# CDCgov/zoe

Measured on AMD Instinct MI355X. Metric: read-alignments/sec (150 bp vs 2 kb ref), higher is better.
Workload: dtype int16

## Files before the change

include/zoe_sw.h:

```cpp
#ifndef ZOE_SW_H
#define ZOE_SW_H

#include <stddef.h>
#include <stdint.h>

#ifdef __cplusplus
extern "C" {
#endif

typedef enum zsw_error {
    ZSW_OK = 0,
    ZSW_ERR_EMPTY_SEQUENCE = 1,
    ZSW_ERR_GAP_OPEN_OUT_OF_RANGE = 2,
    ZSW_ERR_GAP_EXTEND_OUT_OF_RANGE = 3,
    ZSW_ERR_BAD_GAP_WEIGHTS = 4,
    ZSW_ERR_INVALID_ARGUMENT = -1,
    ZSW_ERR_HIP = -2,
    ZSW_ERR_NO_DEVICE = -3,
    ZSW_ERR_UNSUPPORTED = -4,
    ZSW_ERR_NOT_CONFIGURED = -5
} zsw_error;

typedef enum zsw_status {
    ZSW_STATUS_SOME = 0,
    ZSW_STATUS_OVERFLOWED = 1,
    ZSW_STATUS_UNMAPPED = 2,
    ZSW_STATUS_EMPTY = 3,
    ZSW_STATUS_BELOW_MIN_SCORE = 4
} zsw_status;

typedef enum zsw_int_type { ZSW_I8 = 0, ZSW_I16 = 1, ZSW_I32 = 2, ZSW_U8 = 3, ZSW_U16 = 4, ZSW_U32 = 5 } zsw_int_type;

typedef enum zsw_mem { ZSW_MEM_HOST = 0, ZSW_MEM_DEVICE = 1 } zsw_mem;

typedef struct zsw_context zsw_context;

typedef enum zsw_encoding { ZSW_ENCODING_BYTES = 0, ZSW_ENCODING_PACKED4 = 1 } zsw_encoding;

typedef struct zsw_batch {
    const uint8_t* bases;
    const uint64_t* offsets;
    uint32_t fixed_len;
    uint64_t n_reads;
    zsw_mem mem;
    zsw_encoding encoding;
} zsw_batch;

typedef struct zsw_alignment {
    uint32_t score;
    uint32_t ref_start, ref_end;
    uint32_t query_start, query_end;
    uint32_t ref_len, query_len;
    uint32_t n_ciglets;
    uint64_t ciglet_offset;
} zsw_alignment;

zsw_error zsw_pack4_host(zsw_context* ctx, const uint8_t* bases, uint64_t n_reads, uint32_t len, uint8_t* out_packed);

zsw_error zsw_create(int device_id, zsw_context** out);
void zsw_destroy(zsw_context* ctx);
const char* zsw_last_error_string(const zsw_context* ctx);
int zsw_device_count(void);

zsw_error zsw_set_scoring(zsw_context* ctx, const int8_t* weights, int S, const uint8_t* index_map, int gap_open,
                          int gap_extend);

zsw_error zsw_set_reference(zsw_context* ctx, const uint8_t* reference, size_t len, zsw_mem mem);

zsw_error zsw_score_batch(zsw_context* ctx, const zsw_batch* reads, zsw_int_type int_type, int lanes,
                          uint32_t* out_score, uint8_t* out_status, void* stream);

zsw_error zsw_score_batch_from(zsw_context* ctx, const zsw_batch* reads, int from_width, int preset_bits,
                               uint32_t* out_score, uint8_t* out_status, uint8_t* out_tier, void* stream);

zsw_error zsw_score_ends_batch(zsw_context* ctx, const zsw_batch* reads, zsw_int_type int_type, int lanes,
                               uint32_t* out_score, uint32_t* out_ref_end, uint32_t* out_query_end,
                               uint8_t* out_status, void* stream);

zsw_error zsw_score_ranges_batch(zsw_context* ctx, const zsw_batch* reads, zsw_int_type int_type, int lanes,
                                 uint32_t* out_score, uint32_t* out_ref_start, uint32_t* out_ref_end,
                                 uint32_t* out_query_start, uint32_t* out_query_end, uint8_t* out_status, void* stream);

zsw_error zsw_score_ranges_batch_from(zsw_context* ctx, const zsw_batch* reads, int from_width, int preset_bits,
                                      uint32_t* out_score, uint32_t* out_ref_start, uint32_t* out_ref_end,
                                      uint32_t* out_query_start, uint32_t* out_query_end, uint8_t* out_status, uint8_t* out_tier,
                                      void* stream);

zsw_error zsw_align_batch(zsw_context* ctx, const zsw_batch* reads, zsw_int_type int_type, int lanes, int invert,
                          zsw_alignment* out_aln, uint8_t* out_status, uint32_t* out_inc, uint8_t* out_op,
                          uint64_t ciglet_cap, uint64_t* out_n_ciglets, void* stream);

zsw_error zsw_align_batch_from(zsw_context* ctx, const zsw_batch* reads, int from_width, int preset_bits, int invert,
                               zsw_alignment* out_aln, uint8_t* out_status, uint8_t* out_tier, uint32_t* out_inc,
                               uint8_t* out_op, uint64_t ciglet_cap, uint64_t* out_n_ciglets, void* stream);

zsw_error zsw_align_3pass_batch(zsw_context* ctx, const zsw_batch* reads, zsw_int_type int_type, int lanes, int invert,
                                zsw_alignment* out_aln, uint8_t* out_status, uint32_t* out_inc, uint8_t* out_op,
                                uint64_t ciglet_cap, uint64_t* out_n_ciglets, void* stream);
zsw_error zsw_align_3pass_batch_from(zsw_context* ctx, const zsw_batch* reads, int from_width, int preset_bits, int invert,
                                     zsw_alignment* out_aln, uint8_t* out_status, uint8_t* out_tier, uint32_t* out_inc,
                                     uint8_t* out_op, uint64_t ciglet_cap, uint64_t* out_n_ciglets, void* stream);


zsw_error zsw_set_complement(zsw_context* ctx, const uint8_t* table );

zsw_error zsw_score_strands_batch_from(zsw_context* ctx, const zsw_batch* reads, int from_width, int preset_bits,
                                       uint32_t* out_score, uint8_t* out_status, uint8_t* out_tier, uint8_t* out_strand, void* stream);

zsw_error zsw_orient_batch(zsw_context* ctx, const zsw_batch* reads, const uint8_t* strand, uint8_t* out_bases, void* stream);

zsw_error zsw_align_3pass_strands_batch_from(zsw_context* ctx, const zsw_batch* reads, int from_width, int preset_bits, int invert,
                                             zsw_alignment* out_aln, uint8_t* out_status, uint8_t* out_tier, uint8_t* out_strand,
                                             uint32_t* out_inc, uint8_t* out_op, uint64_t ciglet_cap, uint64_t* out_n_ciglets, void* stream);

zsw_error zsw_strand_counts(zsw_context* ctx, uint64_t* out );

zsw_error zsw_set_profile_sequence(zsw_context* ctx, const uint8_t* sequence, size_t len, zsw_mem mem);
zsw_error zsw_score_shared_batch(zsw_context* ctx, const zsw_batch* reads, zsw_int_type int_type, int lanes, uint32_t* out_score,
                                 uint8_t* out_status, void* stream);
zsw_error zsw_score_shared_batch_from(zsw_context* ctx, const zsw_batch* reads, int from_width, int preset_bits, uint32_t* out_score,
                                      uint8_t* out_status, uint8_t* out_tier, void* stream);
zsw_error zsw_score_ends_shared_batch(zsw_context* ctx, const zsw_batch* reads, zsw_int_type int_type, int lanes, uint32_t* out_score,
                                      uint32_t* out_ref_end, uint32_t* out_query_end, uint8_t* out_status, void* stream);
zsw_error zsw_score_ranges_shared_batch(zsw_context* ctx, const zsw_batch* reads, zsw_int_type int_type, int lanes, uint32_t* out_score,
                                        uint32_t* out_ref_start, uint32_t* out_ref_end, uint32_t* out_query_start, uint32_t* out_query_end,
                                        uint8_t* out_status, void* stream);
zsw_error zsw_score_ranges_shared_batch_from(zsw_context* ctx, const zsw_batch* reads, int from_width, int preset_bits, uint32_t* out_score,
                                             uint32_t* out_ref_start, uint32_t* out_ref_end, uint32_t* out_query_start, uint32_t* out_query_end,
                                             uint8_t* out_status, uint8_t* out_tier, void* stream);
zsw_error zsw_align_shared_batch(zsw_context* ctx, const zsw_batch* reads, zsw_int_type int_type, int lanes, int invert, zsw_alignment* out_aln,
                                 uint8_t* out_status, uint32_t* out_inc, uint8_t* out_op, uint64_t ciglet_cap, uint64_t* out_n_ciglets,
                                 void* stream);
zsw_error zsw_align_shared_batch_from(zsw_context* ctx, const zsw_batch* reads, int from_width, int preset_bits, int invert,
                                      zsw_alignment* out_aln, uint8_t* out_status, uint8_t* out_tier, uint32_t* out_inc, uint8_t* out_op,
                                      uint64_t ciglet_cap, uint64_t* out_n_ciglets, void* stream);
zsw_error zsw_align_3pass_shared_batch(zsw_context* ctx, const zsw_batch* reads, zsw_int_type int_type, int lanes, int invert, zsw_alignment* out_aln,
                                       uint8_t* out_status, uint32_t* out_inc, uint8_t* out_op, uint64_t ciglet_cap, uint64_t* out_n_ciglets,
                                       void* stream);
zsw_error zsw_align_3pass_shared_batch_from(zsw_context* ctx, const zsw_batch* reads, int from_width, int preset_bits, int invert,
                                            zsw_alignment* out_aln, uint8_t* out_status, uint8_t* out_tier, uint32_t* out_inc, uint8_t* out_op,
                                            uint64_t ciglet_cap, uint64_t* out_n_ciglets, void* stream);

typedef enum zsw_filter_result {
    ZSW_FILTER_REJECT = 0,
    ZSW_FILTER_PASS = 1,
    ZSW_FILTER_NONE = 2,
    ZSW_FILTER_BAD_WINDOW = 255
} zsw_filter_result;
zsw_error zsw_sneaky_snake_batch(zsw_context* ctx, const zsw_batch* reads, const uint32_t* ref_start, const uint32_t* ref_len,
                                 float threshold, uint8_t* out_pass, void* stream);

typedef struct zsw_group zsw_group;
zsw_error zsw_group_create(const int* device_ids, int n_devices, zsw_group** out);
void zsw_group_destroy(zsw_group* group);
int zsw_group_size(const zsw_group* group);
zsw_context* zsw_group_context(zsw_group* group, int i);
const char* zsw_group_last_error_string(const zsw_group* group);
zsw_error zsw_group_set_scoring(zsw_group* group, const int8_t* weights, int S, const uint8_t* index_map, int gap_open,
                                int gap_extend);
zsw_error zsw_group_set_reference(zsw_group* group, const uint8_t* reference, size_t len);

zsw_error zsw_group_score_batch_from(zsw_group* group, const zsw_batch* reads, int from_width, int preset_bits,
                                     uint32_t* out_score, uint8_t* out_status, uint8_t* out_tier);

zsw_error zsw_group_align_batch_from(zsw_group* group, const zsw_batch* reads, int from_width, int preset_bits, int invert,
                                     zsw_alignment* out_aln, uint8_t* out_status, uint8_t* out_tier, uint32_t* out_inc,
                                     uint8_t* out_op, uint64_t ciglet_cap, uint64_t* out_n_ciglets);
zsw_error zsw_group_align_3pass_batch_from(zsw_group* group, const zsw_batch* reads, int from_width, int preset_bits, int invert,
                                           zsw_alignment* out_aln, uint8_t* out_status, uint8_t* out_tier, uint32_t* out_inc,
                                           uint8_t* out_op, uint64_t ciglet_cap, uint64_t* out_n_ciglets);

zsw_error zsw_group_score_batch_from_device(zsw_group* group, const zsw_batch* shards, int from_width, int preset_bits,
                                            uint32_t* const* out_score, uint8_t* const* out_status);

zsw_error zsw_synth_reads(zsw_context* ctx, uint64_t seed, uint64_t first, uint64_t n, uint32_t len, uint8_t* out_device,
                          void* stream);
zsw_error zsw_synth_reads_ragged(zsw_context* ctx, uint64_t seed, uint64_t first, uint64_t n, uint32_t min_len,
                                 uint32_t max_len, const uint64_t* offsets_device, uint8_t* out_device, void* stream);
uint32_t zsw_synth_length(uint64_t seed, uint64_t index, uint32_t min_len, uint32_t max_len);

zsw_error zsw_selftest(zsw_context* ctx);

void zsw_synth_reference_host(uint64_t seed, uint64_t len, uint8_t* out);
void zsw_synth_reads_host(uint64_t seed, uint64_t first, uint64_t n, uint32_t len, const uint8_t* ref, uint32_t R,
                          uint8_t* out);
void zsw_synth_reads_ragged_host(uint64_t seed, uint64_t first, uint64_t n, uint32_t min_len, uint32_t max_len,
                                 const uint64_t* offsets, const uint8_t* ref, uint32_t R, uint8_t* out);

zsw_error zsw_timing_enable(zsw_context* ctx, int enable);
zsw_error zsw_timing_read(zsw_context* ctx, double* seconds, uint64_t* launches);
zsw_error zsw_timing_read_window(zsw_context* ctx, double* seconds, uint64_t* launches);

typedef enum zsw_option { ZSW_OPTION_EXACT_PRUNING = 1, ZSW_OPTION_MIN_SCORE = 2 } zsw_option;
zsw_error zsw_set_option(zsw_context* ctx, zsw_option option, int64_t value);

zsw_error zsw_min_score_counts(zsw_context* ctx, uint64_t* out );

typedef enum zsw_debug_flag {
    ZSW_DEBUG_SCORE_V1 = 1,
    ZSW_DEBUG_NO_TILES = 2,
    ZSW_DEBUG_NO_W32 = 4,
    ZSW_DEBUG_NO_WIDE = 8,
    ZSW_DEBUG_NO_SIDE_STREAMS = 16,
    ZSW_DEBUG_NO_PIPELINE = 32,
    ZSW_DEBUG_ALIGN_NO_PACKED = 64,
    ZSW_DEBUG_SCORE_PRUNE = 128,
    ZSW_DEBUG_SCORE_PRUNE_ANY_SIZE = 256,
    ZSW_DEBUG_PRUNE_STRIP = 512,
    ZSW_DEBUG_ALIGN_LONG_WARMUP = 1024,
    ZSW_DEBUG_SEED_NO_BAND = 2048,
    ZSW_DEBUG_SEED_WIDE_BAND = 4096,
    ZSW_DEBUG_NO_ROW_CHUNKS = 8192,
    ZSW_DEBUG_RANGES_EXACT_REVERSE = 16384,
    ZSW_DEBUG_ALIGN_NO_CERTIFICATE = 32768,
    ZSW_DEBUG_SEED_STRIP_FIRST_TIER = 65536,
    ZSW_DEBUG_SEED_DIAG_LANE_EVENTS = 131072
} zsw_debug_flag;
zsw_error zsw_debug_set(zsw_context* ctx, uint32_t flags);

zsw_error zsw_debug_band_records(zsw_context* ctx, int32_t* records);

zsw_error zsw_debug_cert_records(zsw_context* ctx, int32_t* records);

zsw_error zsw_debug_strand_records(zsw_context* ctx, int32_t* records);

typedef enum zsw_launch_kind {
    ZSW_LAUNCH_V1_FAST = 0,
    ZSW_LAUNCH_V1_BIASED = 1,
    ZSW_LAUNCH_V2 = 2,
    ZSW_LAUNCH_WIDE = 3,
    ZSW_LAUNCH_V1_FAST_REV = 4,
    ZSW_LAUNCH_V1_BIASED_REV = 5,
    ZSW_LAUNCH_WIDE_REV = 6,
    ZSW_LAUNCH_TILE_V2 = 7,
    ZSW_LAUNCH_TILE_WIDE = 8,
    ZSW_LAUNCH_TILE_W32 = 9,
    ZSW_LAUNCH_EXACT32 = 10,
    ZSW_LAUNCH_EXACT32_WORKLIST = 11,
    ZSW_LAUNCH_SEED_WINDOW = 12,
    ZSW_LAUNCH_SEED_BAND = 13,
    ZSW_LAUNCH_PRUNED = 14
} zsw_launch_kind;
zsw_error zsw_debug_score_launches(zsw_context* ctx, uint32_t* records, uint32_t capacity, uint32_t* out_n);

zsw_error zsw_prune_rescored(zsw_context* ctx, uint64_t* out_reads);

#ifdef __cplusplus
}
#endif
#endif
```

zoe_amd/_lib.py:

```python
from __future__ import annotations

import ctypes as C
import os

_HERE = os.path.dirname(os.path.abspath(__file__))
LIB_PATH = os.path.join(_HERE, "libzoe_sw_hip.so")

ZSW_OK = 0
ERROR_NAMES = {
    0: "ZSW_OK",
    1: "ProfileError::EmptySequence",
    2: "ProfileError::GapOpenOutOfRange",
    3: "ProfileError::GapExtendOutOfRange",
    4: "ProfileError::BadGapWeights",
    -1: "ZSW_ERR_INVALID_ARGUMENT",
    -2: "ZSW_ERR_HIP",
    -3: "ZSW_ERR_NO_DEVICE",
    -4: "ZSW_ERR_UNSUPPORTED",
    -5: "ZSW_ERR_NOT_CONFIGURED",
}
MEM_HOST, MEM_DEVICE = 0, 1
DEBUG_SCORE_V1, DEBUG_NO_TILES, DEBUG_NO_W32, DEBUG_NO_WIDE, DEBUG_NO_SIDE_STREAMS, DEBUG_NO_PIPELINE, DEBUG_ALIGN_NO_PACKED = 1, 2, 4, 8, 16, 32, 64
DEBUG_SCORE_PRUNE, DEBUG_SCORE_PRUNE_ANY_SIZE, DEBUG_PRUNE_STRIP, DEBUG_ALIGN_LONG_WARMUP, DEBUG_SEED_NO_BAND, DEBUG_SEED_WIDE_BAND = 128, 256, 512, 1024, 2048, 4096
DEBUG_NO_ROW_CHUNKS = 8192
DEBUG_RANGES_EXACT_REVERSE = 16384
DEBUG_ALIGN_NO_CERTIFICATE = 32768
DEBUG_SEED_STRIP_FIRST_TIER = 65536
DEBUG_SEED_DIAG_LANE_EVENTS = 131072
(LAUNCH_V1_FAST, LAUNCH_V1_BIASED, LAUNCH_V2, LAUNCH_WIDE, LAUNCH_V1_FAST_REV, LAUNCH_V1_BIASED_REV, LAUNCH_WIDE_REV, LAUNCH_TILE_V2, LAUNCH_TILE_WIDE,
 LAUNCH_TILE_W32, LAUNCH_EXACT32, LAUNCH_EXACT32_WORKLIST, LAUNCH_SEED_WINDOW, LAUNCH_SEED_BAND, LAUNCH_PRUNED) = range(15)
OPTION_EXACT_PRUNING = 1
OPTION_MIN_SCORE = 2
INT_TYPES = {"i8": 0, "i16": 1, "i32": 2, "u8": 3, "u16": 4, "u32": 5}

SYMBOLS = [
    "zsw_pack4_host", "zsw_create", "zsw_destroy", "zsw_last_error_string", "zsw_device_count", "zsw_set_scoring", "zsw_set_reference",
    "zsw_score_batch", "zsw_score_batch_from", "zsw_score_ends_batch", "zsw_score_ranges_batch", "zsw_score_ranges_batch_from", "zsw_align_batch", "zsw_align_batch_from", "zsw_align_3pass_batch", "zsw_align_3pass_batch_from", "zsw_sneaky_snake_batch",
    "zsw_set_profile_sequence", "zsw_score_shared_batch", "zsw_score_shared_batch_from", "zsw_score_ends_shared_batch", "zsw_score_ranges_shared_batch",
    "zsw_score_ranges_shared_batch_from", "zsw_align_shared_batch", "zsw_align_shared_batch_from", "zsw_align_3pass_shared_batch", "zsw_align_3pass_shared_batch_from",
    "zsw_synth_reads", "zsw_synth_reads_ragged", "zsw_synth_length", "zsw_synth_reference_host", "zsw_synth_reads_host",
    "zsw_synth_reads_ragged_host", "zsw_selftest", "zsw_timing_enable", "zsw_timing_read", "zsw_timing_read_window", "zsw_debug_set", "zsw_debug_band_records", "zsw_debug_cert_records", "zsw_prune_rescored", "zsw_set_option",
    "zsw_group_create", "zsw_group_destroy", "zsw_group_size", "zsw_group_context", "zsw_group_last_error_string", "zsw_group_set_scoring",
    "zsw_group_set_reference", "zsw_group_score_batch_from", "zsw_group_score_batch_from_device", "zsw_group_align_batch_from",
    "zsw_group_align_3pass_batch_from",
    "zsw_set_complement", "zsw_score_strands_batch_from", "zsw_orient_batch", "zsw_align_3pass_strands_batch_from", "zsw_strand_counts", "zsw_debug_strand_records", "zsw_debug_score_launches",
    "zsw_min_score_counts",
]


class ZswBatch(C.Structure):
    _fields_ = [
        ("bases", C.c_void_p),
        ("offsets", C.c_void_p),
        ("fixed_len", C.c_uint32),
        ("n_reads", C.c_uint64),
        ("mem", C.c_int),
        ("encoding", C.c_int),
    ]


class ZswAlignment(C.Structure):
    _fields_ = [
        ("score", C.c_uint32),
        ("ref_start", C.c_uint32),
        ("ref_end", C.c_uint32),
        ("query_start", C.c_uint32),
        ("query_end", C.c_uint32),
        ("ref_len", C.c_uint32),
        ("query_len", C.c_uint32),
        ("n_ciglets", C.c_uint32),
        ("ciglet_offset", C.c_uint64),
    ]


class ZswError(RuntimeError):
    def __init__(self, code: int, detail: str = ""):
        self.code = code
        name = ERROR_NAMES.get(code, str(code))
        super().__init__(f"{name}{': ' + detail if detail else ''}")


_lib = None


def load() -> C.CDLL:
    global _lib
    if _lib is not None:
        return _lib
    if not os.path.exists(LIB_PATH):
        raise ZswError(-3, f"{LIB_PATH} not built: run `python -m zoe_amd.build` (hipcc, gfx950)")
    import torch

    lib = C.CDLL(LIB_PATH)
    vp, u8p, u32p, u64p = C.c_void_p, C.c_void_p, C.c_void_p, C.c_void_p
    lib.zsw_create.argtypes = [C.c_int, C.POINTER(C.c_void_p)]
    lib.zsw_destroy.argtypes = [vp]
    lib.zsw_destroy.restype = None
    lib.zsw_last_error_string.argtypes = [vp]
    lib.zsw_last_error_string.restype = C.c_char_p
    lib.zsw_set_scoring.argtypes = [vp, C.c_void_p, C.c_int, C.c_void_p, C.c_int, C.c_int]
    lib.zsw_set_reference.argtypes = [vp, C.c_void_p, C.c_size_t, C.c_int]
    lib.zsw_score_batch.argtypes = [vp, C.POINTER(ZswBatch), C.c_int, C.c_int, u32p, u8p, vp]
    lib.zsw_score_batch_from.argtypes = [vp, C.POINTER(ZswBatch), C.c_int, C.c_int, u32p, u8p, u8p, vp]
    lib.zsw_score_ends_batch.argtypes = [vp, C.POINTER(ZswBatch), C.c_int, C.c_int, u32p, u32p, u32p, u8p, vp]
    lib.zsw_score_ranges_batch.argtypes = [vp, C.POINTER(ZswBatch), C.c_int, C.c_int, u32p, u32p, u32p, u32p, u32p, u8p, vp]
    lib.zsw_score_ranges_batch_from.argtypes = [vp, C.POINTER(ZswBatch), C.c_int, C.c_int, u32p, u32p, u32p, u32p, u32p, u8p, u8p, vp]
    lib.zsw_align_batch.argtypes = [vp, C.POINTER(ZswBatch), C.c_int, C.c_int, C.c_int, vp, u8p, u32p, u8p, C.c_uint64, C.POINTER(C.c_uint64), vp]
    lib.zsw_align_batch_from.argtypes = [vp, C.POINTER(ZswBatch), C.c_int, C.c_int, C.c_int, vp, u8p, u8p, u32p, u8p, C.c_uint64, C.POINTER(C.c_uint64), vp]
    lib.zsw_align_3pass_batch.argtypes = lib.zsw_align_batch.argtypes
    lib.zsw_align_3pass_batch_from.argtypes = lib.zsw_align_batch_from.argtypes
    lib.zsw_set_profile_sequence.argtypes = [vp, C.c_void_p, C.c_size_t, C.c_int]
    lib.zsw_score_shared_batch.argtypes = lib.zsw_score_batch.argtypes
    lib.zsw_score_shared_batch_from.argtypes = lib.zsw_score_batch_from.argtypes
    lib.zsw_score_ends_shared_batch.argtypes = lib.zsw_score_ends_batch.argtypes
    lib.zsw_score_ranges_shared_batch.argtypes = lib.zsw_score_ranges_batch.argtypes
    lib.zsw_score_ranges_shared_batch_from.argtypes = lib.zsw_score_ranges_batch_from.argtypes
    lib.zsw_align_shared_batch.argtypes = lib.zsw_align_batch.argtypes
    lib.zsw_align_shared_batch_from.argtypes = lib.zsw_align_batch_from.argtypes
    lib.zsw_align_3pass_shared_batch.argtypes = lib.zsw_align_shared_batch.argtypes
    lib.zsw_align_3pass_shared_batch_from.argtypes = lib.zsw_align_batch_from.argtypes
    lib.zsw_sneaky_snake_batch.argtypes = [vp, C.POINTER(ZswBatch), u32p, u32p, C.c_float, u8p, vp]
    lib.zsw_synth_reads.argtypes = [vp, C.c_uint64, C.c_uint64, C.c_uint64, C.c_uint32, vp, vp]
    lib.zsw_synth_reads_ragged.argtypes = [vp, C.c_uint64, C.c_uint64, C.c_uint64, C.c_uint32, C.c_uint32, u64p, vp, vp]
    lib.zsw_synth_length.argtypes = [C.c_uint64, C.c_uint64, C.c_uint32, C.c_uint32]
    lib.zsw_synth_length.restype = C.c_uint32
    lib.zsw_synth_reference_host.argtypes = [C.c_uint64, C.c_uint64, vp]
    lib.zsw_synth_reference_host.restype = None
    lib.zsw_synth_reads_host.argtypes = [C.c_uint64, C.c_uint64, C.c_uint64, C.c_uint32, vp, C.c_uint32, vp]
    lib.zsw_synth_reads_host.restype = None
    lib.zsw_synth_reads_ragged_host.argtypes = [C.c_uint64, C.c_uint64, C.c_uint64, C.c_uint32, C.c_uint32, u64p, vp, C.c_uint32, vp]
    lib.zsw_synth_reads_ragged_host.restype = None
    lib.zsw_selftest.argtypes = [vp]
    lib.zsw_timing_enable.argtypes = [vp, C.c_int]
    lib.zsw_timing_read.argtypes = [vp, C.POINTER(C.c_double), C.POINTER(C.c_uint64)]
    lib.zsw_timing_read_window.argtypes = [vp, C.POINTER(C.c_double), C.POINTER(C.c_uint64)]
    lib.zsw_debug_set.argtypes = [vp, C.c_uint32]
    lib.zsw_debug_band_records.argtypes = [vp, vp]
    lib.zsw_debug_cert_records.argtypes = [vp, vp]
    lib.zsw_pack4_host.argtypes = [vp, vp, C.c_uint64, C.c_uint32, vp]
    lib.zsw_prune_rescored.argtypes = [vp, C.POINTER(C.c_uint64)]
    lib.zsw_set_option.argtypes = [vp, C.c_int, C.c_int64]
    lib.zsw_group_create.argtypes = [C.POINTER(C.c_int), C.c_int, C.POINTER(vp)]
    lib.zsw_group_destroy.argtypes = [vp]
    lib.zsw_group_destroy.restype = None
    lib.zsw_group_size.argtypes = [vp]
    lib.zsw_group_context.argtypes = [vp, C.c_int]
    lib.zsw_group_context.restype = vp
    lib.zsw_group_last_error_string.argtypes = [vp]
    lib.zsw_group_last_error_string.restype = C.c_char_p
    lib.zsw_group_set_scoring.argtypes = [vp, vp, C.c_int, vp, C.c_int, C.c_int]
    lib.zsw_group_set_reference.argtypes = [vp, vp, C.c_size_t]
    lib.zsw_group_score_batch_from.argtypes = [vp, C.POINTER(ZswBatch), C.c_int, C.c_int, vp, vp, vp]
    lib.zsw_group_score_batch_from_device.argtypes = [vp, C.POINTER(ZswBatch), C.c_int, C.c_int, C.POINTER(vp), C.POINTER(vp)]
    lib.zsw_group_align_batch_from.argtypes = [vp, C.POINTER(ZswBatch), C.c_int, C.c_int, C.c_int, vp, vp, vp, vp, vp, C.c_uint64, C.POINTER(C.c_uint64)]
    lib.zsw_group_align_3pass_batch_from.argtypes = lib.zsw_group_align_batch_from.argtypes
    lib.zsw_set_complement.argtypes = [vp, vp]
    lib.zsw_score_strands_batch_from.argtypes = [vp, C.POINTER(ZswBatch), C.c_int, C.c_int, u32p, u8p, u8p, u8p, vp]
    lib.zsw_orient_batch.argtypes = [vp, C.POINTER(ZswBatch), u8p, u8p, vp]
    lib.zsw_align_3pass_strands_batch_from.argtypes = [vp, C.POINTER(ZswBatch), C.c_int, C.c_int, C.c_int, vp, u8p, u8p, u8p, u32p, u8p, C.c_uint64, C.POINTER(C.c_uint64), vp]
    lib.zsw_strand_counts.argtypes = [vp, C.POINTER(C.c_uint64)]
    lib.zsw_debug_strand_records.argtypes = [vp, vp]
    lib.zsw_debug_score_launches.argtypes = [vp, u32p, C.c_uint32, u32p]
    lib.zsw_min_score_counts.argtypes = [vp, C.POINTER(C.c_uint64)]
    _lib = lib
    return lib
```

zoe_amd/build.py:

```python
from __future__ import annotations

import os
import shutil
import subprocess
import sys

HERE = os.path.dirname(os.path.abspath(__file__))
CSRC = os.path.join(HERE, "csrc")
LIB = os.path.join(HERE, "libzoe_sw_hip.so")
SOURCES = ["zsw_capi.hip", "zsw_capi_shared.hip", "zsw_shared.hip", "zsw_score.hip", "zsw_align.hip", "zsw_align_pk8.hip", "zsw_align_pk16.hip", "zsw_align_pk32.hip", "zsw_align_pk64.hip", "zsw_group.hip", "zsw_threepass.hip", "zsw_filter.hip", "zsw_score_wide.hip", "zsw_score_w32.hip", "zsw_score_prune.hip", "zsw_score_seed.hip", "zsw_score_seed_m0.hip", "zsw_score_seed_m1.hip", "zsw_score_seed_m2.hip", "zsw_score_band.hip", "zsw_multi.hip", "zsw_strand.hip"]
HEADERS = ["zsw_internal.hpp", "zsw_align_dev.hpp", "zsw_align_pk.hpp", "zsw_align_pk_kernel.hpp", "zsw_score_v1.hpp", "zsw_score_v2.hpp", "zsw_handback.hpp", "zsw_score_prune.hpp", "zsw_seed.hpp", "zsw_seed_diag.hpp", "zsw_cert.hpp", "zsw_context.hpp", "zsw_shared.hpp", "zsw_score_seed.hpp", "zsw_score_seed_kernel.hpp", "zsw_align.hpp", "zsw_timer.hpp", "zsw_strand.hpp", "zsw_synth.h", "zsw_exports.map", os.path.join("..", "..", "include", "zoe_sw.h")]
ARCH = "gfx950"
EXTRA_FLAGS = {}


def _hipcc() -> str:
    for cand in (shutil.which("hipcc"), "/opt/rocm/bin/hipcc"):
        if cand and os.path.exists(cand):
            return cand
    raise RuntimeError("hipcc not found: the HIP extension cannot be built")


def needs_build() -> bool:
    if not os.path.exists(LIB):
        return True
    t = os.path.getmtime(LIB)
    deps = [os.path.join(CSRC, s) for s in SOURCES + HEADERS] + [os.path.abspath(__file__)]
    return any(os.path.exists(d) and os.path.getmtime(d) > t for d in deps)


def build(force: bool = False, verbose: bool = False) -> str:
    if not force and not needs_build():
        return LIB
    objs = []
    procs = []
    for s in SOURCES:
        src = os.path.join(CSRC, s)
        if not os.path.exists(src):
            continue
        obj = os.path.join(CSRC, s.replace(".hip", ".o"))
        cmd = [_hipcc(), f"--offload-arch={ARCH}", "-O3", "-std=c++17", "-fPIC", "-c", src, "-o", obj,
               "-Wall", "-Wno-unused-function", "-Wno-unused-result"] + EXTRA_FLAGS.get(s, [])
        if verbose:
            cmd.append("-Rpass-analysis=kernel-resource-usage")
        procs.append((s, subprocess.Popen(cmd, stdout=subprocess.PIPE, stderr=subprocess.STDOUT, text=True)))
        objs.append(obj)
    failed = False
    for s, p in procs:
        out, _ = p.communicate()
        if p.returncode != 0:
            failed = True
            sys.stderr.write(f"--- hipcc failed for {s}\n{out}\n")
        elif verbose or out.strip():
            sys.stderr.write(out)
    if failed:
        raise RuntimeError("hipcc compilation failed")
    cmd = [_hipcc(), f"--offload-arch={ARCH}", "-shared", "-fPIC", "-o", LIB, "-Wl,--version-script=" + os.path.join(CSRC, "zsw_exports.map")] + objs
    subprocess.run(cmd, check=True)
    return LIB


def fatbin_sha256(path: str = LIB) -> str:
    import hashlib
    import struct

    with open(path, "rb") as f:
        data = f.read()
    if data[:4] != b"\x7fELF" or data[4] != 2:
        raise RuntimeError("not a 64-bit ELF file: " + path)
    shoff, = struct.unpack_from("<Q", data, 0x28)
    shentsize, shnum, shstrndx = struct.unpack_from("<HHH", data, 0x3A)

    def section(i):
        name, _type, _flags, _addr, off, size = struct.unpack_from("<IIQQQQ", data, shoff + i * shentsize)
        return name, off, size

    _, stroff, strsize = section(shstrndx)
    names = data[stroff:stroff + strsize]
    for i in range(shnum):
        name, off, size = section(i)
        if names[name:names.index(b"\0", name)] == b".hip_fatbin":
            return hashlib.sha256(data[off:off + size]).hexdigest()
    raise RuntimeError("no .hip_fatbin section in " + path)


def build_driver(name: str = "zsw_driver") -> str:
    root = os.path.dirname(HERE)
    src = os.path.join(root, "examples", name + ".cpp")
    out = os.path.join(root, "examples", name)
    deps = [src, os.path.join(root, "include", "zoe_sw.hpp"), os.path.join(root, "include", "zoe_sw.h"), LIB]
    if os.path.exists(out) and all(os.path.getmtime(d) <= os.path.getmtime(out) for d in deps):
        return out
    subprocess.run(["g++", "-O2", "-std=c++17", "-Wall", "-I" + os.path.join(root, "include"), src, "-o", out, "-L" + HERE,
                    "-lzoe_sw_hip", "-Wl,-rpath,$ORIGIN/../zoe_amd", "-Wl,-rpath-link,/opt/rocm/lib"], check=True)
    return out


if __name__ == "__main__":
    print(build(force="--force" in sys.argv, verbose="-v" in sys.argv))
```

zoe_amd/csrc/zsw_handback.hpp:

```cpp
#pragma once
#include <algorithm>
#include <cstdint>

namespace zsw {

struct StripCfg {
    int G, C;
};

inline bool strip_config_first_fit(const StripCfg* cfgs, int n_ascending, uint32_t max_len, int* G, int* C) {
    for (int k = 0; k < n_ascending; ++k) {
        if ((uint32_t)(cfgs[k].G * cfgs[k].C) >= max_len) {
            *G = cfgs[k].G;
            *C = cfgs[k].C;
            return true;
        }
    }
    return false;
}

inline bool strip_config_for_batch(const StripCfg* cfgs, int n_cfgs, uint32_t max_len, uint32_t n_items, int* G, int* C) {
    double best = 0;
    bool found = false;
    for (int k = 0; k < n_cfgs; ++k) {
        const StripCfg& c = cfgs[k];
        if ((uint32_t)(c.G * c.C) < max_len) continue;
        const double waves = ((double)((n_items + 1) / 2) * c.G) / 64.0;
        const double cost = (7.5 * c.C + 25.0) * std::max(2048.0, waves);
        if (!found || cost < best * 0.97) {
            best = cost;
            *G = c.G;
            *C = c.C;
            found = true;
        }
    }
    return found;
}

constexpr uint32_t HANDBACK_CUTS[2] = {49152u, 327680u};
constexpr uint32_t HANDBACK_PROBE[2] = {16384u, 131072u};
constexpr int HANDBACK_MAX_LAUNCHES = 3;

struct HandbackLaunch {
    uint32_t lo, hi;
    int G, C;
    uint32_t grid_items;
    bool own_tables;
};

template <class TablesOk>
inline int handback_plan(const StripCfg* cfgs, int n_cfgs, uint32_t longest, int g, int c, uint32_t n_items, TablesOk tables_ok,
                         HandbackLaunch out[HANDBACK_MAX_LAUNCHES]) {
    int n = 0;
    uint32_t lo = 0;
    for (int k = 0; k < 3; ++k) {
        const uint32_t hi = k < 2 ? HANDBACK_CUTS[k] : 0xffffffffu;
        if (n_items == 0 || lo > n_items) break;
        int g2 = g, c2 = c;
        const bool other = k < 2 && strip_config_for_batch(cfgs, n_cfgs, longest, HANDBACK_PROBE[k], &g2, &c2) && g2 != g;
        if (k < 2 && (!other || !tables_ok(g2))) continue;
        out[n++] = other ? HandbackLaunch{lo, hi, g2, c2, std::min(n_items, hi), true} : HandbackLaunch{lo, hi, g, c, n_items, false};
        lo = hi;
    }
    return n;
}

}
```

zoe_amd/csrc/zsw_score.hip:

```cpp
#include <stdlib.h>

#include <algorithm>

#include "zsw_internal.hpp"
#include "zsw_score_v1.hpp"
#include "zsw_score_prune.hpp"
#include "zsw_score_seed.hpp"
#include "zsw_score_v2.hpp"
#include "zsw_handback.hpp"
#include "zsw_timer.hpp"

namespace zsw {

__global__ __launch_bounds__(64) void exact32_kernel(BatchDev b, const uint32_t* list, const uint32_t* list_count,
                                                     const uint8_t* ref, uint32_t ref_len, const ScoringDev* sc,
                                                     ResultRule rule, ScoreOut out, int32_t* scratch, uint32_t slots,
                                                     uint32_t scratch_len, const uint32_t* rev_ref_end,
                                                     const uint32_t* rev_query_end) {
    __shared__ uint8_t lut[256];
    __shared__ int32_t w[MAX_S * MAX_S];
    for (int i = threadIdx.x; i < 256; i += 64) lut[i] = sc->index_map[i];
    for (int i = threadIdx.x; i < MAX_S * MAX_S; i += 64) w[i] = sc->w[i];
    __syncthreads();
    const int S = sc->S;
// ... 235 lines not shown
    }
    return v2_range_setup(s, G, a);
}

static bool doubled_tables(const ScoringDev& s, ScoreArgsV2* a) {
    ScoringDev d = s;
    for (int i = 0; i < s.S * s.S; ++i) d.w[i] = 2 * s.w[i];
    d.gap_open = 2 * s.gap_open;
    d.gap_extend = 2 * s.gap_extend;
    return v2_ok(d, 0) && build_tables_v2(d, 1, a);
}

static bool wide_ok(const ScoringDev& s, uint32_t debug) {
    if (debug & ZSW_DEBUG_NO_WIDE) return false;
    if (s.S <= 7 || s.S > 32) return false;
    for (int i = 0; i < s.S * s.S; ++i) {
        const int t = s.w[i] + s.gap_extend;
        if (t < -128 || t > 127) return false;
    }
    return true;
}

static void fill_wide_table(const ScoringDev& s, ScoreArgsV2* a) {
    const int ge = s.gap_extend;
    for (int r = 0; r < 33; ++r)
        for (int q = 0; q < WIDE_STRIDE; ++q)
            a->wide[r * WIDE_STRIDE + q] = (int8_t)((r < s.S && q < s.S) ? s.w[r * s.S + q] + ge : ge);
}

static bool build_tables_wide(const ScoringDev& s, int G, ScoreArgsV2* a) {
    fill_wide_table(s, a);
    return v2_range_setup(s, G, a);
}

static bool w32_ok(const ScoringDev& s, uint32_t ref_len, uint32_t max_len, uint32_t debug) {
    if ((debug & ZSW_DEBUG_NO_W32) || s.S > 32) return false;
    int maxw = 0;
    for (int i = 0; i < s.S * s.S; ++i) {
        const int t = s.w[i] + s.gap_extend;
        if (t < -128 || t > 127) return false;
        maxw = std::max(maxw, (int)s.w[i]);
    }
    const uint64_t top = ((uint64_t)ref_len + TILE_G + 4) * (uint64_t)s.gap_extend + (uint64_t)max_len * (uint64_t)maxw;
    return top < 0x7f000000ull;
}

static hipError_t launch_table_cfg(const ScoreArgs& a, int G, int C, bool fast, int mode, hipStream_t stream) {
    switch (G * 100 + C) {
#define ZSW_CASE(GV, CV) \
    case GV * 100 + CV: return launch_cfg<GV, CV>(a, fast, mode, stream);
        ZSW_FOR_EACH_STRIP_CONFIG(ZSW_CASE)
#undef ZSW_CASE
    }
    return hipErrorInvalidValue;
}

static const int kBucketCfg[] = {0, 1, 2, 3, 4, 5, 6, 8, 9, 10, 11, 12, 13, 14, 15, 16, 17, 18, 19};
constexpr int NCLS = 19;

struct BucketCaps {
    uint32_t cap[NCLS];
};

__device__ __forceinline__ int bucket_of(const BucketCaps& caps, uint32_t len) {
    int k = 0;
    while (k < NCLS && len > caps.cap[k]) ++k;
    return k;
}

__global__ void reverse_bytes_kernel(const uint8_t* in, uint32_t n, uint8_t* out) {
    const uint32_t i = blockIdx.x * blockDim.x + threadIdx.x;
    if (i < n) out[i] = in[n - 1 - i];
}

__global__ void iota_kernel(uint32_t* out, uint32_t n) {
    const uint32_t i = blockIdx.x * blockDim.x + threadIdx.x;
    if (i < n) out[i] = i;
}

__global__ void bucket_count_kernel(const uint64_t* offsets, uint32_t n, BucketCaps caps, uint32_t* counts) {
    __shared__ uint32_t sh[NCLS + 1];
    if (threadIdx.x <= NCLS) sh[threadIdx.x] = 0;
    __syncthreads();
    for (uint32_t i = blockIdx.x * blockDim.x + threadIdx.x; i < n; i += gridDim.x * blockDim.x)
        atomicAdd(&sh[bucket_of(caps, (uint32_t)(offsets[i + 1] - offsets[i]))], 1u);
    __syncthreads();
    if (threadIdx.x <= NCLS && sh[threadIdx.x]) atomicAdd(&counts[threadIdx.x], sh[threadIdx.x]);
}

__global__ void bucket_scatter_kernel(const uint64_t* offsets, uint32_t n, BucketCaps caps, uint32_t* cursors, uint32_t* items) {
    const int lane = threadIdx.x & 63;
    const uint32_t per_sweep = gridDim.x * blockDim.x;
    for (uint32_t base = blockIdx.x * blockDim.x; base < n; base += per_sweep) {
        const uint32_t i = base + threadIdx.x;
        const bool valid = i < n;
        const int k = valid ? bucket_of(caps, (uint32_t)(offsets[i + 1] - offsets[i])) : -1;
        unsigned long long todo = __ballot(valid);
        while (todo) {
            const int leader = __ffsll((long long)todo) - 1;
            const int kl = __shfl(k, leader, 64);
            const unsigned long long same = __ballot(valid && k == kl);
            if (k == kl) {
                uint32_t start = 0;
                if (lane == leader) start = atomicAdd(&cursors[kl], (uint32_t)__popcll(same));
                start = (uint32_t)__shfl((int)start, leader, 64);
                items[start + (uint32_t)__popcll(same & ((1ull << lane) - 1ull))] = i;
            }
            todo &= ~same;
        }
    }
}

__global__ void add_count_kernel(const uint32_t* count, uint32_t* total) { atomicAdd(total, *count); }

__global__ void min_filter_kernel(BatchDev b, uint32_t min_thr, ScoreOut out, uint32_t* count) {
    uint32_t mine = 0;
    for (uint32_t i = blockIdx.x * blockDim.x + threadIdx.x; i < b.n_items; i += gridDim.x * blockDim.x) {
        const uint32_t id = b.items ? b.items[i] : i;
        const uint8_t st = out.status[id];
        if (st == ZSW_STATUS_UNMAPPED || (st == ZSW_STATUS_SOME && out.score[id] < min_thr)) {
            out.score[id] = 0;
            out.status[id] = ZSW_STATUS_BELOW_MIN_SCORE;
            if (out.tier) out.tier[id] = 0;
            if (out.ref_end) out.ref_end[id] = 0;
            if (out.query_end) out.query_end[id] = 0;
            ++mine;
        }
    }
#pragma unroll
    for (int d = 32; d >= 1; d >>= 1) mine += (uint32_t)__shfl_xor((int)mine, d, 64);
    if ((threadIdx.x & 63) == 0 && mine) atomicAdd(count, mine);
}

static hipError_t launch_score_passes(const ScoringDev* d_sc, const ScoringDev& h_sc, const BatchDev& b, uint32_t max_len,
                                      const uint8_t* d_ref, uint32_t ref_len, const ResultRule& rule, const ScoreOut& out,
                                      const ScoreWorkspace& ws, hipStream_t stream, KernelTimer* timer, int mode);

hipError_t launch_score(const ScoringDev* d_sc, const ScoringDev& h_sc, const BatchDev& b, uint32_t max_len,
                        const uint8_t* d_ref, uint32_t ref_len, const ResultRule& rule, const ScoreOut& out,
                        const ScoreWorkspace& ws, hipStream_t stream, KernelTimer* timer, int mode) {
    hipError_t e = launch_score_passes(d_sc, h_sc, b, max_len, d_ref, ref_len, rule, out, ws, stream, timer, mode);
    if (e != hipSuccess || !ws.min_score || !ws.min_counts || b.n_items == 0) return e;
    hipLaunchKernelGGL(min_filter_kernel, dim3(std::min<uint32_t>((b.n_items + 255) / 256, 4096u)), dim3(256), 0, stream, b, min_threshold(rule, ws.min_score), out,
                       ws.min_counts + 2);
    return hipGetLastError();
}

static hipError_t launch_score_passes(const ScoringDev* d_sc, const ScoringDev& h_sc, const BatchDev& b, uint32_t max_len,
                                      const uint8_t* d_ref, uint32_t ref_len, const ResultRule& rule, const ScoreOut& out,
                                      const ScoreWorkspace& ws, hipStream_t stream, KernelTimer* timer, int mode) {
    hipError_t e = hipMemsetAsync(out.fb_count, 0, sizeof(uint32_t), stream);
    if (e != hipSuccess) return e;
    int G = 0, C = 0;
    const bool wide = wide_ok(h_sc, ws.debug);
    const bool table_ok = h_sc.S <= 7 || fast_ok(h_sc) || wide;
    const uint32_t exact_grid = (uint32_t)(ws.slots / 64);
    ScoreArgs a;
    a.b = b;
    a.ref = d_ref;
    a.ref_len = ref_len;
    a.sc = d_sc;
    a.rule = rule;
    a.out = out;
    a.rev_ref_end = nullptr;
    a.rev_query_end = nullptr;
    a.rev_score = nullptr;
    a.gtab = nullptr;
    const bool fast = fast_ok(h_sc);
    if (table_ok && !wide) build_tables(h_sc, fast, &a);
    const bool use_v2 = table_ok && !wide && v2_ok(h_sc, ws.debug);
    ScoreArgsV2 a2;
    a2.b = b;
    a2.ref = d_ref;
    a2.ref_len = ref_len;
    a2.sc = d_sc;
    a2.rule = rule;
    a2.out = out;
    a2.tile_q0 = 0;
    a2.tile_in = nullptr;
    a2.tile_out = nullptr;
    a2.tile_state = nullptr;
    a2.rev_ref_end = nullptr;
    a2.rev_query_end = nullptr;
    std::vector<uint32_t>* const launches = ws.launch_log;
    auto launch_one = [&](const BatchDev& bb, int g, int c) -> hipError_t {
        if (wide) {
            if (build_tables_wide(h_sc, g, &a2)) {
                a2.b = bb;
                if (bb.n_items) note_launch(launches, ZSW_LAUNCH_WIDE, g, c, mode == 0 ? 0 : 2);
                return launch_table_cfg_v2_wide(a2, g, c, mode, stream);
            }
            note_launch(launches, ZSW_LAUNCH_EXACT32, 0, 0, std::min(mode, 2));
            hipLaunchKernelGGL(exact32_kernel, dim3(exact_grid), dim3(64), 0, stream, bb, (const uint32_t*)nullptr,
                               (const uint32_t*)nullptr, d_ref, ref_len, d_sc, rule, out, ws.scratch, (uint32_t)ws.slots,
                               ws.scratch_len, (const uint32_t*)nullptr, (const uint32_t*)nullptr);
            return hipGetLastError();
        }
        if (use_v2 && build_tables_v2(h_sc, g, &a2)) {
            a2.b = bb;
            if (bb.n_items) note_launch(launches, ZSW_LAUNCH_V2, g, c, std::min(mode, 2));
            return launch_table_cfg_v2(a2, g, c, mode, stream);
        }
        a.b = bb;
        if (bb.n_items) note_launch(launches, fast ? ZSW_LAUNCH_V1_FAST : ZSW_LAUNCH_V1_BIASED, g, c, std::min(mode, 2));
        return launch_table_cfg(a, g, c, fast, mode, stream);
    };
    auto launch_tiled = [&](const BatchDev& bb, uint32_t longest) -> hipError_t {
        if (!ws.tile_buf || !ws.tile_state || !bb.items || (ws.debug & ZSW_DEBUG_NO_TILES)) return hipErrorNotSupported;
        if (!(wide || use_v2)) return hipErrorNotSupported;
        if (!(wide ? build_tables_wide(h_sc, TILE_G, &a2) : build_tables_v2(h_sc, TILE_G, &a2))) return hipErrorNotSupported;
        const size_t per_pair = (size_t)ref_len * sizeof(uint2);
        const size_t half = ws.tile_bytes / 2;
        const size_t fit = per_pair ? half / per_pair : (size_t)bb.n_items;
        if (fit == 0) return hipErrorNotSupported;
        const uint32_t chunk = (uint32_t)std::min<size_t>(2 * fit, 0x7ffffffeu);
        uint2* buf[2] = {ws.tile_buf, reinterpret_cast<uint2*>(reinterpret_cast<uint8_t*>(ws.tile_buf) + half)};
        const uint32_t n_tiles = (longest + TILE_COLS - 1) / TILE_COLS;
        for (uint32_t first = 0; first < bb.n_items; first += chunk) {
            a2.b = bb;
            a2.b.items = bb.items + first;
            a2.b.n_items = std::min<uint32_t>(chunk, bb.n_items - first);
            a2.tile_state = ws.tile_state;
            for (uint32_t t = 0; t < n_tiles; ++t) {
                a2.tile_q0 = t * (uint32_t)TILE_COLS;
                a2.tile_in = t ? buf[(t - 1) & 1] : nullptr;
                a2.tile_out = t + 1 < n_tiles ? buf[t & 1] : nullptr;
                if (a2.b.n_items) note_launch(launches, wide ? ZSW_LAUNCH_TILE_WIDE : ZSW_LAUNCH_TILE_V2, TILE_G, TILE_C, mode == 0 ? 0 : 2);
                hipError_t te = launch_tile_v2(a2, wide, mode, stream);
                if (te != hipSuccess) return te;
            }
        }
        return hipSuccess;
    };
    auto finish_worklist = [&]() -> hipError_t {
        int maxw = 1;
        for (int i = 0; i < h_sc.S * h_sc.S; ++i) maxw = std::max(maxw, (int)h_sc.w[i]);
        if ((uint64_t)max_len * (uint64_t)maxw >= 16384 && ws.tile_buf && ws.tile_state && w32_ok(h_sc, ref_len, max_len, ws.debug)) {
            uint32_t cnt = 0;
            hipError_t we = hipMemcpyAsync(&cnt, out.fb_count, sizeof(cnt), hipMemcpyDeviceToHost, stream);
            if (we == hipSuccess) we = hipStreamSynchronize(stream);
            if (we != hipSuccess) return we;
            if (cnt == 0) return hipSuccess;
            fill_wide_table(h_sc, &a2);
            a2.ge2 = (uint32_t)h_sc.gap_extend * 0x00010001u;
            a2.gd2 = (uint32_t)(h_sc.gap_open - h_sc.gap_extend) * 0x00010001u;
            const size_t per_read = (size_t)ref_len * sizeof(uint2), half = ws.tile_bytes / 2;
            const size_t fit = per_read ? half / per_read : (size_t)cnt;
            if (fit > 0) {
                uint2* buf[2] = {ws.tile_buf, reinterpret_cast<uint2*>(reinterpret_cast<uint8_t*>(ws.tile_buf) + half)};
                const uint32_t n_tiles = (max_len + TILE_COLS - 1) / TILE_COLS;
                for (uint32_t first = 0; first < cnt; first += (uint32_t)std::min<size_t>(fit, 0x7fffffffu)) {
                    a2.b = b;
                    a2.b.n_items = (uint32_t)std::min<size_t>(fit, cnt - first);
                    a2.tile_state = ws.tile_state;
                    for (uint32_t t = 0; t < n_tiles; ++t) {
                        a2.tile_q0 = t * (uint32_t)TILE_COLS;
                        a2.tile_in = t ? buf[(t - 1) & 1] : nullptr;
                        a2.tile_out = t + 1 < n_tiles ? buf[t & 1] : nullptr;
                        if (a2.b.n_items) note_launch(launches, ZSW_LAUNCH_TILE_W32, TILE_G, TILE_C, mode == 0 ? 0 : 2);
                        we = launch_tile_w32(a2, out.fb_list + first, mode, stream);
                        if (we != hipSuccess) return we;
                    }
                }
                return hipSuccess;
            }
        }
        note_launch(launches, ZSW_LAUNCH_EXACT32_WORKLIST, 0, 0, std::min(mode, 2));
        hipLaunchKernelGGL(exact32_kernel, dim3(exact_grid), dim3(64), 0, stream, b, out.fb_list, out.fb_count, d_ref, ref_len, d_sc,
                           rule, out, ws.scratch, (uint32_t)ws.slots, ws.scratch_len, (const uint32_t*)nullptr, (const uint32_t*)nullptr);
        return hipGetLastError();
    };
    auto exact_all = [&](const BatchDev& bb) {
        note_launch(launches, ZSW_LAUNCH_EXACT32, 0, 0, std::min(mode, 2));
        hipLaunchKernelGGL(exact32_kernel, dim3(exact_grid), dim3(64), 0, stream, bb, (const uint32_t*)nullptr,
                           (const uint32_t*)nullptr, d_ref, ref_len, d_sc, rule, out, ws.scratch, (uint32_t)ws.slots, ws.scratch_len, (const uint32_t*)nullptr, (const uint32_t*)nullptr);
        return hipGetLastError();
    };
    bool gtab_built = false;
    auto seed_items = [&](const BatchDev& bb, int g, int c, uint32_t longest, size_t work_off, uint32_t list_off, uint32_t* counter,
                          uint32_t band_grid_cap) -> hipError_t {
        if (!use_v2 || !ws.seed || !ws.seed_work || !ws.prune_fail_list || !(ws.debug & ZSW_DEBUG_SCORE_PRUNE) || (ws.debug & ZSW_DEBUG_PRUNE_STRIP))
            return hipErrorNotSupported;
        if (bb.n_items < SEED_MIN_READS && !(ws.debug & ZSW_DEBUG_SCORE_PRUNE_ANY_SIZE)) return hipErrorNotSupported;
        if (g == 32 || work_off + seed_workspace_bytes(bb.n_items, longest, band_grid_cap) > ws.seed_bytes) return hipErrorNotSupported;
        ScoreArgsV2 ap = a2;
        if (!build_tables_v2(h_sc, g, &ap) || !seed_applicable(*ws.seed, longest, ref_len, ap.limit)) return hipErrorNotSupported;
        if (!ws.seed_gtab) return hipErrorNotSupported;
        hipError_t pe = hipSuccess;
        ScoreArgsV2 ab = a2;
        const bool band_ok = !(ws.debug & ZSW_DEBUG_SEED_NO_BAND) && doubled_tables(h_sc, &ab);
        uint2* const gtab_band = ws.seed_gtab + (ref_len + 2 * SEED_GTAB_PAD);
        if (!gtab_built) {
            pe = seed_build_gtab(ap, ws.seed_gtab, stream);
            if (pe != hipSuccess) return pe;
            if (band_ok) {
                pe = seed_build_gtab(ab, gtab_band, stream);
                if (pe != hipSuccess) return pe;
            }
            gtab_built = true;
        }
        pe = hipMemsetAsync(counter, 0, 4, stream);
        if (pe != hipSuccess) return pe;
        ap.b = bb;
        pe = launch_score_seeded(ap, g, c, longest, *ws.seed, ws.seed_work + work_off, seed_workspace_bytes(bb.n_items, longest, band_grid_cap), ws.seed_gtab,
                                 ws.prune_fail_list + list_off, counter, mode, band_ok ? &ab : nullptr, gtab_band, ws.band_dbg,
                                 (ws.debug & ZSW_DEBUG_SEED_WIDE_BAND) ? 0xffffffffu : (ws.debug & ZSW_DEBUG_SCORE_PRUNE_ANY_SIZE) ? 0u : SEED_NARROW_MIN_READS, band_grid_cap, stream,
                                 ws.window_timer, out.narrow_only, out.reads_reversed && out.skip_handed_back, launches,
                                 (ws.debug & ZSW_DEBUG_SEED_STRIP_FIRST_TIER) != 0, (ws.debug & ZSW_DEBUG_SEED_DIAG_LANE_EVENTS) != 0,
                                 (ws.min_score && ws.min_counts && !out.skip_handed_back) ? min_threshold(rule, ws.min_score) : 0u, ws.min_counts);
        if (pe != hipSuccess) return pe;
        ap.b.items = ws.prune_fail_list + list_off;
        ap.n_items_dev = counter;
        if (!out.skip_handed_back) {
            int maxw = 0;
            for (int i = 0; i < h_sc.S * h_sc.S; ++i) maxw = std::max(maxw, (int)h_sc.w[i]);
            const uint64_t overlap = h_sc.gap_extend > 0 ? (uint64_t)longest + (uint64_t)longest * (uint64_t)maxw / (uint64_t)h_sc.gap_extend + 2 : ~0ull;
            const uint64_t rows = std::max<uint64_t>(4 * overlap, 2048);
            if (ws.chunk_keys && !(ws.debug & ZSW_DEBUG_NO_ROW_CHUNKS) && h_sc.gap_extend > 0 && rows * 2 <= ref_len && longest < (1u << CHUNK_COL_BITS) &&
                ref_len < (1u << CHUNK_ROW_BITS) - 2) {
                ap.chunk_rows = (uint32_t)rows;
                ap.chunk_overlap = (uint32_t)overlap;
                ap.chunk_keys = ws.chunk_keys;
                const uint32_t zgrid = (bb.n_items + 255) / 256;
                hipLaunchKernelGGL(chunk_zero_kernel, dim3(zgrid), dim3(256), 0, stream, ap.b.items, counter, bb.n_items, ws.chunk_keys);
                note_launch(launches, ZSW_LAUNCH_V2, g, c, std::min(mode, 2));
                pe = launch_table_cfg_v2(ap, g, c, mode, stream);
                if (pe != hipSuccess) return pe;
                hipLaunchKernelGGL(chunk_finalize_kernel, dim3(zgrid), dim3(256), 0, stream, ap.b, counter, ws.chunk_keys, ap.limit, rule, out, std::min(mode, 2));
                pe = hipGetLastError();
            } else {
                HandbackLaunch plan[HANDBACK_MAX_LAUNCHES];
                ScoreArgsV2 tabs[HANDBACK_MAX_LAUNCHES];
                int n_tabs = 0;
                const int n_plan = handback_plan(kCfgs, N_CFGS, longest, g, c, bb.n_items, [&](int g2) {
                    tabs[n_tabs] = a2;
                    if (!build_tables_v2(h_sc, g2, &tabs[n_tabs])) return false;
                    ++n_tabs;
                    return true;
                }, plan);
                for (int k = 0, t = 0; k < n_plan && pe == hipSuccess; ++k) {
                    ScoreArgsV2 ah = ap;
                    if (plan[k].own_tables) {
                        ah = tabs[t++];
                        ah.b = ap.b;
                        ah.n_items_dev = counter;
                    }
                    ah.b.n_items = plan[k].grid_items;
                    ah.gate_lo = plan[k].lo;
                    ah.gate_hi = plan[k].hi;
                    note_launch(launches, ZSW_LAUNCH_V2, plan[k].G, plan[k].C, std::min(mode, 2));
                    pe = launch_table_cfg_v2(ah, plan[k].G, plan[k].C, mode, stream);
                }
            }
        }
        if (pe != hipSuccess) return pe;
        if (!out.skip_handed_back) hipLaunchKernelGGL(add_count_kernel, dim3(1), dim3(1), 0, stream, counter, ws.prune_fail_count + 1);
        return hipGetLastError();
    };
    auto prune_items = [&](const BatchDev& bb, int cls, uint32_t n_cls) -> hipError_t {
        if (!(use_v2 || wide) || !ws.prune_work || !(ws.debug & ZSW_DEBUG_SCORE_PRUNE)) return hipErrorNotSupported;
        if (!wide && !(ws.debug & ZSW_DEBUG_PRUNE_STRIP)) return hipErrorNotSupported;
        if (bb.n_items < PR_MIN_READS && !(ws.debug & ZSW_DEBUG_SCORE_PRUNE_ANY_SIZE)) return hipErrorNotSupported;
        const int last = n_cls < bb.n_items ? cls + 1 : cls;
        ScoreArgsV2 ap = a2;
        auto tables = [&](int g, ScoreArgsV2* t) { return wide ? build_tables_wide(h_sc, g, t) : build_tables_v2(h_sc, g, t); };
        if (!tables(1, &ap)) return hipErrorNotSupported;
        const uint32_t floor_strip = ap.floor0;
        uint32_t limit = ap.limit, floor_window[2] = {0, 0};
        for (int c = cls; c <= last; ++c) {
            if (!tables(kPruneClasses[c].g, &ap)) return hipErrorNotSupported;
            floor_window[c - cls] = ap.floor0;
            limit = std::min(limit, ap.limit);
        }
        if (!prune_applicable(h_sc, kPruneClasses[last].max_len, ref_len, limit)) return hipErrorNotSupported;
        int Gr = 0, Cr = 0;
        if (!score_config_for(kPruneClasses[last].max_len, &Gr, &Cr)) return hipErrorNotSupported;
        hipError_t pe = hipMemsetAsync(ws.prune_fail_count, 0, 4, stream);
        if (pe != hipSuccess) return pe;
        ap.b = bb;
        uint32_t est_failed = 0xffffffffu;
        pe = launch_score_pruned(ap, cls, n_cls, floor_strip, floor_window, h_sc, ws.prune_work, ws.prune_bytes, ws.prune_chunk,
                                 ws.prune_fail_list, ws.prune_fail_count, mode, wide, stream, &est_failed);
        if (pe != hipSuccess) return pe;
        note_launch(launches, ZSW_LAUNCH_PRUNED, kPruneClasses[cls].g, kPruneClasses[cls].cp, std::min(mode, 2));
        if (est_failed != 0xffffffffu) (void)score_config_for_batch(kPruneClasses[last].max_len, est_failed + est_failed / 4 + 1024, &Gr, &Cr);
        if (!tables(Gr, &a2)) return hipErrorInvalidValue;
        a2.b = bb;
        a2.b.items = ws.prune_fail_list;
        a2.n_items_dev = ws.prune_fail_count;
        note_launch(launches, wide ? ZSW_LAUNCH_WIDE : ZSW_LAUNCH_V2, Gr, Cr, wide ? (mode == 0 ? 0 : 2) : std::min(mode, 2));
        pe = wide ? launch_table_cfg_v2_wide(a2, Gr, Cr, mode, stream) : launch_table_cfg_v2(a2, Gr, Cr, mode, stream);
        a2.n_items_dev = nullptr;
        if (pe != hipSuccess) return pe;
        hipLaunchKernelGGL(add_count_kernel, dim3(1), dim3(1), 0, stream, ws.prune_fail_count, ws.prune_fail_count + 1);
        return hipGetLastError();
    };
    if (!table_ok) {
        if (timer) timer->begin(stream);
        e = exact_all(b);
        if (timer) timer->end(stream);
        return e;
    }
    if (b.offsets && !b.items && b.n_items > 0) {
        BucketCaps caps;
        for (int k = 0; k < NCLS; ++k) caps.cap[k] = (uint32_t)(kCfgs[kBucketCfg[k]].G * kCfgs[kBucketCfg[k]].C);
        e = hipMemsetAsync(ws.bucket_counts, 0, 64 * sizeof(uint32_t), stream);
        if (e != hipSuccess) return e;
        const uint32_t hgrid = std::min<uint32_t>(1024, (b.n_items + 255) / 256);
        hipLaunchKernelGGL(bucket_count_kernel, dim3(hgrid), dim3(256), 0, stream, b.offsets, b.n_items, caps, ws.bucket_counts);
        uint32_t counts[NCLS + 1];
        e = hipMemcpyAsync(counts, ws.bucket_counts, sizeof(counts), hipMemcpyDeviceToHost, stream);
        if (e != hipSuccess) return e;
        e = hipStreamSynchronize(stream);
        if (e != hipSuccess) return e;
        uint32_t starts[NCLS + 1], run = 0;
        for (int k = 0; k <= NCLS; ++k) {
            starts[k] = run;
            run += counts[k];
        }
        e = hipMemcpyAsync(ws.bucket_counts + 32, starts, sizeof(starts), hipMemcpyHostToDevice, stream);
        if (e != hipSuccess) return e;
        hipLaunchKernelGGL(bucket_scatter_kernel, dim3(hgrid), dim3(256), 0, stream, b.offsets, b.n_items, caps,
                           ws.bucket_counts + 32, ws.bucket_items);
        if (timer) timer->begin(stream);
        SideStreams* side = ws.side;
        const bool fork = side != nullptr && !(ws.debug & ZSW_DEBUG_NO_SIDE_STREAMS);
        if (use_v2 && ws.seed && ws.seed_gtab && (ws.debug & ZSW_DEBUG_SCORE_PRUNE) && !(ws.debug & ZSW_DEBUG_PRUNE_STRIP)) {
            ScoreArgsV2 ag = a2;
            if (build_tables_v2(h_sc, 4, &ag)) {
                e = seed_build_gtab(ag, ws.seed_gtab, stream);
                if (e != hipSuccess) return e;
                ScoreArgsV2 ab = a2;
                if (!(ws.debug & ZSW_DEBUG_SEED_NO_BAND) && doubled_tables(h_sc, &ab)) {
                    e = seed_build_gtab(ab, ws.seed_gtab + (ref_len + 2 * SEED_GTAB_PAD), stream);
                    if (e != hipSuccess) return e;
                }
                gtab_built = true;
            }
        }
        if (fork) {
            e = hipEventRecord(side->fork, stream);
            if (e != hipSuccess) return e;
            for (int i = 0; i < SideStreams::N; ++i) {
                e = hipStreamWaitEvent(side->s[i], side->fork, 0);
                if (e != hipSuccess) return e;
            }
        }
        const hipStream_t main_stream = stream;
        int used = 0;
        {
            size_t work_off = 0;
            uint32_t n_seedable = 0;
            for (int k = 0; k < NCLS; ++k) n_seedable += counts[k];
            for (int k = NCLS - 1; k >= 0; --k) {
                if (!counts[k]) continue;
                BatchDev bk = b;
                bk.items = ws.bucket_items + starts[k];
                bk.n_items = counts[k];
                const Cfg& cf = kCfgs[kBucketCfg[k]];
                stream = fork ? side->s[used % SideStreams::N] : main_stream;
                const uint32_t grid_cap = seed_band_class_cap(counts[k], n_seedable);
                e = seed_items(bk, cf.G, cf.C, caps.cap[k], work_off, starts[k], ws.prune_fail_count + 2 + k, grid_cap);
                stream = main_stream;
                if (e == hipSuccess) ++used;
                if (e == hipSuccess) {
                    work_off += seed_workspace_bytes(counts[k], caps.cap[k], grid_cap);
                    counts[k] = 0;
                } else if (e != hipErrorNotSupported) {
                    return e;
                }
            }
        }
        {
            int k0[PR_N_CLASSES], k1[PR_N_CLASSES];
            uint32_t cnt[PR_N_CLASSES];
            for (int pc = 0; pc < PR_N_CLASSES; ++pc) {
                k0[pc] = k1[pc] = -1;
                cnt[pc] = 0;
                for (int k = 0; k < NCLS; ++k) {
                    const uint32_t cap = caps.cap[k];
                    if (cap <= kPruneClasses[pc].max_len && (pc == 0 || cap > kPruneClasses[pc - 1].max_len) && cap > (uint32_t)kPruneClasses[pc].cp + 40) {
                        if (k0[pc] < 0) k0[pc] = k;
                        k1[pc] = k;
                        cnt[pc] += counts[k];
                    }
                }
            }
            for (int pc = 0; pc < PR_N_CLASSES; ++pc) {
                if (k0[pc] < 0) continue;
                int last = pc;
                if (pc + 1 < PR_N_CLASSES && k0[pc + 1] == k1[pc] + 1 && kPruneClasses[pc + 1].cp == kPruneClasses[pc].cp && ref_len < (1u << 24)) last = pc + 1;
                BatchDev bp = b;
                bp.items = ws.bucket_items + starts[k0[pc]];
                bp.n_items = starts[k1[last]] + counts[k1[last]] - starts[k0[pc]];
                if (bp.n_items) {
                    e = prune_items(bp, pc, cnt[pc]);
                    if (e == hipSuccess) {
                        for (int k = k0[pc]; k <= k1[last]; ++k) counts[k] = 0;
                    } else if (e != hipErrorNotSupported) {
                        return e;
                    }
                }
                pc = last;
            }
        }
        for (int k = NCLS; k >= 0; --k) {
            if (!counts[k]) continue;
            BatchDev bk = b;
            bk.items = ws.bucket_items + starts[k];
            bk.n_items = counts[k];
            if (k == NCLS) {
                e = launch_tiled(bk, max_len);
                if (e == hipErrorNotSupported) e = exact_all(bk);
            } else {
                stream = fork ? side->s[used++ % SideStreams::N] : main_stream;
                e = launch_one(bk, kCfgs[kBucketCfg[k]].G, kCfgs[kBucketCfg[k]].C);
                stream = main_stream;
            }
            if (e != hipSuccess) return e;
        }
        if (fork) {
            for (int i = 0; i < SideStreams::N; ++i) {
                e = hipEventRecord(side->join[i], side->s[i]);
                if (e != hipSuccess) return e;
                e = hipStreamWaitEvent(stream, side->join[i], 0);
                if (e != hipSuccess) return e;
            }
        }
        if (timer) timer->end(stream);
    } else {
        if (!score_config_for_batch(max_len, b.n_items, &G, &C)) {
            if (timer) timer->begin(stream);
            BatchDev bl = b;
            if (!bl.items && ws.bucket_items) {
                hipLaunchKernelGGL(iota_kernel, dim3((b.n_items + 255) / 256), dim3(256), 0, stream, ws.bucket_items, b.n_items);
                bl.items = ws.bucket_items;
            }
            e = launch_tiled(bl, max_len);
            if (e == hipErrorNotSupported) {
                e = exact_all(b);
                if (timer) timer->end(stream);
                return e;
            }
            if (timer) timer->end(stream);
            if (e != hipSuccess) return e;
            return finish_worklist();
        }
        if (timer) timer->begin(stream);
        e = hipErrorNotSupported;
        {
            int Gs = 0, Cs = 0;
            if (score_config_for(max_len, &Gs, &Cs)) e = seed_items(b, Gs, Cs, max_len, 0, 0, ws.prune_fail_count, SEED_BAND_MAX_GRID);
        }
        const int cls = prune_class_for(max_len);
        if (e == hipErrorNotSupported && cls >= 0) e = prune_items(b, cls, b.n_items);
        if (e == hipErrorNotSupported) e = launch_one(b, G, C);
        if (timer) timer->end(stream);
        if (e != hipSuccess) return e;
    }
    return finish_worklist();
}

__global__ void gtab_kernel(const uint8_t* ref, uint32_t n, const ScoringDev* sc, ScoreArgs a, int wide, uint2* gtab) {
    const uint32_t i = blockIdx.x * blockDim.x + threadIdx.x;
    if (i < n) {
        const int idx = sc->index_map[ref[i]];
        gtab[i] = wide ? make_uint2((uint32_t)(idx * WIDE_STRIDE), 0u) : make_uint2(a.wtab[idx][0], a.wtab[idx][1]);
    }
}

template <int G, int C>
static hipError_t launch_cfg_rev(const ScoreArgs& a, bool fast, hipStream_t stream) {
    const uint32_t reads_per_block = 2 * (BLOCK / G);
    const uint32_t grid = (a.b.n_items + reads_per_block - 1) / reads_per_block;
    if (grid == 0) return hipSuccess;
    if (fast) hipLaunchKernelGGL((score_kernel<G, C, true, 2, true>), dim3(grid), dim3(BLOCK), 0, stream, a);
    else hipLaunchKernelGGL((score_kernel<G, C, false, 2, true>), dim3(grid), dim3(BLOCK), 0, stream, a);
    return hipGetLastError();
}

hipError_t launch_score_rev(const ScoringDev* d_sc, const ScoringDev& h_sc, const BatchDev& b, uint32_t max_len,
                            const uint8_t* d_ref, uint32_t ref_len, const ResultRule& rule, const ScoreOut& out,
                            const ScoreWorkspace& ws, const uint32_t* d_fwd_ref_end, const uint32_t* d_fwd_query_end,
                            const uint32_t* d_fwd_score, uint2* d_gtab, hipStream_t stream) {
    hipError_t e = hipMemsetAsync(out.fb_count, 0, sizeof(uint32_t), stream);
    if (e != hipSuccess) return e;
    const uint32_t exact_grid = (uint32_t)(ws.slots / 64);
    int G = 0, C = 0;
    const bool wide = wide_ok(h_sc, ws.debug);
    const bool table_ok = (h_sc.S <= 7 || fast_ok(h_sc) || wide) && score_config_for(max_len, &G, &C);
    if (!score_config_for(max_len, &G, &C) && ws.tile_buf && ws.tile_state && ws.bucket_items && w32_ok(h_sc, ref_len, max_len, ws.debug) && b.n_items) {
        uint8_t* d_rev = reinterpret_cast<uint8_t*>(d_gtab);
        if (ref_len) hipLaunchKernelGGL(reverse_bytes_kernel, dim3((ref_len + 255) / 256), dim3(256), 0, stream, d_ref, ref_len, d_rev);
        hipLaunchKernelGGL(iota_kernel, dim3((b.n_items + 255) / 256), dim3(256), 0, stream, ws.bucket_items, b.n_items);
        ScoreArgsV2 a2;
        a2.b = b;
        a2.ref = d_rev;
        a2.ref_len = ref_len;
        a2.sc = d_sc;
        a2.rule = rule;
        a2.out = out;
        a2.rev_ref_end = d_fwd_ref_end;
        a2.rev_query_end = d_fwd_query_end;
        a2.tile_state = ws.tile_state;
        fill_wide_table(h_sc, &a2);
        a2.ge2 = (uint32_t)h_sc.gap_extend * 0x00010001u;
        a2.gd2 = (uint32_t)(h_sc.gap_open - h_sc.gap_extend) * 0x00010001u;
        const size_t per_read = (size_t)ref_len * sizeof(uint2), half = ws.tile_bytes / 2;
        const size_t fit = per_read ? half / per_read : (size_t)b.n_items;
        if (fit > 0) {
            uint2* buf[2] = {ws.tile_buf, reinterpret_cast<uint2*>(reinterpret_cast<uint8_t*>(ws.tile_buf) + half)};
            const uint32_t n_tiles = (max_len + TILE_COLS - 1) / TILE_COLS;
            for (uint32_t first = 0; first < b.n_items; first += (uint32_t)std::min<size_t>(fit, 0x7fffffffu)) {
                a2.b.n_items = (uint32_t)std::min<size_t>(fit, b.n_items - first);
                for (uint32_t t = 0; t < n_tiles; ++t) {
                    a2.tile_q0 = t * (uint32_t)TILE_COLS;
                    a2.tile_in = t ? buf[(t - 1) & 1] : nullptr;
                    a2.tile_out = t + 1 < n_tiles ? buf[t & 1] : nullptr;
                    note_launch(ws.launch_log, ZSW_LAUNCH_TILE_W32, TILE_G, TILE_C, 2);
                    e = launch_tile_w32(a2, ws.bucket_items + first, 2, stream);
                    if (e != hipSuccess) return e;
                }
            }
            return hipSuccess;
        }
    }
    if (!table_ok) {
        note_launch(ws.launch_log, ZSW_LAUNCH_EXACT32, 0, 0, 2);
        hipLaunchKernelGGL(exact32_kernel, dim3(exact_grid), dim3(64), 0, stream, b, (const uint32_t*)nullptr,
                           (const uint32_t*)nullptr, d_ref, ref_len, d_sc, rule, out, ws.scratch, (uint32_t)ws.slots,
                           ws.scratch_len, d_fwd_ref_end, d_fwd_query_end);
        return hipGetLastError();
    }
    ScoreArgs a;
    a.b = b;
    a.ref = d_ref;
    a.ref_len = ref_len;
    a.sc = d_sc;
    a.rule = rule;
    a.out = out;
    a.rev_ref_end = d_fwd_ref_end;
    a.rev_query_end = d_fwd_query_end;
    a.rev_score = d_fwd_score;
    a.gtab = d_gtab;
    const bool fast = fast_ok(h_sc);
    if (wide) {
        for (int r = 0; r < 33; ++r)
            for (int q = 0; q < WIDE_STRIDE; ++q)
// ... 34 lines not shown
```

zoe_amd/csrc/zsw_score_band.hip:

```cpp
#include <algorithm>
#include <type_traits>

#include "zsw_score_seed.hpp"
#include "zsw_seed_diag.hpp"
#include "zsw_score_v2.hpp"
#include "zsw_timer.hpp"

namespace zsw {

namespace {

constexpr int BC_NARROW = 16, BC_WIDE = 48;

enum BandField {
    BF_M_A, BF_STRIDE_A, BF_C0_A, BF_MAGIC_A, BF_MASKS_A, BF_M_B, BF_STRIDE_B, BF_C0_B, BF_MAGIC_B, BF_MASKS_B, BF_LAM2,
    BF_UP_CH, BF_UP_FR, BF_LO_CH, BF_LO_FR, BF_OA, BF_OB, BF_YH, BF_YF, BF_N
};
constexpr uint32_t PKB = 0x2000u, PKB2 = PKB * 0x00010001u;

struct BandLayout {
    int m, stride, c0;
    uint32_t magic, fa, fb;
};
struct BandPk {
    uint32_t ch, fr;
};

__device__ __forceinline__ void band_lane_init(const SeedParams& p, int* st, int lenA, uint32_t masksA, int lenB, uint32_t masksB) {
    int m, stride, c0;
    seed_layout(lenA, p.K, p.spacer, &m, &stride, &c0);
    st[BF_M_A * BLOCK] = m;
    st[BF_STRIDE_A * BLOCK] = stride;
    st[BF_C0_A * BLOCK] = c0;
    st[BF_MAGIC_A * BLOCK] = (int)seed_div_magic(stride);
    st[BF_MASKS_A * BLOCK] = (int)masksA;
    const uint32_t lamA = (uint32_t)seed_lambda(p, stride);
    seed_layout(lenB, p.K, p.spacer, &m, &stride, &c0);
    st[BF_M_B * BLOCK] = m;
    st[BF_STRIDE_B * BLOCK] = stride;
    st[BF_C0_B * BLOCK] = c0;
    st[BF_MAGIC_B * BLOCK] = (int)seed_div_magic(stride);
    st[BF_MASKS_B * BLOCK] = (int)masksB;
    st[BF_LAM2 * BLOCK] = (int)(lamA | ((uint32_t)seed_lambda(p, stride) << 16));
    st[BF_UP_CH * BLOCK] = st[BF_LO_CH * BLOCK] = (int)PKB2;
    st[BF_UP_FR * BLOCK] = st[BF_LO_FR * BLOCK] = 0;
    st[BF_OA * BLOCK] = st[BF_OB * BLOCK] = 0;
    st[BF_YH * BLOCK] = st[BF_YF * BLOCK] = 0;
}
__device__ __forceinline__ BandLayout band_layout(const int* st, bool second) {
    BandLayout y;
    const int o = second ? (BF_M_B - BF_M_A) * BLOCK : 0;
    y.m = st[BF_M_A * BLOCK + o];
    y.stride = st[BF_STRIDE_A * BLOCK + o];
    y.c0 = st[BF_C0_A * BLOCK + o];
    y.magic = (uint32_t)st[BF_MAGIC_A * BLOCK + o];
    const uint32_t masks = (uint32_t)st[BF_MASKS_A * BLOCK + o];
    y.fa = masks & 0xffffu;
    y.fb = masks >> 16;
    return y;
}

__device__ __forceinline__ uint32_t half_mask(uint32_t bitsA, uint32_t bitsB, int c) {
    const uint32_t mA = (uint32_t)__builtin_amdgcn_sbfe((int)bitsA, (uint32_t)c, 1u), mB = (uint32_t)__builtin_amdgcn_sbfe((int)bitsB, (uint32_t)c, 1u);
    return __builtin_amdgcn_perm(mB, mA, 0x05040100u);
}
__device__ __forceinline__ uint32_t half_mask(uint64_t bitsA, uint64_t bitsB, int c) {
    return half_mask((uint32_t)(c < 32 ? bitsA : bitsA >> 32), (uint32_t)(c < 32 ? bitsB : bitsB >> 32), c & 31);
}
__device__ __forceinline__ int mask_popc(uint32_t x) { return __popc(x); }
__device__ __forceinline__ int mask_popc(uint64_t x) { return __popcll(x); }
template <class M>
__device__ __forceinline__ M mask_first(int n) {
    return n >= (int)sizeof(M) * 8 ? ~(M)0 : (((M)1 << n) - 1u);
}
__device__ __forceinline__ uint32_t pk_subu_sat(uint32_t a, uint32_t b) {
    return __builtin_bit_cast(uint32_t, __builtin_elementwise_sub_sat(__builtin_bit_cast(us2, a), __builtin_bit_cast(us2, b)));
}
__device__ __forceinline__ uint32_t pk_shr1(uint32_t a) { return __builtin_bit_cast(uint32_t, __builtin_bit_cast(us2, a) >> (us2){1, 1}); }
template <int TAG>
__device__ __forceinline__ uint32_t pk_tag(uint32_t v) {
    if (TAG < 0) return pk_maxu(v << 1, 0x00010001u) - 0x00010001u;
    uint32_t nz;
    asm("v_pk_min_u16 %0, %1, %2" : "=v"(nz) : "v"(v), "v"(0x00010001u));
    return (v << 1) | nz;
}
template <int TAG>
__device__ __forceinline__ uint32_t pk_untag(uint32_t t2) {
    return TAG > 0 ? pk_shr1(t2) : pk_shr1(pk_addu(t2, 0x00010001u));
}
__device__ __forceinline__ void pk_events(BandPk* t, uint32_t sm, uint32_t em, uint32_t lam2) {
    t->fr = pk_maxu(t->fr, PKB2 & sm);
    t->ch = pk_subu(t->ch, lam2 & em);
    t->ch = pk_maxu(t->ch, t->fr & em);
    t->fr &= ~em;
}

struct BandPair {
    uint32_t ridA, ridB, idA, idB, itemA, itemB, lenA, lenB;
    int dtA, dtB;
    bool validB;
};
struct BandEnds {
    int rowA = 0x7fffffff, rowB = 0x7fffffff, colA = 0x7fffffff, colB = 0x7fffffff;
    bool multA = false, multB = false;
};

__device__ __forceinline__ int band_fetch(const SeedBandArgs& a, int tid, uint32_t n_items, uint32_t n_pairs, bool bail, int slack, BandPair* p) {
    uint32_t base = 0;
    if ((tid & 63) == 0) base = atomicAdd(a.next_pair, 64u);
    base = (uint32_t)__shfl((int)base, 0, 64);
    if (base >= n_pairs) return 0;
    const uint32_t pair = base + (uint32_t)(tid & 63);
    const uint32_t itemA = 2 * pair, itemB = itemA + 1;
    uint32_t ridA = 0, keyA = a.fail_key;
    if (pair < n_pairs) {
        ridA = a.order[itemA];
        keyA = a.keys[ridA];
    }
    const bool active = keyA != a.fail_key;
    if (__ballot(active) == 0) return 0;
    if (!active) return 1;
    uint32_t ridB = itemB < n_items ? a.order[itemB] : ridA;
    uint32_t keyB = itemB < n_items ? a.keys[ridB] : a.fail_key;
    bool validB = keyB != a.fail_key;
    const int dtA = (int)keyA - (int)a.key_bias;
    int dtB = validB ? (int)keyB - (int)a.key_bias : dtA;
    const uint32_t idA = a.b.items ? a.b.items[ridA] : ridA;
    uint32_t idB = validB ? (a.b.items ? a.b.items[ridB] : ridB) : idA;
    if (bail) {
        a.fail_list[atomicAdd(a.fail_count, 1u)] = idA;
        if (validB) a.fail_list[atomicAdd(a.fail_count, 1u)] = idB;
        return 1;
    }
    if (validB && dtB - dtA > slack) {
        if (a.retry) a.retry[itemB] = 1;
        else a.fail_list[atomicAdd(a.fail_count, 1u)] = idB;
        validB = false;
        dtB = dtA;
    }
    if (!validB) ridB = ridA;
    p->ridA = ridA;
    p->ridB = ridB;
    p->idA = idA;
    p->idB = idB;
    p->itemA = itemA;
    p->itemB = itemB;
    p->lenA = a.b.offsets ? (uint32_t)(a.b.offsets[idA + 1] - a.b.offsets[idA]) : a.b.fixed_len;
    p->lenB = validB ? (a.b.offsets ? (uint32_t)(a.b.offsets[idB + 1] - a.b.offsets[idB]) : a.b.fixed_len) : 0u;
    p->dtA = dtA;
    p->dtB = dtB;
    p->validB = validB;
    return 2;
}

template <int MODE, bool MINS>
__device__ __forceinline__ void band_finish(const SeedBandArgs& a, const BandPair& p, uint32_t best, uint32_t oa2, uint32_t ob2, int dtmin, int dtmax, int geom, int C,
                                            uint32_t infoA, uint32_t infoB, const BandEnds& e, uint32_t* n_accepted, uint32_t* n_below) {
    const uint32_t best2A = best & 0xffffu, best2B = best >> 16;
    const int tallA = (int)(infoA & 0xffffu), tallB = (int)(infoB & 0xffffu);
    const int dfaA = (int)((infoA >> 16) & 0xffu), dfaB = (int)((infoB >> 16) & 0xffu);
#pragma unroll
    for (int h = 0; h < 2; ++h) {
        if (h == 1 && !p.validB) break;
        const uint32_t id = h ? p.idB : p.idA;
        const uint32_t b2 = h ? best2B : best2A;
        const int oa = (int)((oa2 >> (h ? 16 : 0)) & 0xffffu), ob = (int)((ob2 >> (h ? 16 : 0)) & 0xffffu);
        const int S = (int)(b2 >> 1), outside = max(oa, ob);
        const bool redo = (b2 & 1u) != 0 || (MODE == 0 ? outside > S : outside >= S);
        if (a.dbg) {
            int* rec = a.dbg + (size_t)id * 8;
            rec[0] = (int)b2;
            rec[1] = oa;
            rec[2] = ob;
            rec[3] = dtmin;
            rec[4] = dtmax;
            rec[5] = geom;
            rec[6] = h ? p.dtB : p.dtA;
            rec[7] = (((h ? p.lenB : p.lenA) == 0 || redo) ? 0 : 1) | (C << 8);
        }
        if (MINS && (h ? p.lenB : p.lenA) != 0 && redo && seed_below_min(seed_band_upper(b2, oa, ob), a.min_thr)) {
            ++*n_accepted;
            ++*n_below;
            a.out.score[id] = 0;
            a.out.status[id] = ZSW_STATUS_BELOW_MIN_SCORE;
            if (a.out.tier) a.out.tier[id] = 0;
            if (MODE != 0 && a.out.ref_end) a.out.ref_end[id] = 0;
            if (MODE >= 2 && a.out.query_end) a.out.query_end[id] = 0;
        } else if ((h ? p.lenB : p.lenA) == 0 || redo) {
            if (a.retry) a.retry[h ? p.itemB : p.itemA] = 1;
            else a.fail_list[atomicAdd(a.fail_count, 1u)] = id;
        } else {
            ++*n_accepted;
            uint32_t score;
            uint8_t status, tier;
            apply_rule(a.rule, (uint64_t)S, &score, &status, &tier);
            a.out.score[id] = score;
            a.out.status[id] = status;
            if (a.out.tier) a.out.tier[id] = tier;
            const bool some = status == ZSW_STATUS_SOME;
            if (MODE != 0 && a.out.ref_end) a.out.ref_end[id] = some ? (uint32_t)(h ? e.rowB : e.rowA) + 1 : 0;
            if (MODE >= 2 && a.out.query_end) a.out.query_end[id] = some ? (uint32_t)(h ? e.colB : e.colA) + 1 : 0;
            if (MODE == 3 && a.out.unique) a.out.unique[id] = (some && !(h ? e.multB : e.multA)) ? 1 : 0;
            if (MODE != 0 && a.out.safe_row)
                a.out.safe_row[id] = (uint32_t)seed_safe_start(a.sp, h ? tallB : tallA, h ? dfaB : dfaA, h ? p.dtB : p.dtA, S);
        }
    }
}

__device__ __forceinline__ void band_count_accepted(const SeedBandArgs& a, int tid, uint32_t n_accepted) {
    if (a.retry && a.accepted) {
#pragma unroll
        for (int d = 32; d >= 1; d >>= 1) n_accepted += (uint32_t)__shfl_xor((int)n_accepted, d, 64);
        if ((tid & 63) == 0 && n_accepted) atomicAdd(a.accepted, n_accepted);
    }
}
__device__ __forceinline__ void band_count_below(const SeedBandArgs& a, int tid, uint32_t n_below) {
#pragma unroll
    for (int d = 32; d >= 1; d >>= 1) n_below += (uint32_t)__shfl_xor((int)n_below, d, 64);
    if ((tid & 63) == 0 && n_below) atomicAdd(a.min_count, n_below);
}

template <int C, int MINW, int MODE, bool MINS>
__global__ __launch_bounds__(BLOCK, MINW) void seed_band_kernel(SeedBandArgs a) {
    constexpr int TAG = MODE == 0 ? -1 : 1;
    using M = std::conditional_t<(C > 32), uint64_t, uint32_t>;
    static_assert(C % 8 == 0 && C <= 64, "a strip's residue codes are whole dwords; its column masks at most 64 bits");
    __shared__ uint16_t sel_lut[16];
    __shared__ int sst[BF_N * BLOCK];
    const int tid = threadIdx.x;
    int* const st = sst + tid;
    if (tid < 16) {
        const uint32_t k = (uint32_t)tid;
        sel_lut[tid] = (uint16_t)(k < 4 ? (2 * k + 1) | ((8 + k) << 8) : (k == 15 ? 0x0c00u : (2 * (k - 3)) | 0x0c00u));
    }
    __syncthreads();
    const int R = (int)a.ref_len;
    const uint32_t n_items = a.n_dev ? min(*a.n_dev, a.n) : a.n;
    const uint32_t n_pairs = (n_items + 1) / 2;
    const bool bail = a.bail_check && a.accepted && ((uint64_t)(*a.accepted) * SEED_BAIL_RATIO < (uint64_t)n_items || n_items < a.bail_below);
    uint32_t n_accepted = 0;
    uint32_t n_below = 0;
    const uint32_t ge2 = a.ge2, gd2 = a.gd2;
    const uint32_t ge1 = ge2 & 0xffffu;
    const uint32_t maxw2 = (uint32_t)a.sp.maxw * 0x00010001u, go2p = (uint32_t)a.sp.go * 0x00010001u;
    uint2* bnd = a.bnd + (size_t)blockIdx.x * (size_t)a.nb * BLOCK + tid;

    for (;;) {
        BandPair P;
        const int fetched = band_fetch(a, tid, n_items, n_pairs, bail, SEED_BAND_SLACK, &P);
        if (fetched == 0) break;
        if (fetched == 2) {
        const uint32_t ridA = P.ridA, ridB = P.ridB, lenA = P.lenA, lenB = P.lenB;
        const int dtA = P.dtA, dtB = P.dtB;
        const bool validB = P.validB;
        const int lenmax = (int)max(lenA, lenB);
        const int n_strips = (lenmax + C - 1) / C;
        const int wu = a.wu0 + lenmax * a.wu_per16 / 16, wd = a.wd0 + lenmax * a.wd_per32 / 32;
        const int dtmin = min(dtA, dtB), dtmax = max(dtA, dtB);
        const uint32_t infoA = a.info[ridA], infoB = a.info[ridB];
        band_lane_init(a.sp, st, (int)lenA, a.band_masks[ridA], (int)lenB, validB ? a.band_masks[ridB] : 0u);

        const uint32_t* codeA = a.codes + (size_t)ridA * a.cs;
        const uint32_t* codeB = a.codes + (size_t)ridB * a.cs;
        uint32_t best = 0;
        int bestA = 0, bestB = 0, rowA = 0x7fffffff, rowB = 0x7fffffff, colA = 0x7fffffff, colB = 0x7fffffff;
        bool multA = false, multB = false;
        int prev_bot = 0;
#pragma unroll 1
        for (int k = 0; k < n_strips; ++k) {
            uint32_t sel[C];
#pragma unroll
            for (int d = 0; d < C / 8; ++d) {
                const uint32_t di = (uint32_t)(k * (C / 8) + d);
                const uint32_t wa = di < a.cs ? codeA[di] : 0xffffffffu;
                const uint32_t wb = (validB && di < a.cs) ? codeB[di] : 0xffffffffu;
#pragma unroll
                for (int j = 0; j < 8; ++j)
                    sel[8 * d + j] = (uint32_t)sel_lut[(wa >> (4 * j)) & 15u] | ((uint32_t)sel_lut[(wb >> (4 * j)) & 15u] << 16);
            }
            const int top = max(0, min(R, dtmin + k * C - wu)), bot = max(0, min(R, dtmax + (k + 1) * C + wd));
            const bool has_next = k + 1 < n_strips;
            const int next_top = max(0, min(R, dtmin + (k + 1) * C - wu));
            const int nrA = max(0, min(C, (int)lenA - k * C)), nrB = max(0, min(C, (int)lenB - k * C));
            uint32_t Dr = (a.floor0 - ge1) * 0x00010001u;
            uint32_t H[C], E[C];
            const bool all_full = __ballot(nrA != C || nrB != C) == 0;
            const uint32_t lam2 = (uint32_t)st[BF_LAM2 * BLOCK];
            {
                const BandLayout yA = band_layout(st, false), yB = band_layout(st, true);
                const SeedStripEventsT<M> eA = seed_strip_events_t<M>(k * C, C, yA.m, yA.c0, yA.stride, a.sp.K, yA.magic, yA.fa);
                const SeedStripEventsT<M> eB = seed_strip_events_t<M>(k * C, C, yB.m, yB.c0, yB.stride, a.sp.K, yB.magic, yB.fa);
                const M any = eA.start | eA.end | eB.start | eB.end;
                BandPk up;
                up.ch = (uint32_t)st[BF_UP_CH * BLOCK];
                up.fr = (uint32_t)st[BF_UP_FR * BLOCK];
                uint32_t oa2 = (uint32_t)st[BF_OA * BLOCK];
                const uint32_t above = top > 0 ? 0xffffffffu : 0u;
                const uint32_t DrE = pk_addu(Dr, ge2);
                auto sweep = [&](auto full_tag) {
                    constexpr bool FULL = decltype(full_tag)::value;
                    const M realA = mask_first<M>(nrA), realB = mask_first<M>(nrB);
#pragma unroll
                    for (int c = 0; c < C; ++c) {
                        up.ch += maxw2;
                        up.fr += maxw2;
                        if (__ballot((uint32_t)(any >> c) & 1u) != 0) pk_events(&up, half_mask(eA.start, eB.start, c), half_mask(eA.end, eB.end, c), lam2);
                        uint32_t v = pk_subu_sat(pk_maxu(up.ch, up.fr), PKB2) & above;
                        if (!FULL) v &= half_mask(realA, realB, c);
                        oa2 = pk_maxu(oa2, v);
                        H[c] = pk_addu(Dr, pk_tag<TAG>(v));
                        E[c] = pk_addu(DrE, pk_tag<TAG>(pk_subu_sat(v, go2p)));
                    }
                };
                if (all_full) sweep(std::true_type{});
                else sweep(std::false_type{});
                st[BF_UP_CH * BLOCK] = (int)up.ch;
                st[BF_UP_FR * BLOCK] = (int)up.fr;
                st[BF_OA * BLOCK] = (int)oa2;
            }
            const bool have_left = k > 0;
            const uint32_t yh2 = have_left ? pk_tag<TAG>((uint32_t)st[BF_YH * BLOCK]) : 0u;
            const uint32_t yf2 = have_left ? pk_tag<TAG>((uint32_t)st[BF_YF * BLOCK]) : 0u;
            uint32_t Hin_prev = Dr;
            if (have_left && top >= 1) Hin_prev = pk_addu(Dr, top - 1 < prev_bot ? bnd[0].x : yh2);
            uint2 w = a.gtab[SEED_GTAB_PAD + top];
            uint2 bl = make_uint2(0u, 0u);
            if (have_left && top < prev_bot) bl = bnd[(size_t)1 * BLOCK];
            uint32_t uk = 0;
            uint32_t sbest = 0, snapD = 0;
            int srA = 0x7fffffff, srB = 0x7fffffff;
            uint32_t snap[MODE >= 2 ? C : 1];
            if (MODE >= 2) {
#pragma unroll
                for (int c = 0; c < C; ++c) snap[MODE >= 2 ? c : 0] = 0;
            }
            const M realA = mask_first<M>(nrA), realB = mask_first<M>(nrB);
            bool smA = false, smB = false;
#pragma unroll 1
            for (int r = top; r < bot; ++r) {
                const uint2 wn = a.gtab[SEED_GTAB_PAD + r + 1];
                const bool left = have_left && r < prev_bot;
                uint2 bln = make_uint2(0u, 0u);
                if (have_left && r + 1 < prev_bot) bln = bnd[(size_t)(r + 1 - top + 1) * BLOCK];
                Dr = pk_addu(Dr, ge2);
                const uint32_t Dn = pk_addu(Dr, ge2);
                const uint32_t Hin = pk_addu(Dr, left ? bl.x : yh2);
                uint32_t F = pk_addu(Dr, left ? bl.y : yf2);
                uint32_t hd = pk_addu(Hin_prev, __builtin_amdgcn_perm(w.y, w.x, sel[0]));
                Hin_prev = Hin;
                uint32_t rmax = 0x04000400u;
#pragma unroll
                for (int c = 0; c < C; ++c) {
                    uint32_t hd_next = 0;
                    if (c + 1 < C) hd_next = pk_addu(H[c], __builtin_amdgcn_perm(w.y, w.x, sel[c + 1 < C ? c + 1 : c]));
                    const uint32_t h = pk_max3(hd, E[c], F);
                    H[c] = h;
                    const uint32_t hg = h - gd2;
                    E[c] = pk_max3(E[c], hg, Dn);
                    F = pk_max3(F, hg, Dn) - ge2;
                    if (c & 1) rmax = pk_max3(rmax, H[c - (c & 1)], h);
                    else if (c == C - 1) rmax = pk_max3(rmax, h, h);
                    hd = hd_next;
                }
                const uint32_t tH = pk_subu(H[C - 1], Dr);
                if (has_next) {
                    if (r >= next_top - 1) bnd[(size_t)(r - (next_top - 1)) * BLOCK] = make_uint2(tH, pk_subu(F, Dr));
                    if (r < next_top) uk = pk_maxu(uk, tH);
                }
                const uint32_t tmax = pk_subu(rmax, Dr);
                if (MODE != 0) {
                    const uint32_t nsb = pk_maxu(sbest, tmax);
                    const uint32_t ch = nsb ^ sbest;
                    if (ch & 0xffffu) srA = r;
                    if (ch >> 16) srB = r;
                    if (MODE >= 2) {
                        const uint32_t m = ((ch & 0xffffu) ? 0xffffu : 0u) | ((ch >> 16) ? 0xffff0000u : 0u);
#pragma unroll
                        for (int c = 0; c < C; ++c) snap[MODE >= 2 ? c : 0] = (H[c] & m) | (snap[MODE >= 2 ? c : 0] & ~m);
                        snapD = (Dr & m) | (snapD & ~m);
                    }
                    if (MODE == 3) {
                        const uint32_t eq = tmax ^ nsb;
                        const bool tA = !(ch & 0xffffu) && !(eq & 0xffffu) && (nsb & 0xffffu) != 0;
                        const bool tB = !(ch >> 16) && !(eq >> 16) && (nsb >> 16) != 0;
                        if (ch & 0xffffu) smA = false;
                        if (ch >> 16) smB = false;
                        if (tA || tB) {
                            const uint32_t target = pk_addu(nsb, Dr);
                            M hitA = 0, hitB = 0;
#pragma unroll
                            for (int c = 0; c < C; ++c) {
                                const uint32_t x = H[c] ^ target;
                                if (!(x & 0xffffu)) hitA |= (M)1 << c;
                                if (!(x >> 16)) hitB |= (M)1 << c;
                            }
                            if (tA && (hitA & realA)) smA = true;
                            if (tB && (hitB & realB)) smB = true;
                        }
                    }
                    sbest = nsb;
                }
                best = pk_maxu(best, tmax);
                w = wn;
                bl = bln;
            }
            if (MODE != 0) {
                const int sA = (int)(sbest & 0xffffu), sB = (int)(sbest >> 16);
                const bool eqA = sA == bestA && sA > 0, eqB = sB == bestB && sB > 0;
                const bool upA = sA > bestA || (eqA && srA < rowA);
                const bool upB = sB > bestB || (eqB && srB < rowB);
                if (upA) {
                    bestA = sA;
                    rowA = srA;
                }
                if (upB) {
                    bestB = sB;
                    rowB = srB;
                }
                if (MODE >= 2 && (upA || upB || (MODE == 3 && (eqA || eqB)))) {
                    int cA = 0x7fffffff, cB = 0x7fffffff;
                    M hitA = 0, hitB = 0;
                    const int sdA = (int)(snapD & 0xffffu), sdB = (int)(snapD >> 16);
#pragma unroll
                    for (int c = C - 1; c >= 0; --c) {
                        const uint32_t sv = snap[MODE >= 2 ? c : 0];
                        if ((int)(sv & 0xffffu) - sdA == sA) {
                            cA = k * C + c;
                            hitA |= (M)1 << c;
                        }
                        if ((int)(sv >> 16) - sdB == sB) {
                            cB = k * C + c;
                            hitB |= (M)1 << c;
                        }
                    }
                    if (upA) colA = cA;
                    if (upB) colB = cB;
                    if (MODE == 3) {
                        const int nA = mask_popc(hitA & realA) + (smA ? 1 : 0), nB = mask_popc(hitB & realB) + (smB ? 1 : 0);
                        if (sA > 0 && (upA && !eqA)) multA = nA > 1;
                        else if (eqA && nA > 0) multA = true;
                        if (sB > 0 && (upB && !eqB)) multB = nB > 1;
                        else if (eqB && nB > 0) multB = true;
                    }
                }
            }
            const int xl = (k + 1) * C - 1;
            const BandLayout yA = band_layout(st, false), yB = band_layout(st, true);
            if (has_next && min(bot, next_top) > top) {
                const uint32_t joinA = xl < (int)lenA - 1 ? 0xffffu : 0u, joinB = xl < (int)lenB - 1 ? 0xffff0000u : 0u;
                const uint32_t freeA = seed_exit_is_free(xl, yA.m, yA.c0, yA.stride, a.sp.K, a.sp.spacer, yA.magic, yA.fa) ? 0xffffu : 0u;
                const uint32_t freeB = seed_exit_is_free(xl, yB.m, yB.c0, yB.stride, a.sp.K, a.sp.spacer, yB.magic, yB.fa) ? 0xffff0000u : 0u;
                const uint32_t ux = pk_addu(pk_untag<TAG>(uk), PKB2) & (joinA | joinB);
                st[BF_UP_FR * BLOCK] = (int)pk_maxu((uint32_t)st[BF_UP_FR * BLOCK], ux & (freeA | freeB));
                st[BF_UP_CH * BLOCK] = (int)pk_maxu((uint32_t)st[BF_UP_CH * BLOCK], ux & ~(freeA | freeB));
            }
            {
                const uint32_t below = bot < R ? 0xffffffffu : 0u, exits = (bot < R && bot > top) ? 0xffffffffu : 0u;
                const SeedStripEventsT<M> eA = seed_strip_events_t<M>(k * C, C, yA.m, yA.c0, yA.stride, a.sp.K, yA.magic, yA.fb);
                const SeedStripEventsT<M> eB = seed_strip_events_t<M>(k * C, C, yB.m, yB.c0, yB.stride, a.sp.K, yB.magic, yB.fb);
                const M any = eA.start | eA.end | eB.start | eB.end;
                BandPk lo;
                lo.ch = (uint32_t)st[BF_LO_CH * BLOCK];
                lo.fr = (uint32_t)st[BF_LO_FR * BLOCK];
                uint32_t ob2 = (uint32_t)st[BF_OB * BLOCK], b2 = 0;
                auto sweep = [&](auto full_tag) {
                    constexpr bool FULL = decltype(full_tag)::value;
                    const M realA = mask_first<M>(nrA), realB = mask_first<M>(nrB);
#pragma unroll
                    for (int c = 0; c < C; ++c) {
                        lo.ch += maxw2;
                        lo.fr += maxw2;
                        if (__ballot((uint32_t)(any >> c) & 1u) != 0) pk_events(&lo, half_mask(eA.start, eB.start, c), half_mask(eA.end, eB.end, c), lam2);
                        uint32_t he = pk_addu(pk_untag<TAG>(pk_subu(H[c], Dr)), PKB2) & exits;
                        uint32_t rm = 0xffffffffu;
                        if (!FULL) {
                            rm = half_mask(realA, realB, c);
                            he &= rm;
                        }
                        const uint32_t im = half_mask(eA.inside, eB.inside, c);
                        lo.fr = pk_maxu(lo.fr, he & im);
                        lo.ch = pk_maxu(lo.ch, he & ~im);
                        b2 = pk_subu_sat(pk_maxu(lo.ch, lo.fr), PKB2) & rm;
                        ob2 = pk_maxu(ob2, b2 & below);
                    }
                };
                if (all_full) sweep(std::true_type{});
                else sweep(std::false_type{});
                st[BF_LO_CH * BLOCK] = (int)lo.ch;
                st[BF_LO_FR * BLOCK] = (int)lo.fr;
                st[BF_OB * BLOCK] = (int)ob2;
                const uint32_t nm = ((nrA == C ? 0xffffu : 0u) | (nrB == C ? 0xffff0000u : 0u)) & below;
                st[BF_YH * BLOCK] = (int)(b2 & nm);
                st[BF_YF * BLOCK] = (int)(pk_subu_sat(pk_addu(b2, pk_subu_sat(lam2, maxw2)), go2p) & nm);
            }
            prev_bot = bot;
        }
        BandEnds ends;
        ends.rowA = rowA;
        ends.rowB = rowB;
        ends.colA = colA;
        ends.colB = colB;
        ends.multA = multA;
        ends.multB = multB;
        band_finish<MODE, MINS>(a, P, best, (uint32_t)st[BF_OA * BLOCK], (uint32_t)st[BF_OB * BLOCK], dtmin, dtmax, n_strips | (wu << 8) | (wd << 20), C, infoA, infoB, ends,
                                &n_accepted, &n_below);
        }
    }
    band_count_accepted(a, tid, n_accepted);
    if (MINS) band_count_below(a, tid, n_below);
}

constexpr int DIAG_D = SEED_NARROW_WU + SEED_NARROW_WD + 1 + SEED_DIAG_SLACK;

__device__ __forceinline__ uint32_t pk_bit_mask(uint32_t x, uint32_t sh) {
    const uint32_t top = __builtin_bit_cast(uint32_t, __builtin_bit_cast(us2, x) << __builtin_bit_cast(us2, sh));
    uint32_t m;
    asm("v_pk_ashrrev_i16 %0, 15, %1 op_sel_hi:[0,1]" : "=v"(m) : "v"(top));
    return m;
}
__device__ __forceinline__ uint32_t pair_mask(uint32_t x, int u) { return pk_bit_mask(x, (uint32_t)(15 - u) * 0x00010001u); }
__device__ __forceinline__ uint32_t lane_mask(uint32_t x, int u) { return (uint32_t)__builtin_amdgcn_sbfe((int)x, (uint32_t)u, 1u); }
__device__ __forceinline__ uint32_t pair_bits(uint32_t bitsA, uint32_t bitsB) { return (bitsA & 0xffffu) | (bitsB << 16); }

struct DiagGroupEvents {
    uint32_t upS, upE, freeb, loS, loE, loI;
};
__device__ __forceinline__ DiagGroupEvents diag_group_events(const SeedGroupPatterns& gA, const SeedGroupPatterns& gB, uint32_t fa2, uint32_t fb2) {
    DiagGroupEvents e;
    e.upS = e.upE = e.freeb = e.loS = e.loE = e.loI = 0;
#pragma unroll
    for (int t = 0; t < SEED_GROUP_KMERS; ++t) {
        const uint32_t sh = (uint32_t)((15 - gA.j0 - t) & 15) | ((uint32_t)((15 - gB.j0 - t) & 15) << 16);
        const uint32_t ma = pk_bit_mask(fa2, sh), mb = pk_bit_mask(fb2, sh);
        const uint32_t s = pair_bits(gA.start[t], gB.start[t]), en = pair_bits(gA.end[t], gB.end[t]);
        e.upS |= ma & s;
        e.upE |= ma & en;
        e.freeb |= ma & pair_bits(gA.terr[t], gB.terr[t]);
        e.loS |= mb & s;
        e.loE |= mb & en;
        e.loI |= mb & pair_bits(gA.inside[t], gB.inside[t]);
    }
    return e;
}

template <int D, bool UNI, bool MINS>
__global__ __launch_bounds__(BLOCK, 3) void seed_diag_kernel(SeedBandArgs a) {
    constexpr int TAG = -1;
    static_assert(D == 16, "a group of columns is two dwords of residue codes and 16 bits per read in the column masks");
    static_assert(D <= SEED_GROUP_MAX, "three k-mers per group (zsw_seed_diag.hpp)");
    static_assert(SEED_NARROW_WU_PER16 == 0 && SEED_NARROW_WD_PER32 == 0, "the window's height is fixed at compile time");
    __shared__ uint16_t sel_lut[16];
    __shared__ int sst[UNI ? 1 : BF_N * BLOCK];
    const int tid = threadIdx.x;
    int* const st = sst + (UNI ? 0 : tid);
    if (tid < 16) {
        const uint32_t k = (uint32_t)tid;
        sel_lut[tid] = (uint16_t)(k < 4 ? (2 * k + 1) | ((8 + k) << 8) : (k == 15 ? 0x0c00u : (2 * (k - 3)) | 0x0c00u));
    }
    __syncthreads();
    const int R = (int)a.ref_len;
    const uint32_t n_items = a.n_dev ? min(*a.n_dev, a.n) : a.n;
    const uint32_t n_pairs = (n_items + 1) / 2;
    const bool bail = a.bail_check && a.accepted && ((uint64_t)(*a.accepted) * SEED_BAIL_RATIO < (uint64_t)n_items || n_items < a.bail_below);
    uint32_t n_accepted = 0;
    uint32_t n_below = 0;
    const uint32_t ge2 = a.ge2, gd2 = a.gd2;
    const uint32_t ge1 = ge2 & 0xffffu;
    const uint32_t maxw2 = (uint32_t)a.sp.maxw * 0x00010001u, go2p = (uint32_t)a.sp.go * 0x00010001u;
    const int wu = a.wu0, wd = a.wd0;
    int um = 0, ustride = 0, uc0 = 0;
    uint32_t umagic = 0, ulam2 = 0;
    if (UNI) {
        seed_layout((int)a.b.fixed_len, a.sp.K, a.sp.spacer, &um, &ustride, &uc0);
        umagic = seed_div_magic(ustride);
        ulam2 = (uint32_t)seed_lambda(a.sp, ustride) * 0x00010001u;
    }
    const char* const gt = reinterpret_cast<const char*>(a.gtab + SEED_GTAB_PAD);
    const uint32_t row_end = (uint32_t)R * (uint32_t)sizeof(uint2);

    for (;;) {
        BandPair P;
        const int fetched = band_fetch(a, tid, n_items, n_pairs, bail, SEED_DIAG_SLACK, &P);
        if (fetched == 0) break;
        if (fetched == 2) {
        const uint32_t ridA = P.ridA, ridB = P.ridB;
        const bool validB = P.validB;
        const int lenA = UNI ? (int)a.b.fixed_len : (int)P.lenA, lenB = UNI ? (validB ? (int)a.b.fixed_len : 0) : (int)P.lenB;
        const int lenmax = UNI ? (int)a.b.fixed_len : max(lenA, lenB);
        const int dtmin = min(P.dtA, P.dtB), dtmax = max(P.dtA, P.dtB);
        const bool narrow = dtmax - dtmin < SEED_DIAG_SLACK;
        const uint32_t infoA = a.info[ridA], infoB = a.info[ridB];
        const uint32_t masksA = a.band_masks[ridA], masksB = validB ? a.band_masks[ridB] : 0u;
        const uint32_t fa2 = __builtin_amdgcn_perm(masksB, masksA, 0x05040100u), fb2 = __builtin_amdgcn_perm(masksB, masksA, 0x07060302u);
        uint32_t lam2 = ulam2;
        if (!UNI) {
            band_lane_init(a.sp, st, lenA, masksA, lenB, masksB);
            lam2 = (uint32_t)st[BF_LAM2 * BLOCK];
        }
        const uint32_t lamx = pk_subu_sat(lam2, maxw2);
        const uint32_t* codeA = a.codes + (size_t)ridA * a.cs;
        const uint32_t* codeB = a.codes + (size_t)ridB * a.cs;
        const int base = dtmin - wu;
        const auto table_row = [&](uint32_t off) { return *reinterpret_cast<const uint2*>(gt + min(off, row_end)); };
        uint2 w[D];
        uint32_t H[D], F[D];
        uint32_t Dc = (a.floor0 - ge1) * 0x00010001u;
#pragma unroll
        for (int j = 0; j < D; ++j) {
            w[j] = table_row((uint32_t)(base + j) * (uint32_t)sizeof(uint2));
            H[j] = Dc;
            F[j] = pk_addu(Dc, ge2);
        }
        uint32_t Fbelow = pk_addu(Dc, ge2);
        BandPk up, lo;
        up.ch = lo.ch = PKB2;
        up.fr = lo.fr = 0;
        uint32_t oa2 = 0, ob2 = 0, best = 0;
#pragma unroll 1
        for (int k0 = 0; k0 < lenmax; k0 += D) {
            uint32_t sel[D];
#pragma unroll
            for (int d = 0; d < D / 8; ++d) {
                const uint32_t di = (uint32_t)(k0 / 8 + d);
                const uint32_t wa = di < a.cs ? codeA[di] : 0xffffffffu;
                const uint32_t wb = (validB && di < a.cs) ? codeB[di] : 0xffffffffu;
#pragma unroll
                for (int j = 0; j < 8; ++j)
                    sel[8 * d + j] = (uint32_t)sel_lut[(wa >> (4 * j)) & 15u] | ((uint32_t)sel_lut[(wb >> (4 * j)) & 15u] << 16);
            }
            uint32_t upS, upE, loS, loE, loI, freeb, anyup, anylo, inj, join, ex, bel, nm, topin;
            {
                DiagGroupEvents ev;
                if (UNI) {
                    const SeedGroupPatterns g = seed_group_patterns(k0, D, um, uc0, ustride, a.sp.K, a.sp.spacer, umagic);
                    ev = diag_group_events(g, g, fa2, fb2);
                } else {
                    const BandLayout yA = band_layout(st, false), yB = band_layout(st, true);
                    ev = diag_group_events(seed_group_patterns(k0, D, yA.m, yA.c0, yA.stride, a.sp.K, a.sp.spacer, yA.magic),
                                           seed_group_patterns(k0, D, yB.m, yB.c0, yB.stride, a.sp.K, a.sp.spacer, yB.magic), fa2, fb2);
                }
                upS = ev.upS;
                upE = ev.upE;
                loS = ev.loS;
                loE = ev.loE;
                loI = ev.loI;
                freeb = ev.freeb;
                anyup = upS | upE;
                anyup |= anyup >> 16;
                anylo = loS | loE;
                anylo |= anylo >> 16;
                const int t0 = base + k0, t1 = dtmax + k0 + 1 + wd;
                const uint32_t above = seed_bits_from(1 - t0), below = seed_bits_below(R - t1);
                topin = seed_bits_from(-t0) & seed_bits_below(R - t0);
                const uint32_t exits = below & seed_bits_from(1 - t1), yfok = below & seed_bits_from(-t1);
                const uint32_t realA = seed_bits_below(lenA - k0), realB = seed_bits_below(lenB - k0);
                inj = pair_bits(realA & above, realB & above);
                join = pair_bits(seed_bits_below(lenA - k0 - 1) & topin, seed_bits_below(lenB - k0 - 1) & topin);
                ex = pair_bits(realA & exits, realB & exits);
                bel = pair_bits(realA & below, realB & below);
                nm = pair_bits(realA & yfok, realB & yfok);
            }
            const uint32_t enter = (uint32_t)(base + k0 + D) * (uint32_t)sizeof(uint2);
#pragma unroll
            for (int u = 0; u < D; ++u) {
                if (k0 + u < lenmax) {
                Dc = pk_addu(Dc, ge2);
                const uint32_t Dn = pk_addu(Dc, ge2);
                up.ch += maxw2;
                up.fr += maxw2;
                if (__ballot((anyup >> u) & 1u) != 0) pk_events(&up, pair_mask(upS, u), pair_mask(upE, u), lam2);
                const uint32_t v = pk_subu_sat(pk_maxu(up.ch, up.fr), PKB2) & pair_mask(inj, u);
                oa2 = pk_maxu(oa2, v);
                uint32_t E = pk_addu(Dc, pk_tag<TAG>(pk_subu_sat(v, go2p) & lane_mask(topin, u)));
                uint32_t rmax = 0x04000400u;
#pragma unroll
                for (int j = 0; j < D; ++j) {
                    const uint2 wr = w[(u + j) % D];
                    const uint32_t hd = pk_addu(H[j], __builtin_amdgcn_perm(wr.y, wr.x, sel[u]));
                    const uint32_t Fin = j + 1 < D ? F[j + 1 < D ? j + 1 : j] : Fbelow;
                    const uint32_t h = pk_max3(hd, E, Fin);
                    H[j] = h;
                    const uint32_t hg = h - gd2;
                    F[j] = pk_max3(Fin, hg, Dn);
                    E = pk_max3(E, hg, Dn) - ge2;
                    if (j == D - 1) rmax = pk_max3(rmax, H[j - 1], narrow ? 0u : h);
                    else if (j & 1) rmax = pk_max3(rmax, H[j - 1], h);
                    if (j == 0) w[u] = table_row(enter + (uint32_t)u * (uint32_t)sizeof(uint2));
                }
                best = pk_maxu(best, pk_subu(rmax, Dc));
                {
                    const uint32_t ux = pk_addu(pk_untag<TAG>(pk_subu(H[0], Dc)), PKB2) & pair_mask(join, u);
                    const uint32_t fm = pair_mask(freeb, u);
                    up.fr = pk_maxu(up.fr, ux & fm);
                    up.ch = pk_maxu(up.ch, ux & ~fm);
                }
                lo.ch += maxw2;
                lo.fr += maxw2;
                if (__ballot((anylo >> u) & 1u) != 0) pk_events(&lo, pair_mask(loS, u), pair_mask(loE, u), lam2);
                const uint32_t he = pk_addu(pk_untag<TAG>(pk_subu(narrow ? H[D - 2] : H[D - 1], Dc)), PKB2) & pair_mask(ex, u);
                const uint32_t im = pair_mask(loI, u);
                lo.fr = pk_maxu(lo.fr, he & im);
                lo.ch = pk_maxu(lo.ch, he & ~im);
                const uint32_t b2 = pk_subu_sat(pk_maxu(lo.ch, lo.fr), PKB2);
                ob2 = pk_maxu(ob2, b2 & pair_mask(bel, u));
                Fbelow = pk_addu(Dn, pk_tag<TAG>(pk_subu_sat(pk_addu(b2, lamx), go2p) & pair_mask(nm, u)));
                if (narrow) F[D - 1] = Fbelow;
                }
            }
        }
        band_finish<0, MINS>(a, P, best, oa2, ob2, dtmin, dtmax, lenmax | (wu << 8) | (wd << 20), 1, infoA, infoB, BandEnds{}, &n_accepted, &n_below);
        }
    }
    band_count_accepted(a, tid, n_accepted);
    if (MINS) band_count_below(a, tid, n_below);
}

}

uint32_t seed_band_rows(const SeedParams& p, uint32_t max_len) { return (uint32_t)seed_rows_above(p, (int)max_len) + (uint32_t)seed_rows_below(p, (int)max_len) + SEED_BAND_SLACK + 4; }

uint32_t seed_band_grid(uint32_t n, uint32_t grid_cap) {
    const uint32_t pairs = (n + 1) / 2;
    return std::max<uint32_t>(1, std::min<uint32_t>((pairs + BLOCK - 1) / BLOCK, std::min(grid_cap, SEED_BAND_MAX_GRID)));
}

size_t seed_band_buffer_bytes(const SeedParams& p, uint32_t n, uint32_t max_len, uint32_t grid_cap) {
    return n ? (size_t)seed_band_grid(n, grid_cap) * BLOCK * (size_t)seed_band_rows(p, max_len) * sizeof(uint2) : 0;
}

constexpr int BC = BC_WIDE;
bool seed_band_applicable(const SeedParams& p, uint32_t max_len, uint32_t rebase_rows, uint32_t limit) {
    static_assert(SEED_NARROW_WU >= SEED_DN && SEED_NARROW_WD >= SEED_DM, "the band must hold the diagonals that count as near the anchor");
    if (p.M1 < p.Dn || p.Wd < p.Dm) return false;
    if (2ull * (uint64_t)p.maxw * max_len + 8 >= limit || (uint64_t)p.maxw * (max_len + BC) >= 0x2000u) return false;
    return (uint32_t)BC + seed_band_rows(p, max_len) + 2 <= rebase_rows;
}

bool seed_diag_applicable(uint32_t max_len, uint32_t rebase_rows) {
    return max_len <= SEED_DIAG_MAX_LEN && max_len + 2 <= rebase_rows;
}

template <bool MINS>
static hipError_t launch_seed_band_t(const SeedBandArgs& a, int mode, bool narrow_strips, hipStream_t stream, bool diagonal) {
    if (diagonal) {
        if (mode != 0 || !narrow_strips || a.wu_per16 != 0 || a.wd_per32 != 0 || a.wu0 + a.wd0 + 1 + SEED_DIAG_SLACK != DIAG_D) return hipErrorInvalidValue;
        if (a.sp.K + a.sp.spacer < SEED_GROUP_MIN_STRIDE || a.ref_len >= (1u << 24)) return hipErrorInvalidValue;
        if (a.b.offsets == nullptr && !a.diag_lane_events) hipLaunchKernelGGL((seed_diag_kernel<DIAG_D, true, MINS>), dim3(a.grid), dim3(BLOCK), 0, stream, a);
        else hipLaunchKernelGGL((seed_diag_kernel<DIAG_D, false, MINS>), dim3(a.grid), dim3(BLOCK), 0, stream, a);
        return hipGetLastError();
    }
    if (narrow_strips) {
        if (mode == 0) hipLaunchKernelGGL((seed_band_kernel<BC_NARROW, 4, 0, MINS>), dim3(a.grid), dim3(BLOCK), 0, stream, a);
        else if (mode == 1) hipLaunchKernelGGL((seed_band_kernel<BC_NARROW, 4, 1, MINS>), dim3(a.grid), dim3(BLOCK), 0, stream, a);
        else if (mode == 2) hipLaunchKernelGGL((seed_band_kernel<BC_NARROW, 3, 2, MINS>), dim3(a.grid), dim3(BLOCK), 0, stream, a);
        else hipLaunchKernelGGL((seed_band_kernel<BC_NARROW, 3, 3, MINS>), dim3(a.grid), dim3(BLOCK), 0, stream, a);
    } else {
        if (mode == 0) hipLaunchKernelGGL((seed_band_kernel<BC_WIDE, 2, 0, MINS>), dim3(a.grid), dim3(BLOCK), 0, stream, a);
        else if (mode == 1) hipLaunchKernelGGL((seed_band_kernel<BC_WIDE, 1, 1, MINS>), dim3(a.grid), dim3(BLOCK), 0, stream, a);
        else if (mode == 2) hipLaunchKernelGGL((seed_band_kernel<BC_WIDE, 1, 2, MINS>), dim3(a.grid), dim3(BLOCK), 0, stream, a);
        else hipLaunchKernelGGL((seed_band_kernel<BC_WIDE, 1, 3, MINS>), dim3(a.grid), dim3(BLOCK), 0, stream, a);
    }
    return hipGetLastError();
}

hipError_t launch_seed_band(const SeedBandArgs& a, int mode, bool narrow_strips, hipStream_t stream, bool diagonal) {
    if (a.min_thr && a.min_count) return launch_seed_band_t<true>(a, mode, narrow_strips, stream, diagonal);
    return launch_seed_band_t<false>(a, mode, narrow_strips, stream, diagonal);
}

}
```

zoe_amd/csrc/zsw_score_seed.hip:

```cpp
#include <hipcub/hipcub.hpp>

#include <algorithm>
#include <vector>

#include "zsw_score_seed.hpp"
#include "zsw_score_v2.hpp"
#include "zsw_timer.hpp"

namespace zsw {

namespace {

struct SeedArgs {
    BatchDev b;
    const ScoringDev* sc;
    SeedParams sp;
    const uint2* table;
    uint32_t first, n;
    uint32_t* keys;
    uint32_t* ids;
    uint32_t* info;
    uint32_t* masks;
    uint32_t* band_masks;
    uint8_t* band_dfb;
    uint32_t* codes;
    uint32_t cs;
    uint32_t key_bias, fail_key;
    uint32_t ref_len;
    uint32_t* fail_list;
    uint32_t* fail_count;
    bool reversed;
    uint32_t min_thr;
    ScoreOut out;
    uint32_t* min_count;
};

constexpr uint32_t SEED_STAGE_LEN = 160;

template <bool STAGED, bool MINS>
__global__ __launch_bounds__(256) void seed_kernel(SeedArgs a) {
    __shared__ uint16_t cell_lut[256];
    __shared__ __attribute__((aligned(16))) uint8_t sbytes[STAGED ? 256 * SEED_STAGE_LEN + 16 : 16];
    {
        const int res = (int)a.sc->index_map[threadIdx.x];
        const uint32_t cellv = seed_cell(a.sp, res);
        cell_lut[threadIdx.x] = (uint16_t)((cellv & 0xffu) | (((cellv >> 8) == 0xffu ? 0xfu : ((cellv >> 8) & 3u)) << 8) | ((uint32_t)(res & 15) << 12));
    }
    const uint32_t k = blockIdx.x * 256 + threadIdx.x;
    const bool valid = k < a.n;
    uint32_t id = 0, len = 0;
    uint64_t off = 0;
    if (valid) {
        id = a.b.items ? a.b.items[a.first + k] : a.first + k;
        off = a.b.offsets ? a.b.offsets[id] : (uint64_t)id * a.b.fixed_len;
        len = a.b.offsets ? (uint32_t)(a.b.offsets[id + 1] - off) : a.b.fixed_len;
    }
    if (STAGED) {
        const uint32_t L = a.b.fixed_len;
        const uint64_t b0 = (uint64_t)(a.first + blockIdx.x * 256u) * L;
        const uint32_t cnt = min(256u, a.n - blockIdx.x * 256u) * L;
        const uint8_t* src = a.b.bases + b0;
        const uint32_t head = (uint32_t)((16u - (uint32_t)(reinterpret_cast<uintptr_t>(src) & 15u)) & 15u);
        const uint32_t shift = (16u - head) & 15u;
        for (uint32_t i = threadIdx.x; i < min(head, cnt); i += 256) sbytes[shift + i] = src[i];
        const uint32_t n16 = cnt > head ? (cnt - head) / 16 : 0;
        for (uint32_t i = threadIdx.x; i < n16; i += 256)
            *reinterpret_cast<uint4*>(&sbytes[shift + head + 16 * i]) = *reinterpret_cast<const uint4*>(src + head + 16 * i);
        for (uint32_t i = head + 16 * n16 + threadIdx.x; i < cnt; i += 256) sbytes[shift + i] = src[i];
        __syncthreads();
        off = (uint64_t)shift + (uint64_t)threadIdx.x * L;
    } else {
        __syncthreads();
    }
    SeedRead sr;
    sr.ok = 0;
    sr.t_all = sr.d_fa = sr.d_bl = 0;
    sr.bl_mask = 0;
    if (valid && len >= SEED_MIN_LEN && len < SEED_KEY_BIAS) {
        const uint8_t* bases = STAGED ? sbytes + off : a.b.bases + off;
        const bool rev = a.reversed;
        const uint2* table = a.table;
        uint32_t* code_out = a.codes ? a.codes + (size_t)k * a.cs : nullptr;
        uint32_t acc = 0;
        sr = seed_read<MINS>(
            a.sp, (int)len,
            [&](int c) {
                const uint32_t v = cell_lut[bases[rev ? (int)len - 1 - c : c]];
                if (code_out) {
                    acc |= (v >> 12) << (4 * (c & 7));
                    if ((c & 7) == 7) {
                        code_out[c >> 3] = acc;
                        acc = 0;
                    }
                }
                return (v & 0xffu) | (((v >> 8) & 0xfu) == 0xfu ? 0xff00u : (v & 0x300u));
            },
            [&](uint32_t code, uint32_t* f1, uint32_t* l1) {
                const uint2 e = table[code];
                *f1 = e.x;
                *l1 = e.y;
            });
    }
    bool below = false;
    if (MINS && valid && len > 0 && len < SEED_KEY_BIAS) {
        int bound = sr.u_whole;
        if (len < SEED_MIN_LEN) {
            const uint8_t* bases = STAGED ? sbytes + off : a.b.bases + off;
            bound = 0;
            for (uint32_t c = 0; c < len; ++c) bound += (int)(cell_lut[bases[c]] & 0xffu);
        }
        below = seed_below_min(bound, a.min_thr);
        if (below) {
            a.out.score[id] = 0;
            a.out.status[id] = ZSW_STATUS_BELOW_MIN_SCORE;
            if (a.out.tier) a.out.tier[id] = 0;
            if (a.out.ref_end) a.out.ref_end[id] = 0;
            if (a.out.query_end) a.out.query_end[id] = 0;
        }
    }
    if (MINS) {
        const unsigned long long mb = __ballot(below);
        if (mb && (threadIdx.x & 63) == 0) atomicAdd(a.min_count, (uint32_t)__popcll(mb));
    }
    const bool fail = valid && !sr.ok && !below;
    if (valid) {
        a.keys[k] = (sr.ok && !below) ? (uint32_t)(sr.dt + (int)a.key_bias) : a.fail_key;
        a.ids[k] = k;
        a.info[k] = (uint32_t)sr.t_all | ((uint32_t)sr.d_fa << 16) | ((uint32_t)sr.d_bl << 24);
        a.masks[k] = sr.bl_mask;
        if (a.codes) {
            a.band_masks[k] = sr.fa_mask | (sr.fb_mask << 16);
            a.band_dfb[k] = (uint8_t)sr.d_fb;
            uint32_t* code_row = a.codes + (size_t)k * a.cs;
            const bool swept = len >= SEED_MIN_LEN && len < SEED_KEY_BIAS;
            const uint32_t full = swept ? len >> 3 : 0;
            if (full < a.cs) {
                uint32_t tail = 0xffffffffu;
                if (swept && (len & 7u)) {
                    const uint8_t* bases = STAGED ? sbytes + off : a.b.bases + off;
                    tail = 0;
                    for (uint32_t c = full * 8; c < full * 8 + 8; ++c)
                        tail |= (c < len ? (uint32_t)(cell_lut[bases[a.reversed ? len - 1 - c : c]] >> 12) : 15u) << (4 * (c & 7));
                }
                code_row[full] = tail;
                for (uint32_t d = full + 1; d < a.cs; ++d) code_row[d] = 0xffffffffu;
            }
        }
    }
    const unsigned long long m = __ballot(fail);
    if (m) {
        const int lane = threadIdx.x & 63;
        const int leader = __ffsll((long long)m) - 1;
        uint32_t base = 0;
        if (lane == leader) base = atomicAdd(a.fail_count, (uint32_t)__popcll(m));
        base = (uint32_t)__shfl((int)base, leader, 64);
        if (fail) a.fail_list[base + (uint32_t)__popcll(m & ((1ull << lane) - 1ull))] = id;
    }
}

__global__ void seed_gtab_kernel(const uint8_t* ref, uint32_t ref_len, const ScoringDev* sc, ScoreArgsV2 a, uint2* gtab) {
    const uint32_t i = blockIdx.x * blockDim.x + threadIdx.x;
    if (i >= ref_len + 2 * SEED_GTAB_PAD) return;
    const int row = (int)i - SEED_GTAB_PAD;
    const int idx = (row >= 0 && row < (int)ref_len) ? (int)sc->index_map[ref[row]] : NEUTRAL;
    gtab[i] = make_uint2(a.wtab[idx][0], a.wtab[idx][1]);
}

size_t round256(size_t x) { return (x + 255) & ~(size_t)255; }

size_t sort_temp_bytes(uint32_t n) {
    size_t bytes = 0, sel = 0;
    (void)hipcub::DeviceRadixSort::SortPairs(nullptr, bytes, (const uint32_t*)nullptr, (uint32_t*)nullptr, (const uint32_t*)nullptr,
                                             (uint32_t*)nullptr, (int)n, 0, 32, (hipStream_t)0);
    (void)hipcub::DeviceSelect::Flagged(nullptr, sel, (const uint32_t*)nullptr, (const uint8_t*)nullptr, (uint32_t*)nullptr, (uint32_t*)nullptr,
                                        (int)n, (hipStream_t)0);
    return std::max(bytes, sel);
}

}

uint32_t seed_codes_stride(uint32_t max_len) { return (max_len + 7) / 8 + 1; }

size_t seed_workspace_bytes(uint32_t n, uint32_t max_len, uint32_t band_grid_cap) {
    SeedParams p{};
    p.M1 = SEED_M1;
    p.M1_per8 = SEED_M1_PER8;
    p.Wd = SEED_WD;
    p.Wd_per16 = SEED_WD_PER16;
    return 7 * round256((size_t)n * 4 + 8) + round256((size_t)n + 8) + round256((size_t)n * seed_codes_stride(max_len) * 4 + 8) +
           round256(sort_temp_bytes(n)) + round256(seed_band_buffer_bytes(p, n, max_len, band_grid_cap)) + 256;
}

bool seed_applicable(const SeedIndex& ix, uint32_t max_len, uint32_t ref_len, uint32_t limit) {
    if (!ix.valid || !ix.usable || !ix.d_table || ref_len == 0 || ref_len >= (1u << 24)) return false;
    if (max_len < SEED_MIN_LEN || max_len > SEED_MAX_LEN) return false;
    return (uint64_t)ix.params.maxw * max_len + 8 < limit;
}

hipError_t launch_score_seeded(const ScoreArgsV2& a2, int G, int C, uint32_t max_len, const SeedIndex& ix, uint8_t* work, size_t work_bytes,
                               uint2* gtab, uint32_t* fail_list, uint32_t* fail_count, int mode, const ScoreArgsV2* band_tabs, const uint2* gtab_band, int32_t* band_dbg,
                               uint32_t narrow_min_reads, uint32_t band_grid_cap, hipStream_t stream, KernelTimer* window_timer, bool narrow_only, bool reads_reversed,
                               std::vector<uint32_t>* launches, bool strip_first_tier, bool diag_lane_events, uint32_t min_thr, uint32_t* min_counts) {
    const uint32_t n = a2.b.n_items;
    if (!min_counts) min_thr = 0;
    if (n == 0) return hipSuccess;
    if (!work || !gtab || work_bytes < seed_workspace_bytes(n, max_len, band_grid_cap)) return hipErrorNotSupported;
    const bool band = band_tabs != nullptr && gtab_band != nullptr && seed_band_applicable(ix.params, max_len, band_tabs->K, band_tabs->limit);
    const size_t per = round256((size_t)n * 4 + 8);
    uint32_t* keys = reinterpret_cast<uint32_t*>(work);
    uint32_t* keys_out = reinterpret_cast<uint32_t*>(work + per);
    uint32_t* ids = reinterpret_cast<uint32_t*>(work + 2 * per);
    uint32_t* order = reinterpret_cast<uint32_t*>(work + 3 * per);
    uint32_t* info = reinterpret_cast<uint32_t*>(work + 4 * per);
    uint32_t* masks = reinterpret_cast<uint32_t*>(work + 5 * per);
    uint32_t* band_masks = reinterpret_cast<uint32_t*>(work + 6 * per);
    uint8_t* p8 = work + 7 * per;
    uint8_t* band_dfb = p8;
    p8 += round256((size_t)n + 8);
    const uint32_t cs = seed_codes_stride(max_len);
    uint32_t* codes = reinterpret_cast<uint32_t*>(p8);
    p8 += round256((size_t)n * cs * 4 + 8);
    void* temp = p8;
    p8 += round256(sort_temp_bytes(n));
    uint2* band_buf = reinterpret_cast<uint2*>(p8);
    size_t temp_bytes = sort_temp_bytes(n);
    int key_bits = 1;
    while ((1ull << key_bits) < (uint64_t)a2.ref_len + 2ull * SEED_KEY_BIAS + 2 && key_bits < 32) ++key_bits;
    const uint32_t fail_key = key_bits >= 32 ? 0xffffffffu : (1u << key_bits) - 1u;

    SeedArgs s;
    s.b = a2.b;
    s.sc = a2.sc;
    s.sp = ix.params;
    s.table = reinterpret_cast<const uint2*>(ix.d_table);
    s.first = 0;
    s.n = n;
    s.keys = keys;
    s.ids = ids;
    s.info = info;
    s.masks = masks;
    s.band_masks = band_masks;
    s.band_dfb = band_dfb;
    s.codes = band ? codes : nullptr;
    s.cs = cs;
    s.key_bias = SEED_KEY_BIAS;
    s.fail_key = fail_key;
    s.ref_len = a2.ref_len;
    s.fail_list = fail_list;
    s.fail_count = fail_count;
    s.reversed = reads_reversed;
    s.min_thr = min_thr;
    s.out = a2.out;
    s.min_count = min_counts;
    const bool staged = !s.b.offsets && !s.b.items && s.b.fixed_len <= SEED_STAGE_LEN;
    if (min_thr) {
        if (staged) hipLaunchKernelGGL((seed_kernel<true, true>), dim3((n + 255) / 256), dim3(256), 0, stream, s);
        else hipLaunchKernelGGL((seed_kernel<false, true>), dim3((n + 255) / 256), dim3(256), 0, stream, s);
    } else if (staged)
        hipLaunchKernelGGL((seed_kernel<true, false>), dim3((n + 255) / 256), dim3(256), 0, stream, s);
    else
        hipLaunchKernelGGL((seed_kernel<false, false>), dim3((n + 255) / 256), dim3(256), 0, stream, s);
    hipError_t e = hipcub::DeviceRadixSort::SortPairs(temp, temp_bytes, (const uint32_t*)keys, keys_out, (const uint32_t*)ids, order, (int)n, 0,
                                                      key_bits, stream);
    if (e != hipSuccess) return e;

    if (band) {
        SeedBandArgs b;
        b.b = a2.b;
        b.ref_len = a2.ref_len;
        b.ge2 = band_tabs->ge2;
        b.gd2 = band_tabs->gd2;
        b.floor0 = band_tabs->floor0;
        b.rule = a2.rule;
        b.out = a2.out;
        b.sp = ix.params;
        b.n = n;
        b.order = order;
        b.keys = keys;
        b.info = info;
        b.band_masks = band_masks;
        b.band_dfb = band_dfb;
        b.codes = codes;
        b.cs = cs;
        b.gtab = gtab_band;
        b.bnd = band_buf;
        b.dbg = band_dbg;
        b.nb = seed_band_rows(ix.params, max_len);
        b.grid = seed_band_grid(n, band_grid_cap);
        b.key_bias = SEED_KEY_BIAS;
        b.fail_key = fail_key;
        b.fail_list = fail_list;
        b.fail_count = fail_count;
        b.wu0 = ix.params.M1;
        b.wu_per16 = 2 * ix.params.M1_per8;
        b.wd0 = ix.params.Wd;
        b.wd_per32 = 2 * ix.params.Wd_per16;
        b.n_dev = nullptr;
        b.retry = nullptr;
        b.min_thr = min_thr;
        b.min_count = min_counts ? min_counts + 1 : nullptr;
        uint32_t* queue1 = reinterpret_cast<uint32_t*>(work + 3 * per + (size_t)n * 4) + 1;
        uint32_t* queue2 = reinterpret_cast<uint32_t*>(work + (size_t)n * 4);
        e = hipMemsetAsync(queue1, 0, 4, stream);
        if (e != hipSuccess) return e;
        e = hipMemsetAsync(queue2, 0, 8, stream);
        if (e != hipSuccess) return e;
        uint32_t* accepted = queue2 + 1;
        b.next_pair = queue2;
        if (window_timer) window_timer->begin(stream);
        if (max_len <= SEED_NARROW_MAX_LEN && n >= narrow_min_reads) {
            uint8_t* retry = reinterpret_cast<uint8_t*>(ids);
            uint32_t* order2 = keys_out;
            uint32_t* n2 = reinterpret_cast<uint32_t*>(work + 3 * per + (size_t)n * 4);
            e = hipMemsetAsync(retry, 0, n, stream);
            if (e != hipSuccess) return e;
            SeedBandArgs b1 = b;
            b1.wu0 = SEED_NARROW_WU;
            b1.wu_per16 = SEED_NARROW_WU_PER16;
            b1.wd0 = SEED_NARROW_WD;
            b1.wd_per32 = SEED_NARROW_WD_PER32;
            b1.retry = narrow_only ? nullptr : retry;
            b1.accepted = narrow_only ? nullptr : accepted;
            b1.next_pair = queue1;
            b1.diag_lane_events = diag_lane_events;
            note_launch(launches, ZSW_LAUNCH_SEED_BAND, G, C, mode);
            const bool diagonal = mode == 0 && !narrow_only && !strip_first_tier && seed_diag_applicable(max_len, band_tabs->K);
            e = launch_seed_band(b1, mode, true, stream, diagonal);
            if (e != hipSuccess) return e;
            if (narrow_only) {
                if (window_timer) window_timer->end(stream);
                return hipSuccess;
            }
            e = hipcub::DeviceSelect::Flagged(temp, temp_bytes, (const uint32_t*)order, (const uint8_t*)retry, order2, n2, (int)n, stream);
            if (e != hipSuccess) return e;
            b.order = order2;
            b.n_dev = n2;
            b.wu0 = SEED_SECOND_WU;
            b.wu_per16 = SEED_SECOND_WU_PER16;
            b.wd0 = SEED_SECOND_WD;
            b.wd_per32 = SEED_SECOND_WD_PER32;
            b.accepted = accepted;
            b.bail_check = true;
            b.bail_below = band_dbg ? 0u : SEED_BAIL_BELOW;
        }
        note_launch(launches, ZSW_LAUNCH_SEED_BAND, G, C, mode);
        e = launch_seed_band(b, mode, false, stream);
        if (window_timer) window_timer->end(stream);
        return e;
    }
    SeedWindowArgs w;
    w.b = a2.b;
    w.ref = a2.ref;
    w.ref_len = a2.ref_len;
    w.sc = a2.sc;
    for (int r = 0; r < 9; ++r) {
        w.wtab[r][0] = a2.wtab[r][0];
        w.wtab[r][1] = a2.wtab[r][1];
    }
    w.ge2 = a2.ge2;
    w.gd2 = a2.gd2;
    w.floor0 = a2.floor0;
    w.K = a2.K;
    w.rule = a2.rule;
    w.out = a2.out;
    w.sp = ix.params;
    w.first = 0;
    w.n = n;
    w.order = order;
    w.keys = keys;
    w.info = info;
    w.masks = masks;
    w.gtab = gtab;
    w.key_bias = SEED_KEY_BIAS;
    w.fail_key = fail_key;
    w.fail_list = fail_list;
    w.fail_count = fail_count;
    w.reversed = reads_reversed;
    if (window_timer) window_timer->begin(stream);
    note_launch(launches, ZSW_LAUNCH_SEED_WINDOW, G, C, std::min(mode, 2));
    e = mode == 0 ? launch_seed_window_m0(w, G, C, stream) : mode == 1 ? launch_seed_window_m1(w, G, C, stream) : launch_seed_window_m2(w, G, C, stream);
    if (window_timer) window_timer->end(stream);
    return e;
}

hipError_t seed_build_gtab(const ScoreArgsV2& a2, uint2* gtab, hipStream_t stream) {
    hipLaunchKernelGGL(seed_gtab_kernel, dim3((a2.ref_len + 2 * SEED_GTAB_PAD + 255) / 256), dim3(256), 0, stream, a2.ref, a2.ref_len, a2.sc, a2, gtab);
    return hipGetLastError();
}

hipError_t seed_index_update(SeedIndex* ix, const ScoringDev& sc, const uint8_t* h_ref, size_t ref_len) {
    ix->valid = true;
    ix->usable = false;
    if (ref_len == 0 || ref_len >= (size_t(1) << 24)) return hipSuccess;
    std::vector<uint8_t> res(ref_len);
    bool ref_has[32] = {false};
    for (size_t i = 0; i < ref_len; ++i) {
        res[i] = sc.index_map[h_ref[i]];
        ref_has[res[i] & 31] = true;
    }
    const int K = seed_k_for(ref_len);
    SeedParams p{};
    if (sc.S > 7 || !seed_analyze(sc.S, sc.w, sc.gap_open, sc.gap_extend, ref_has, K, &p)) return hipSuccess;
    p.M1 = SEED_M1;
    p.M1_per8 = SEED_M1_PER8;
    p.M2 = SEED_M2;
    p.Dn = SEED_DN;
    p.Dm = SEED_DM;
    p.Wd = SEED_WD;
    p.Wd_per16 = SEED_WD_PER16;
    p.tol = SEED_TOL;
    const size_t entries = size_t(1) << (2 * K);
    std::vector<uint32_t> table(2 * entries, 0u);
    seed_index_build(p, res.data(), ref_len, table.data());
    const size_t bytes = table.size() * sizeof(uint32_t);
    if (bytes > ix->table_bytes) {
        if (ix->d_table) (void)hipFree(ix->d_table);
        ix->d_table = nullptr;
        ix->table_bytes = 0;
        hipError_t e = hipMalloc(reinterpret_cast<void**>(&ix->d_table), bytes);
        if (e != hipSuccess) {
            (void)hipGetLastError();
            return hipSuccess;
        }
        ix->table_bytes = bytes;
    }
    hipError_t e = hipMemcpy(ix->d_table, table.data(), bytes, hipMemcpyHostToDevice);
    if (e != hipSuccess) return e;
    ix->params = p;
    ix->usable = true;
    return hipSuccess;
}

void seed_index_release(SeedIndex* ix) {
    if (ix->d_table) (void)hipFree(ix->d_table);
    ix->d_table = nullptr;
    ix->table_bytes = 0;
    ix->valid = false;
    ix->usable = false;
}

}
```

zoe_amd/csrc/zsw_score_seed.hpp:

```cpp
#pragma once
#include "zsw_internal.hpp"
#include "zsw_seed.hpp"

namespace zsw {

constexpr int SEED_M1 = 24;
constexpr int SEED_M1_PER8 = 1;
constexpr int SEED_M2 = 16;
constexpr int SEED_DN = 4;
constexpr int SEED_TOL = 8;
constexpr int SEED_DM = 4;
constexpr int SEED_WD = 9;
constexpr int SEED_WD_PER16 = 1;
constexpr int SEED_NARROW_WU = 8, SEED_NARROW_WU_PER16 = 0, SEED_NARROW_WD = 6, SEED_NARROW_WD_PER32 = 0;
constexpr uint32_t SEED_BAIL_RATIO = 40;
constexpr uint32_t SEED_BAIL_BELOW = 16384;
constexpr int SEED_SECOND_WU = 16, SEED_SECOND_WU_PER16 = 1, SEED_SECOND_WD = 8, SEED_SECOND_WD_PER32 = 1;
constexpr uint32_t SEED_NARROW_MAX_LEN = 640;
constexpr uint32_t SEED_NARROW_MIN_READS = 200000;
constexpr int SEED_BAND_SLACK = 32;
constexpr int SEED_DIAG_SLACK = 1;
constexpr uint32_t SEED_DIAG_MAX_LEN = 255;
constexpr uint32_t SEED_BAND_MAX_GRID = 1024;
constexpr uint32_t SEED_KEY_BIAS = 1u << 16;
constexpr uint32_t SEED_MAX_LEN = 2432;
constexpr uint32_t SEED_MIN_LEN = 24;
constexpr int SEED_GTAB_PAD = 128;
constexpr uint32_t SEED_MIN_READS = 1024;

struct SeedIndex {
    bool valid = false;
    bool usable = false;
    SeedParams params{};
    uint32_t* d_table = nullptr;
    size_t table_bytes = 0;
};

struct SeedWindowArgs {
    BatchDev b;
    const uint8_t* ref;
    uint32_t ref_len;
    const ScoringDev* sc;
    uint32_t wtab[9][2];
    uint32_t ge2, gd2, floor0, K;
    ResultRule rule;
    ScoreOut out;
    SeedParams sp;
    uint32_t first;
    uint32_t n;
    const uint32_t* order;
    const uint32_t* keys;
    const uint32_t* info;
    const uint32_t* masks;
    const uint2* gtab;
    uint32_t key_bias, fail_key;
    uint32_t* fail_list;
    uint32_t* fail_count;
    bool reversed = false;
};

struct SeedBandArgs {
    BatchDev b;
    uint32_t ref_len;
    uint32_t ge2, gd2, floor0;
    ResultRule rule;
    ScoreOut out;
    SeedParams sp;
    uint32_t n;
    const uint32_t* order;
    const uint32_t* keys;
    const uint32_t* info;
    const uint32_t* band_masks;
    const uint8_t* band_dfb;
    const uint32_t* codes;
    uint32_t cs;
    const uint2* gtab;
    uint2* bnd;
    uint32_t nb;
    uint32_t grid;
    int wu0, wu_per16, wd0, wd_per32;
    const uint32_t* n_dev;
    uint32_t* next_pair;
    uint8_t* retry;
    uint32_t* accepted = nullptr;
    bool bail_check = false;
    uint32_t bail_below = 0;
    bool diag_lane_events = false;
    int* dbg;
    uint32_t key_bias, fail_key;
    uint32_t* fail_list;
    uint32_t* fail_count;
    uint32_t min_thr = 0;
    uint32_t* min_count = nullptr;
};
uint32_t seed_band_rows(const SeedParams& p, uint32_t max_len);
uint32_t seed_band_grid(uint32_t n, uint32_t grid_cap);
size_t seed_band_buffer_bytes(const SeedParams& p, uint32_t n, uint32_t max_len, uint32_t grid_cap);
bool seed_band_applicable(const SeedParams& p, uint32_t max_len, uint32_t rebase_rows, uint32_t limit);
hipError_t launch_seed_band(const SeedBandArgs& a, int mode, bool narrow_strips, hipStream_t stream, bool diagonal = false);
bool seed_diag_applicable(uint32_t max_len, uint32_t rebase_rows);

struct ScoreArgsV2;

constexpr uint32_t SEED_BAND_CLASS_MIN_GRID = 64;
inline uint32_t seed_band_class_cap(uint32_t n_class, uint32_t n_total) {
    return SEED_BAND_CLASS_MIN_GRID + (uint32_t)((uint64_t)SEED_BAND_MAX_GRID * n_class / (n_total ? n_total : 1));
}
size_t seed_workspace_bytes(uint32_t n, uint32_t max_len, uint32_t band_grid_cap = SEED_BAND_MAX_GRID);
bool seed_applicable(const SeedIndex& ix, uint32_t max_len, uint32_t ref_len, uint32_t limit);
hipError_t seed_build_gtab(const ScoreArgsV2& a2, uint2* gtab, hipStream_t stream);
hipError_t launch_score_seeded(const ScoreArgsV2& a2, int G, int C, uint32_t max_len, const SeedIndex& ix, uint8_t* work, size_t work_bytes,
                               uint2* gtab, uint32_t* fail_list, uint32_t* fail_count, int mode, const ScoreArgsV2* band_tabs, const uint2* gtab_band, int32_t* band_dbg,
                               uint32_t narrow_min_reads, uint32_t band_grid_cap, hipStream_t stream, KernelTimer* window_timer, bool narrow_only = false, bool reads_reversed = false,
                               std::vector<uint32_t>* launches = nullptr , bool strip_first_tier = false ,
                               bool diag_lane_events = false ,
                               uint32_t min_thr = 0 , uint32_t* min_counts = nullptr );
hipError_t seed_index_update(SeedIndex* ix, const ScoringDev& sc, const uint8_t* h_ref, size_t ref_len);
void seed_index_release(SeedIndex* ix);

hipError_t launch_seed_window_m0(const SeedWindowArgs& a, int G, int C, hipStream_t stream);
hipError_t launch_seed_window_m1(const SeedWindowArgs& a, int G, int C, hipStream_t stream);
hipError_t launch_seed_window_m2(const SeedWindowArgs& a, int G, int C, hipStream_t stream);

}
```

zoe_amd/csrc/zsw_score_v2.hpp:

```cpp
#pragma once
#include "zsw_internal.hpp"

namespace zsw {

constexpr int BLOCK = 256;
constexpr int CH = 2048;
constexpr int NEUTRAL = 8;
constexpr int PAD_K = 255;

#define ZSW_FOR_EACH_STRIP_CONFIG(X)                                                                                            \
    X(4, 19) X(4, 22) X(4, 25) X(4, 28) X(4, 32) X(4, 35) X(4, 38) X(8, 19) X(8, 22) X(8, 25) X(8, 28) X(8, 32) X(8, 35) X(8, 38) \
    X(16, 22) X(16, 25) X(16, 32) X(16, 38) X(64, 19) X(64, 38) X(32, 5)
constexpr int WIDE_STRIDE = 36;
constexpr int WIDE_PAD = 32, WIDE_NEUTRAL = 32;

constexpr int min_waves(int C, int MODE) {
    const int need = (MODE == 2 ? 4 * C : 3 * C) + (MODE == 2 ? 44 : 36);
    return need <= 80 ? 6 : need <= 96 ? 5 : need <= 128 ? 4 : need <= 168 ? 3 : 2;
}

typedef _Float16 h2 __attribute__((ext_vector_type(2)));
typedef unsigned short us2 __attribute__((ext_vector_type(2)));
__device__ __forceinline__ uint32_t pk_max3(uint32_t a, uint32_t b, uint32_t c) {
    return __builtin_bit_cast(uint32_t, __builtin_elementwise_maximum(__builtin_elementwise_maximum(__builtin_bit_cast(h2, a), __builtin_bit_cast(h2, b)),
                                                                       __builtin_bit_cast(h2, c)));
}
__device__ __forceinline__ uint32_t pk_addu(uint32_t a, uint32_t b) { return __builtin_bit_cast(uint32_t, __builtin_bit_cast(us2, a) + __builtin_bit_cast(us2, b)); }
__device__ __forceinline__ uint32_t pk_subu(uint32_t a, uint32_t b) { return __builtin_bit_cast(uint32_t, __builtin_bit_cast(us2, a) - __builtin_bit_cast(us2, b)); }
__device__ __forceinline__ uint32_t pk_maxu(uint32_t a, uint32_t b) {
    return __builtin_bit_cast(uint32_t, __builtin_elementwise_max(__builtin_bit_cast(us2, a), __builtin_bit_cast(us2, b)));
}

struct ScoreArgsV2 {
    BatchDev b;
    const uint8_t* ref;
    uint32_t ref_len;
    const ScoringDev* sc;
    uint32_t wtab[9][2];
    int8_t wide[33 * 36];
    uint32_t ge2, gd2;
    uint32_t floor0;
    uint32_t K;
    uint32_t limit;
    ResultRule rule;
    ScoreOut out;
    uint32_t tile_q0;
    const uint2* tile_in;
    uint2* tile_out;
    uint4* tile_state;
    const uint32_t* rev_ref_end;
    const uint32_t* rev_query_end;
    const uint32_t* n_items_dev = nullptr;
    uint32_t gate_lo = 0, gate_hi = 0xffffffffu;
    uint32_t chunk_rows = 0, chunk_overlap = 0;
    unsigned long long* chunk_keys = nullptr;
};

constexpr uint32_t CHUNK_ROW_BITS = 24, CHUNK_COL_BITS = 12;
__host__ __device__ inline unsigned long long chunk_key(uint32_t score, uint32_t row1, uint32_t col1) {
    return ((unsigned long long)score << (CHUNK_ROW_BITS + CHUNK_COL_BITS)) | ((unsigned long long)(((1u << CHUNK_ROW_BITS) - 1u) - row1) << CHUNK_COL_BITS) |
           (unsigned long long)(((1u << CHUNK_COL_BITS) - 1u) - col1);
}

template <int G, int C, int MODE, bool WIDE = false, bool TILED = false>
__global__ __launch_bounds__(BLOCK, min_waves(C, MODE)) void score_kernel_v2(ScoreArgsV2 a) {
    __shared__ uint2 rp[WIDE ? 1 : CH + G];
    __shared__ uint16_t rpw[WIDE ? CH + G : 1];
    __shared__ uint32_t wt32[WIDE ? 33 * 9 : 1];
    __shared__ uint2 swt[9];
    __shared__ uint32_t lut32[64];
    const uint8_t* lut = reinterpret_cast<const uint8_t*>(lut32);

    const int tid = threadIdx.x;
    const int g = tid & (G - 1);
    const uint32_t group = blockIdx.x * (BLOCK / G) + tid / G;
    const uint32_t itemA = 2 * group, itemB = 2 * group + 1;
    const uint32_t n_items = a.n_items_dev ? min(*a.n_items_dev, a.b.n_items) : a.b.n_items;
    if (2 * blockIdx.x * (BLOCK / G) >= n_items || n_items < a.gate_lo || n_items >= a.gate_hi) return;
    const bool validA = itemA < n_items, validB = itemB < n_items;
    const uint32_t idA = validA ? (a.b.items ? a.b.items[itemA] : itemA) : 0;
    const uint32_t idB = validB ? (a.b.items ? a.b.items[itemB] : itemB) : 0;

    if (tid < 64) lut32[tid] = reinterpret_cast<const uint32_t*>(a.sc->index_map)[tid];
    if (tid < 9) swt[tid] = make_uint2(a.wtab[tid][0], a.wtab[tid][1]);
    if (WIDE) {
        for (int i = tid; i < 33 * 9; i += BLOCK) wt32[WIDE ? i : 0] = reinterpret_cast<const uint32_t*>(a.wide)[i];
    }
    __syncthreads();
    const int8_t* wt = reinterpret_cast<const int8_t*>(wt32);

    uint64_t offA = 0, offB = 0;
    uint32_t lenA = 0, lenB = 0;
    if (validA) {
        if (a.b.offsets) {
            offA = a.b.offsets[idA];
            lenA = (uint32_t)(a.b.offsets[idA + 1] - offA);
        } else {
            offA = (uint64_t)idA * a.b.fixed_len;
            lenA = a.b.fixed_len;
        }
    }
    if (validB) {
        if (a.b.offsets) {
            offB = a.b.offsets[idB];
            lenB = (uint32_t)(a.b.offsets[idB + 1] - offB);
        } else {
            offB = (uint64_t)idB * a.b.fixed_len;
            lenB = a.b.fixed_len;
        }
    }

    uint32_t sel[C];
#pragma unroll
    for (int c = 0; c < C; ++c) {
        const uint32_t q = (TILED ? a.tile_q0 : 0u) + (uint32_t)(g * C + c);
        uint32_t kA = PAD_K, kB = PAD_K;
        if (q < lenA) kA = lut[a.b.bases[offA + q]];
        if (q < lenB) kB = lut[a.b.bases[offB + q]];
        if (WIDE) {
            sel[c] = (kA == PAD_K ? (uint32_t)WIDE_PAD : kA) | ((kB == PAD_K ? (uint32_t)WIDE_PAD : kB) << 16);
        } else {
            const uint32_t sA = kA < 4 ? (2 * kA + 1) | ((8 + kA) << 8) : (kA == PAD_K ? 0x0c00u : (2 * (kA - 3)) | 0x0c00u);
            const uint32_t sB = kB < 4 ? (2 * kB + 1) | ((8 + kB) << 8) : (kB == PAD_K ? 0x0c00u : (2 * (kB - 3)) | 0x0c00u);
            sel[c] = sA | (sB << 16);
        }
    }

    const uint32_t ge2 = a.ge2, gd2 = a.gd2;
    const uint32_t ge1 = ge2 & 0xffffu;
    const uint32_t K = a.K;
    const uint32_t Kge2 = (K * ge1) * 0x00010001u;
    uint32_t Dr = (a.floor0 - (uint32_t)(g + 1) * ge1) * 0x00010001u;
    uint32_t H[C], E[C];
    uint32_t snap[MODE == 2 ? C : 1];
#pragma unroll
    for (int c = 0; c < C; ++c) {
        H[c] = Dr;
        E[c] = pk_addu(Dr, ge2);
    }
    if (MODE == 2) {
#pragma unroll
        for (int c = 0; c < C; ++c) snap[MODE == 2 ? c : 0] = 0;
    }
    uint32_t snapD = 0;
    uint32_t best = 0;
    uint32_t Fout = Dr, Hlast = Dr, Hin_prev = Dr;
    int rA = 0, rB = 0;
    int row_off = 0, R = (int)a.ref_len;
    if (!TILED && a.chunk_rows) {
        const int lo = max(0, (int)(blockIdx.y * a.chunk_rows) - (int)a.chunk_overlap), hi = min(R, (int)((blockIdx.y + 1) * a.chunk_rows));
        row_off = lo;
        R = max(hi - lo, 0);
    }
    const uint8_t* const refp = a.ref + row_off;
    const int T = R + G - 1;
    uint2 bd = make_uint2(0u, 0u);
    if (TILED) {
        if (g == 0 && validA && a.tile_in != nullptr && R > 0) bd = a.tile_in[(size_t)group * (size_t)R];
    }

    for (int base = 0; base < T; base += CH) {
        __syncthreads();
        for (int j = tid; j < CH + G - 1; j += BLOCK) {
            const int row = base - (G - 1) + j;
            if (WIDE) {
                int idx = WIDE_NEUTRAL;
                if (row >= 0 && row < R) idx = lut[refp[row]];
                rpw[WIDE ? j : 0] = (uint16_t)(idx * WIDE_STRIDE);
            } else {
                int idx = NEUTRAL;
                if (row >= 0 && row < R) idx = lut[refp[row]];
                rp[WIDE ? 0 : j] = swt[idx];
            }
        }
        __syncthreads();
        const int tend = (T < base + CH) ? T : base + CH;
        const int joff = (G - 1 - g) - base;
        uint2 w = WIDE ? make_uint2(rpw[WIDE ? base + joff : 0], 0) : rp[WIDE ? 0 : base + joff];
        auto lookup = [&](const uint2 ww, const uint32_t sl) -> uint32_t {
            if constexpr (WIDE) {
                const int sa = wt[ww.x + (sl & 0xffffu)], sb = wt[ww.x + (sl >> 16)];
                return __builtin_amdgcn_perm((uint32_t)sb, (uint32_t)sa, 0x05040100u);
            } else {
                return __builtin_amdgcn_perm(ww.y, ww.x, sl);
            }
        };
#pragma unroll 1
        for (int t = base; t < tend; ++t) {
            const uint2 wn = WIDE ? make_uint2(rpw[WIDE ? t + 1 + joff : 0], 0) : rp[WIDE ? 0 : t + 1 + joff];
            const int row = t - g;
            const bool rebase = ge1 != 0 && row > 0 && (row & (int)(K - 1)) == 0;
            if (__ballot(rebase) != 0) {
                const uint32_t adj = rebase ? Kge2 : 0u;
#pragma unroll
                for (int c = 0; c < C; ++c) {
                    H[c] = pk_subu(H[c], adj);
                    E[c] = pk_subu(E[c], adj);
                }
                Hin_prev = pk_subu(Hin_prev, adj);
                Dr = pk_subu(Dr, adj);
            }
            Dr = pk_addu(Dr, ge2);
            const uint32_t Dn = pk_addu(Dr, ge2);
            uint32_t Fin = (uint32_t)__shfl_up((int)Fout, 1, G);
            uint32_t Hin = (uint32_t)__shfl_up((int)Hlast, 1, G);
            if (g == 0) {
                Fin = Dr;
                Hin = Dr;
                if (TILED) {
                    if (validA && a.tile_in != nullptr && row >= 0 && row < R) {
                        Hin = bd.x;
                        Fin = bd.y;
                    }
                    if (validA && a.tile_in != nullptr && row + 1 < R) bd = a.tile_in[(size_t)group * (size_t)R + (size_t)(row + 1)];
                }
            }
            uint32_t hd = pk_addu(Hin_prev, lookup(w, sel[0]));
            Hin_prev = Hin;
            uint32_t F = Fin;
            uint32_t rmax = 0x04000400u;
#pragma unroll
            for (int c = 0; c < C; ++c) {
                uint32_t hd_next = 0;
                if (c + 1 < C) hd_next = pk_addu(H[c], lookup(w, sel[c + 1 < C ? c + 1 : c]));
                const uint32_t h = pk_max3(hd, E[c], F);
                H[c] = h;
                const uint32_t hg = h - gd2;
                E[c] = pk_max3(E[c], hg, Dn);
                F = pk_max3(F, hg, Dn) - ge2;
                if (c & 1) rmax = pk_max3(rmax, H[c - (c & 1)], h);
                else if (c == C - 1) rmax = pk_max3(rmax, h, h);
                hd = hd_next;
            }
            Fout = F;
            Hlast = H[C - 1];
            if (TILED) {
                if (g == G - 1 && validA && a.tile_out != nullptr && row >= 0 && row < R)
                    a.tile_out[(size_t)group * (size_t)R + (size_t)row] = make_uint2(Hlast, Fout);
            }
            const uint32_t tmax = pk_subu(rmax, Dr);
            const uint32_t nb = pk_maxu(best, tmax);
            if (MODE != 0) {
                const uint32_t ch = nb ^ best;
                if (ch & 0xffffu) rA = row;
                if (ch >> 16) rB = row;
                if (MODE == 2) {
                    const uint32_t m = ((ch & 0xffffu) ? 0xffffu : 0u) | ((ch >> 16) ? 0xffff0000u : 0u);
#pragma unroll
                    for (int c = 0; c < C; ++c) snap[MODE == 2 ? c : 0] = (H[c] & m) | (snap[MODE == 2 ? c : 0] & ~m);
                    snapD = (Dr & m) | (snapD & ~m);
                }
            }
            best = nb;
            w = wn;
        }
    }

    int bA = (int)(best & 0xffffu), bB = (int)(best >> 16);
    int gbA = bA, gbB = bB;
#pragma unroll
    for (int d = 1; d < G; d <<= 1) {
        gbA = max(gbA, __shfl_xor(gbA, d, G));
        gbB = max(gbB, __shfl_xor(gbB, d, G));
    }
    uint32_t reA = 0, reB = 0, qeA = 0, qeB = 0;
    if (MODE != 0) {
        int kA = (bA == gbA) ? rA : 0x7fffffff, kB = (bB == gbB) ? rB : 0x7fffffff;
#pragma unroll
        for (int d = 1; d < G; d <<= 1) {
            kA = min(kA, __shfl_xor(kA, d, G));
            kB = min(kB, __shfl_xor(kB, d, G));
        }
        reA = (uint32_t)kA + 1;
        reB = (uint32_t)kB + 1;
        if (MODE == 2) {
            int cA = 0x7fffffff, cB = 0x7fffffff;
            const int dA = (int)(snapD & 0xffffu), dB = (int)(snapD >> 16);
#pragma unroll
            for (int c = C - 1; c >= 0; --c) {
                const uint32_t sv = snap[MODE == 2 ? c : 0];
                if ((int)(sv & 0xffffu) - dA == gbA) cA = (TILED ? (int)a.tile_q0 : 0) + g * C + c;
                if ((int)(sv >> 16) - dB == gbB) cB = (TILED ? (int)a.tile_q0 : 0) + g * C + c;
            }
            if (!(bA == gbA && rA == kA)) cA = 0x7fffffff;
            if (!(bB == gbB && rB == kB)) cB = 0x7fffffff;
#pragma unroll
            for (int d = 1; d < G; d <<= 1) {
                cA = min(cA, __shfl_xor(cA, d, G));
                cB = min(cB, __shfl_xor(cB, d, G));
            }
            qeA = (uint32_t)cA + 1;
            qeB = (uint32_t)cB + 1;
        }
    }

    const int lane = tid & 63;
    constexpr int RW = 2 * (64 / G);
    const int src = (lane >> 1) * G;
    const bool hi = lane & 1;
    auto pick = [&](int va, int vb) {
        const int xa = __shfl(va, src, 64), xb = __shfl(vb, src, 64);
        return hi ? xb : xa;
    };
    const uint32_t o_valid = (uint32_t)pick((int)validA, (int)validB);
    const uint32_t o_id = (uint32_t)pick((int)idA, (int)idB);
    const uint32_t o_len = (uint32_t)pick((int)lenA, (int)lenB);
    int o_true = pick(gbA, gbB);
    uint32_t o_re = (uint32_t)pick((int)reA, (int)reB);
    uint32_t o_qe = (uint32_t)pick((int)qeA, (int)qeB);
    if (TILED) {
        if (lane < RW && o_valid) {
            uint32_t best_u = (uint32_t)o_true >= a.limit ? 0xffffffffu : (uint32_t)o_true;
            if (a.tile_in != nullptr) {
                const uint4 prev = a.tile_state[o_id];
                const bool keep_prev = prev.x == 0xffffffffu || (best_u != 0xffffffffu && (prev.x > best_u || (prev.x == best_u && prev.y <= o_re)));
                if (keep_prev) {
                    best_u = prev.x;
                    o_re = prev.y;
                    o_qe = prev.z;
                }
            }
            if (a.tile_out != nullptr) a.tile_state[o_id] = make_uint4(best_u, o_re, o_qe, 0u);
            o_true = best_u == 0xffffffffu ? 0x7fffffff : (int)best_u;
        }
        if (a.tile_out != nullptr) return;
    }
    if (!TILED && a.chunk_rows) {
        if (lane < RW && o_valid && o_len != 0 && o_true > 0)
            atomicMax(&a.chunk_keys[o_id], chunk_key((uint32_t)min(o_true, 0xffff), MODE != 0 ? o_re + (uint32_t)row_off : 0u, MODE == 2 ? o_qe : 0u));
        return;
    }
    if (lane < RW && o_valid) {
        if (o_len == 0) {
            a.out.score[o_id] = 0;
            a.out.status[o_id] = ZSW_STATUS_EMPTY;
            if (a.out.tier) a.out.tier[o_id] = 0;
            if (MODE != 0 && a.out.ref_end) a.out.ref_end[o_id] = 0;
            if (MODE == 2 && a.out.query_end) a.out.query_end[o_id] = 0;
        } else if ((uint32_t)o_true >= a.limit) {
            const uint32_t k = atomicAdd(a.out.fb_count, 1u);
            a.out.fb_list[k] = o_id;
        } else {
            uint32_t score;
            uint8_t status, tier;
            apply_rule(a.rule, (uint64_t)o_true, &score, &status, &tier);
            a.out.score[o_id] = score;
            a.out.status[o_id] = status;
            if (a.out.tier) a.out.tier[o_id] = tier;
            const bool some = status == ZSW_STATUS_SOME;
            if (MODE != 0 && a.out.ref_end) a.out.ref_end[o_id] = some ? o_re : 0;
            if (MODE == 2 && a.out.query_end) a.out.query_end[o_id] = some ? o_qe : 0;
        }
    }
}

hipError_t launch_table_cfg_v2_wide(const ScoreArgsV2& a, int G, int C, int mode, hipStream_t stream);
constexpr int TILE_G = 64, TILE_C = 38, TILE_COLS = TILE_G * TILE_C;
hipError_t launch_tile_v2(const ScoreArgsV2& a, bool wide, int mode, hipStream_t stream);
hipError_t launch_tile_w32(const ScoreArgsV2& a, const uint32_t* list, int mode, hipStream_t stream);

}
```

Before: 654.4 million.

## Co-schedule handback scoring blocks with the seeded diagonal band kernel

Adds a co-scheduling path for mode-0 seeded scoring: when the diagonal band kernel runs with G=4 and two tiers, extra blocks in the same launch score the reads the seed stage hands back, instead of leaving them for a separate later kernel. The seed-diag body moves into an include file so it can be shared by the combined kernel. Per-pass first-item counters (n0) let the follow-up exact pass skip items already handled. This removes a serial kernel boundary and the tail idle time between the stages. In exchange it adds more block-role logic and counter bookkeeping, and a debug flag allows turning it off.

```diff
diff --git a/include/zoe_sw.h b/include/zoe_sw.h
--- a/include/zoe_sw.h
+++ b/include/zoe_sw.h
@@ -214,7 +214,8 @@
     ZSW_DEBUG_RANGES_EXACT_REVERSE = 16384,
     ZSW_DEBUG_ALIGN_NO_CERTIFICATE = 32768,
     ZSW_DEBUG_SEED_STRIP_FIRST_TIER = 65536,
-    ZSW_DEBUG_SEED_DIAG_LANE_EVENTS = 131072
+    ZSW_DEBUG_SEED_DIAG_LANE_EVENTS = 131072,
+    ZSW_DEBUG_SEED_NO_COSCHEDULE = 262144
 } zsw_debug_flag;
 zsw_error zsw_debug_set(zsw_context* ctx, uint32_t flags);
 
diff --git a/zoe_amd/_lib.py b/zoe_amd/_lib.py
--- a/zoe_amd/_lib.py
+++ b/zoe_amd/_lib.py
@@ -27,6 +27,7 @@
 DEBUG_ALIGN_NO_CERTIFICATE = 32768
 DEBUG_SEED_STRIP_FIRST_TIER = 65536
 DEBUG_SEED_DIAG_LANE_EVENTS = 131072
+DEBUG_SEED_NO_COSCHEDULE = 262144
 (LAUNCH_V1_FAST, LAUNCH_V1_BIASED, LAUNCH_V2, LAUNCH_WIDE, LAUNCH_V1_FAST_REV, LAUNCH_V1_BIASED_REV, LAUNCH_WIDE_REV, LAUNCH_TILE_V2, LAUNCH_TILE_WIDE,
  LAUNCH_TILE_W32, LAUNCH_EXACT32, LAUNCH_EXACT32_WORKLIST, LAUNCH_SEED_WINDOW, LAUNCH_SEED_BAND, LAUNCH_PRUNED) = range(15)
 OPTION_EXACT_PRUNING = 1
diff --git a/zoe_amd/build.py b/zoe_amd/build.py
--- a/zoe_amd/build.py
+++ b/zoe_amd/build.py
@@ -9,7 +9,7 @@
 CSRC = os.path.join(HERE, "csrc")
 LIB = os.path.join(HERE, "libzoe_sw_hip.so")
 SOURCES = ["zsw_capi.hip", "zsw_capi_shared.hip", "zsw_shared.hip", "zsw_score.hip", "zsw_align.hip", "zsw_align_pk8.hip", "zsw_align_pk16.hip", "zsw_align_pk32.hip", "zsw_align_pk64.hip", "zsw_group.hip", "zsw_threepass.hip", "zsw_filter.hip", "zsw_score_wide.hip", "zsw_score_w32.hip", "zsw_score_prune.hip", "zsw_score_seed.hip", "zsw_score_seed_m0.hip", "zsw_score_seed_m1.hip", "zsw_score_seed_m2.hip", "zsw_score_band.hip", "zsw_multi.hip", "zsw_strand.hip"]
-HEADERS = ["zsw_internal.hpp", "zsw_align_dev.hpp", "zsw_align_pk.hpp", "zsw_align_pk_kernel.hpp", "zsw_score_v1.hpp", "zsw_score_v2.hpp", "zsw_handback.hpp", "zsw_score_prune.hpp", "zsw_seed.hpp", "zsw_seed_diag.hpp", "zsw_cert.hpp", "zsw_context.hpp", "zsw_shared.hpp", "zsw_score_seed.hpp", "zsw_score_seed_kernel.hpp", "zsw_align.hpp", "zsw_timer.hpp", "zsw_strand.hpp", "zsw_synth.h", "zsw_exports.map", os.path.join("..", "..", "include", "zoe_sw.h")]
+HEADERS = ["zsw_internal.hpp", "zsw_align_dev.hpp", "zsw_align_pk.hpp", "zsw_align_pk_kernel.hpp", "zsw_score_v1.hpp", "zsw_score_v2.hpp", "zsw_handback.hpp", "zsw_score_prune.hpp", "zsw_seed.hpp", "zsw_seed_diag.hpp", "zsw_seed_diag_body.inc", "zsw_cert.hpp", "zsw_context.hpp", "zsw_shared.hpp", "zsw_score_seed.hpp", "zsw_score_seed_kernel.hpp", "zsw_align.hpp", "zsw_timer.hpp", "zsw_strand.hpp", "zsw_synth.h", "zsw_exports.map", os.path.join("..", "..", "include", "zoe_sw.h")]
 ARCH = "gfx950"
 EXTRA_FLAGS = {}
 
diff --git a/zoe_amd/csrc/zsw_handback.hpp b/zoe_amd/csrc/zsw_handback.hpp
--- a/zoe_amd/csrc/zsw_handback.hpp
+++ b/zoe_amd/csrc/zsw_handback.hpp
@@ -65,4 +65,36 @@
     return n;
 }
 
+struct CoscheduleCase {
+    int mode;
+    bool two_tiers;
+    bool diagonal;
+    int G;
+    bool mins;
+    bool row_chunks;
+    bool skip_handed_back;
+    bool disabled;
+};
+constexpr bool handback_coschedule(const CoscheduleCase& c) {
+    return c.mode == 0 && c.two_tiers && c.diagonal && c.G == 4 && !c.mins && !c.row_chunks && !c.skip_handed_back && !c.disabled;
 }
+
+constexpr uint32_t HANDBACK_BLOCK_THREADS = 256;
+constexpr uint32_t handback_block_pairs(int G) { return HANDBACK_BLOCK_THREADS / (uint32_t)G; }
+constexpr uint32_t handback_blocks(uint32_t n_items, int G) { return (n_items + 2 * handback_block_pairs(G) - 1) / (2 * handback_block_pairs(G)); }
+struct CoscheduleRole {
+    bool handback;
+    uint32_t index;
+};
+constexpr CoscheduleRole coschedule_role(uint32_t block, uint32_t hb_blocks) {
+    return block < hb_blocks ? CoscheduleRole{true, block} : CoscheduleRole{false, block - hb_blocks};
+}
+struct PairRange {
+    uint32_t first, end;
+};
+constexpr PairRange handback_block_range(uint32_t block, int G, uint32_t count) {
+    const uint64_t pairs = ((uint64_t)count + 1) / 2, lo = (uint64_t)block * handback_block_pairs(G), hi = lo + handback_block_pairs(G);
+    return lo >= pairs ? PairRange{0u, 0u} : PairRange{(uint32_t)lo, (uint32_t)(hi < pairs ? hi : pairs)};
+}
+
+}
diff --git a/zoe_amd/csrc/zsw_score.hip b/zoe_amd/csrc/zsw_score.hip
--- a/zoe_amd/csrc/zsw_score.hip
+++ b/zoe_amd/csrc/zsw_score.hip
@@ -561,22 +561,35 @@
         pe = hipMemsetAsync(counter, 0, 4, stream);
         if (pe != hipSuccess) return pe;
         ap.b = bb;
+        int maxw = 0;
+        for (int i = 0; i < h_sc.S * h_sc.S; ++i) maxw = std::max(maxw, (int)h_sc.w[i]);
+        const uint64_t overlap = h_sc.gap_extend > 0 ? (uint64_t)longest + (uint64_t)longest * (uint64_t)maxw / (uint64_t)h_sc.gap_extend + 2 : ~0ull;
+        const uint64_t rows = std::max<uint64_t>(4 * overlap, 2048);
+        const bool row_chunks = ws.chunk_keys && !(ws.debug & ZSW_DEBUG_NO_ROW_CHUNKS) && h_sc.gap_extend > 0 && rows * 2 <= ref_len && longest < (1u << CHUNK_COL_BITS) &&
+                                ref_len < (1u << CHUNK_ROW_BITS) - 2;
+        const uint32_t min_thr = (ws.min_score && ws.min_counts && !out.skip_handed_back) ? min_threshold(rule, ws.min_score) : 0u;
+        CoscheduleCase co{};
+        co.mode = mode;
+        co.G = g;
+        co.mins = min_thr != 0;
+        co.row_chunks = row_chunks;
+        co.skip_handed_back = out.skip_handed_back;
+        co.disabled = (ws.debug & ZSW_DEBUG_SEED_NO_COSCHEDULE) != 0;
+        uint32_t* const n0 = counter + 32;
+        static_assert(2 + NCLS <= 32, "the n0 words sit 32 behind their counters");
+        bool coscheduled = false;
         pe = launch_score_seeded(ap, g, c, longest, *ws.seed, ws.seed_work + work_off, seed_workspace_bytes(bb.n_items, longest, band_grid_cap), ws.seed_gtab,
                                  ws.prune_fail_list + list_off, counter, mode, band_ok ? &ab : nullptr, gtab_band, ws.band_dbg,
                                  (ws.debug & ZSW_DEBUG_SEED_WIDE_BAND) ? 0xffffffffu : (ws.debug & ZSW_DEBUG_SCORE_PRUNE_ANY_SIZE) ? 0u : SEED_NARROW_MIN_READS, band_grid_cap, stream,
                                  ws.window_timer, out.narrow_only, out.reads_reversed && out.skip_handed_back, launches,
                                  (ws.debug & ZSW_DEBUG_SEED_STRIP_FIRST_TIER) != 0, (ws.debug & ZSW_DEBUG_SEED_DIAG_LANE_EVENTS) != 0,
-                                 (ws.min_score && ws.min_counts && !out.skip_handed_back) ? min_threshold(rule, ws.min_score) : 0u, ws.min_counts);
+                                 min_thr, ws.min_counts, &co, n0, &coscheduled);
         if (pe != hipSuccess) return pe;
         ap.b.items = ws.prune_fail_list + list_off;
         ap.n_items_dev = counter;
+        ap.first_item_dev = coscheduled ? n0 : nullptr;
         if (!out.skip_handed_back) {
-            int maxw = 0;
-            for (int i = 0; i < h_sc.S * h_sc.S; ++i) maxw = std::max(maxw, (int)h_sc.w[i]);
-            const uint64_t overlap = h_sc.gap_extend > 0 ? (uint64_t)longest + (uint64_t)longest * (uint64_t)maxw / (uint64_t)h_sc.gap_extend + 2 : ~0ull;
-            const uint64_t rows = std::max<uint64_t>(4 * overlap, 2048);
-            if (ws.chunk_keys && !(ws.debug & ZSW_DEBUG_NO_ROW_CHUNKS) && h_sc.gap_extend > 0 && rows * 2 <= ref_len && longest < (1u << CHUNK_COL_BITS) &&
-                ref_len < (1u << CHUNK_ROW_BITS) - 2) {
+            if (row_chunks) {
                 ap.chunk_rows = (uint32_t)rows;
                 ap.chunk_overlap = (uint32_t)overlap;
                 ap.chunk_keys = ws.chunk_keys;
@@ -603,6 +616,7 @@
                         ah = tabs[t++];
                         ah.b = ap.b;
                         ah.n_items_dev = counter;
+                        ah.first_item_dev = ap.first_item_dev;
                     }
                     ah.b.n_items = plan[k].grid_items;
                     ah.gate_lo = plan[k].lo;
diff --git a/zoe_amd/csrc/zsw_score_band.hip b/zoe_amd/csrc/zsw_score_band.hip
--- a/zoe_amd/csrc/zsw_score_band.hip
+++ b/zoe_amd/csrc/zsw_score_band.hip
@@ -1,6 +1,7 @@
 #include <algorithm>
 #include <type_traits>
 
+#include "zsw_handback.hpp"
 #include "zsw_score_seed.hpp"
 #include "zsw_seed_diag.hpp"
 #include "zsw_score_v2.hpp"
@@ -545,176 +546,56 @@
 
 template <int D, bool UNI, bool MINS>
 __global__ __launch_bounds__(BLOCK, 3) void seed_diag_kernel(SeedBandArgs a) {
-    constexpr int TAG = -1;
-    static_assert(D == 16, "a group of columns is two dwords of residue codes and 16 bits per read in the column masks");
-    static_assert(D <= SEED_GROUP_MAX, "three k-mers per group (zsw_seed_diag.hpp)");
-    static_assert(SEED_NARROW_WU_PER16 == 0 && SEED_NARROW_WD_PER32 == 0, "the window's height is fixed at compile time");
-    __shared__ uint16_t sel_lut[16];
-    __shared__ int sst[UNI ? 1 : BF_N * BLOCK];
-    const int tid = threadIdx.x;
-    int* const st = sst + (UNI ? 0 : tid);
-    if (tid < 16) {
-        const uint32_t k = (uint32_t)tid;
-        sel_lut[tid] = (uint16_t)(k < 4 ? (2 * k + 1) | ((8 + k) << 8) : (k == 15 ? 0x0c00u : (2 * (k - 3)) | 0x0c00u));
-    }
-    __syncthreads();
-    const int R = (int)a.ref_len;
-    const uint32_t n_items = a.n_dev ? min(*a.n_dev, a.n) : a.n;
-    const uint32_t n_pairs = (n_items + 1) / 2;
-    const bool bail = a.bail_check && a.accepted && ((uint64_t)(*a.accepted) * SEED_BAIL_RATIO < (uint64_t)n_items || n_items < a.bail_below);
-    uint32_t n_accepted = 0;
-    uint32_t n_below = 0;
-    const uint32_t ge2 = a.ge2, gd2 = a.gd2;
-    const uint32_t ge1 = ge2 & 0xffffu;
-    const uint32_t maxw2 = (uint32_t)a.sp.maxw * 0x00010001u, go2p = (uint32_t)a.sp.go * 0x00010001u;
-    const int wu = a.wu0, wd = a.wd0;
-    int um = 0, ustride = 0, uc0 = 0;
-    uint32_t umagic = 0, ulam2 = 0;
-    if (UNI) {
-        seed_layout((int)a.b.fixed_len, a.sp.K, a.sp.spacer, &um, &ustride, &uc0);
-        umagic = seed_div_magic(ustride);
-        ulam2 = (uint32_t)seed_lambda(a.sp, ustride) * 0x00010001u;
-    }
-    const char* const gt = reinterpret_cast<const char*>(a.gtab + SEED_GTAB_PAD);
-    const uint32_t row_end = (uint32_t)R * (uint32_t)sizeof(uint2);
-
-    for (;;) {
-        BandPair P;
-        const int fetched = band_fetch(a, tid, n_items, n_pairs, bail, SEED_DIAG_SLACK, &P);
-        if (fetched == 0) break;
-        if (fetched == 2) {
-        const uint32_t ridA = P.ridA, ridB = P.ridB;
-        const bool validB = P.validB;
-        const int lenA = UNI ? (int)a.b.fixed_len : (int)P.lenA, lenB = UNI ? (validB ? (int)a.b.fixed_len : 0) : (int)P.lenB;
-        const int lenmax = UNI ? (int)a.b.fixed_len : max(lenA, lenB);
-        const int dtmin = min(P.dtA, P.dtB), dtmax = max(P.dtA, P.dtB);
-        const bool narrow = dtmax - dtmin < SEED_DIAG_SLACK;
-        const uint32_t infoA = a.info[ridA], infoB = a.info[ridB];
-        const uint32_t masksA = a.band_masks[ridA], masksB = validB ? a.band_masks[ridB] : 0u;
-        const uint32_t fa2 = __builtin_amdgcn_perm(masksB, masksA, 0x05040100u), fb2 = __builtin_amdgcn_perm(masksB, masksA, 0x07060302u);
-        uint32_t lam2 = ulam2;
-        if (!UNI) {
-            band_lane_init(a.sp, st, lenA, masksA, lenB, masksB);
-            lam2 = (uint32_t)st[BF_LAM2 * BLOCK];
-        }
-        const uint32_t lamx = pk_subu_sat(lam2, maxw2);
-        const uint32_t* codeA = a.codes + (size_t)ridA * a.cs;
-        const uint32_t* codeB = a.codes + (size_t)ridB * a.cs;
-        const int base = dtmin - wu;
-        const auto table_row = [&](uint32_t off) { return *reinterpret_cast<const uint2*>(gt + min(off, row_end)); };
-        uint2 w[D];
-        uint32_t H[D], F[D];
-        uint32_t Dc = (a.floor0 - ge1) * 0x00010001u;
-#pragma unroll
-        for (int j = 0; j < D; ++j) {
-            w[j] = table_row((uint32_t)(base + j) * (uint32_t)sizeof(uint2));
-            H[j] = Dc;
-            F[j] = pk_addu(Dc, ge2);
-        }
-        uint32_t Fbelow = pk_addu(Dc, ge2);
-        BandPk up, lo;
-        up.ch = lo.ch = PKB2;
-        up.fr = lo.fr = 0;
-        uint32_t oa2 = 0, ob2 = 0, best = 0;
-#pragma unroll 1
-        for (int k0 = 0; k0 < lenmax; k0 += D) {
-            uint32_t sel[D];
-#pragma unroll
-            for (int d = 0; d < D / 8; ++d) {
-                const uint32_t di = (uint32_t)(k0 / 8 + d);
-                const uint32_t wa = di < a.cs ? codeA[di] : 0xffffffffu;
-                const uint32_t wb = (validB && di < a.cs) ? codeB[di] : 0xffffffffu;
-#pragma unroll
-                for (int j = 0; j < 8; ++j)
-                    sel[8 * d + j] = (uint32_t)sel_lut[(wa >> (4 * j)) & 15u] | ((uint32_t)sel_lut[(wb >> (4 * j)) & 15u] << 16);
-            }
-            uint32_t upS, upE, loS, loE, loI, freeb, anyup, anylo, inj, join, ex, bel, nm, topin;
-            {
-                DiagGroupEvents ev;
-                if (UNI) {
-                    const SeedGroupPatterns g = seed_group_patterns(k0, D, um, uc0, ustride, a.sp.K, a.sp.spacer, umagic);
-                    ev = diag_group_events(g, g, fa2, fb2);
-                } else {
-                    const BandLayout yA = band_layout(st, false), yB = band_layout(st, true);
-                    ev = diag_group_events(seed_group_patterns(k0, D, yA.m, yA.c0, yA.stride, a.sp.K, a.sp.spacer, yA.magic),
-                                           seed_group_patterns(k0, D, yB.m, yB.c0, yB.stride, a.sp.K, a.sp.spacer, yB.magic), fa2, fb2);
-                }
-                upS = ev.upS;
-                upE = ev.upE;
-                loS = ev.loS;
-                loE = ev.loE;
-                loI = ev.loI;
-                freeb = ev.freeb;
-                anyup = upS | upE;
-                anyup |= anyup >> 16;
-                anylo = loS | loE;
-                anylo |= anylo >> 16;
-                const int t0 = base + k0, t1 = dtmax + k0 + 1 + wd;
-                const uint32_t above = seed_bits_from(1 - t0), below = seed_bits_below(R - t1);
-                topin = seed_bits_from(-t0) & seed_bits_below(R - t0);
-                const uint32_t exits = below & seed_bits_from(1 - t1), yfok = below & seed_bits_from(-t1);
-                const uint32_t realA = seed_bits_below(lenA - k0), realB = seed_bits_below(lenB - k0);
-                inj = pair_bits(realA & above, realB & above);
-                join = pair_bits(seed_bits_below(lenA - k0 - 1) & topin, seed_bits_below(lenB - k0 - 1) & topin);
-                ex = pair_bits(realA & exits, realB & exits);
-                bel = pair_bits(realA & below, realB & below);
-                nm = pair_bits(realA & yfok, realB & yfok);
-            }
-            const uint32_t enter = (uint32_t)(base + k0 + D) * (uint32_t)sizeof(uint2);
-#pragma unroll
-            for (int u = 0; u < D; ++u) {
-                if (k0 + u < lenmax) {
-                Dc = pk_addu(Dc, ge2);
-                const uint32_t Dn = pk_addu(Dc, ge2);
-                up.ch += maxw2;
-                up.fr += maxw2;
-                if (__ballot((anyup >> u) & 1u) != 0) pk_events(&up, pair_mask(upS, u), pair_mask(upE, u), lam2);
-                const uint32_t v = pk_subu_sat(pk_maxu(up.ch, up.fr), PKB2) & pair_mask(inj, u);
-                oa2 = pk_maxu(oa2, v);
-                uint32_t E = pk_addu(Dc, pk_tag<TAG>(pk_subu_sat(v, go2p) & lane_mask(topin, u)));
-                uint32_t rmax = 0x04000400u;
-#pragma unroll
-                for (int j = 0; j < D; ++j) {
-                    const uint2 wr = w[(u + j) % D];
-                    const uint32_t hd = pk_addu(H[j], __builtin_amdgcn_perm(wr.y, wr.x, sel[u]));
-                    const uint32_t Fin = j + 1 < D ? F[j + 1 < D ? j + 1 : j] : Fbelow;
-                    const uint32_t h = pk_max3(hd, E, Fin);
-                    H[j] = h;
-                    const uint32_t hg = h - gd2;
-                    F[j] = pk_max3(Fin, hg, Dn);
-                    E = pk_max3(E, hg, Dn) - ge2;
-                    if (j == D - 1) rmax = pk_max3(rmax, H[j - 1], narrow ? 0u : h);
-                    else if (j & 1) rmax = pk_max3(rmax, H[j - 1], h);
-                    if (j == 0) w[u] = table_row(enter + (uint32_t)u * (uint32_t)sizeof(uint2));
-                }
-                best = pk_maxu(best, pk_subu(rmax, Dc));
-                {
-                    const uint32_t ux = pk_addu(pk_untag<TAG>(pk_subu(H[0], Dc)), PKB2) & pair_mask(join, u);
-                    const uint32_t fm = pair_mask(freeb, u);
-                    up.fr = pk_maxu(up.fr, ux & fm);
-                    up.ch = pk_maxu(up.ch, ux & ~fm);
-                }
-                lo.ch += maxw2;
-                lo.fr += maxw2;
-                if (__ballot((anylo >> u) & 1u) != 0) pk_events(&lo, pair_mask(loS, u), pair_mask(loE, u), lam2);
-                const uint32_t he = pk_addu(pk_untag<TAG>(pk_subu(narrow ? H[D - 2] : H[D - 1], Dc)), PKB2) & pair_mask(ex, u);
-                const uint32_t im = pair_mask(loI, u);
-                lo.fr = pk_maxu(lo.fr, he & im);
-                lo.ch = pk_maxu(lo.ch, he & ~im);
-                const uint32_t b2 = pk_subu_sat(pk_maxu(lo.ch, lo.fr), PKB2);
-                ob2 = pk_maxu(ob2, b2 & pair_mask(bel, u));
-                Fbelow = pk_addu(Dn, pk_tag<TAG>(pk_subu_sat(pk_addu(b2, lamx), go2p) & pair_mask(nm, u)));
-                if (narrow) F[D - 1] = Fbelow;
-                }
-            }
-        }
-        band_finish<0, MINS>(a, P, best, oa2, ob2, dtmin, dtmax, lenmax | (wu << 8) | (wd << 20), 1, infoA, infoB, BandEnds{}, &n_accepted, &n_below);
-        }
-    }
-    band_count_accepted(a, tid, n_accepted);
-    if (MINS) band_count_below(a, tid, n_below);
-}
-
+#include "zsw_seed_diag_body.inc"
+}
+
+struct DiagHandbackArgs {
+    SeedBandArgs band;
+    ScoreArgsV2 score;
+    uint32_t hb_blocks;
+};
+static_assert(sizeof(DiagHandbackArgs) <= 4096, "kernel arguments: 4 KB at most");
+static_assert(HANDBACK_BLOCK_THREADS == BLOCK, "zsw_handback.hpp sizes the hand-back blocks");
+
+template <int D, bool UNI, int G, int C>
+__global__ __launch_bounds__(BLOCK, 3) void seed_diag_handback_kernel(DiagHandbackArgs args) {
+    static_assert(min_waves(C, 0) >= 3, "the score body must fit three waves per SIMD");
+    const CoscheduleRole role = coschedule_role(blockIdx.x, args.hb_blocks);
+    if (role.handback) {
+        score_body_v2<G, C, 0>(args.score, role.index);
+    } else {
+        constexpr bool MINS = false;
+        const SeedBandArgs& a = args.band;
+#include "zsw_seed_diag_body.inc"
+    }
+}
+
+template <bool UNI, int G, int C>
+hipError_t launch_diag_handback_cfg(const DiagHandbackArgs& a, hipStream_t stream) {
+    hipLaunchKernelGGL((seed_diag_handback_kernel<DIAG_D, UNI, G, C>), dim3(a.hb_blocks + a.band.grid), dim3(BLOCK), 0, stream, a);
+    return hipGetLastError();
+}
+
+}
+
+hipError_t launch_seed_diag_handback(const SeedBandArgs& a, const ScoreArgsV2& hb, int G, int C, hipStream_t stream) {
+    if (a.wu_per16 != 0 || a.wd_per32 != 0 || a.wu0 + a.wd0 + 1 + SEED_DIAG_SLACK != DIAG_D) return hipErrorInvalidValue;
+    if (a.sp.K + a.sp.spacer < SEED_GROUP_MIN_STRIDE || a.ref_len >= (1u << 24)) return hipErrorInvalidValue;
+    if (!a.retry || a.bail_check || (a.min_thr && a.min_count)) return hipErrorInvalidValue;
+    if (!hb.n_items_dev || !hb.b.items || hb.first_item_dev || hb.chunk_rows || hb.gate_lo != 0 || hb.gate_hi != 0xffffffffu) return hipErrorInvalidValue;
+    DiagHandbackArgs k;
+    k.band = a;
+    k.score = hb;
+    k.hb_blocks = handback_blocks(hb.b.n_items, G);
+    const bool uni = a.b.offsets == nullptr && !a.diag_lane_events;
+    if (G != 4) return hipErrorInvalidValue;
+    switch (C) {
+#define ZSW_CASE(CV) \
+    case CV: return uni ? launch_diag_handback_cfg<true, 4, CV>(k, stream) : launch_diag_handback_cfg<false, 4, CV>(k, stream);
+        ZSW_CASE(19) ZSW_CASE(22) ZSW_CASE(25) ZSW_CASE(28) ZSW_CASE(32) ZSW_CASE(35) ZSW_CASE(38)
+#undef ZSW_CASE
+    }
+    return hipErrorInvalidValue;
 }
 
 uint32_t seed_band_rows(const SeedParams& p, uint32_t max_len) { return (uint32_t)seed_rows_above(p, (int)max_len) + (uint32_t)seed_rows_below(p, (int)max_len) + SEED_BAND_SLACK + 4; }
diff --git a/zoe_amd/csrc/zsw_score_seed.hip b/zoe_amd/csrc/zsw_score_seed.hip
--- a/zoe_amd/csrc/zsw_score_seed.hip
+++ b/zoe_amd/csrc/zsw_score_seed.hip
@@ -200,8 +200,10 @@
 hipError_t launch_score_seeded(const ScoreArgsV2& a2, int G, int C, uint32_t max_len, const SeedIndex& ix, uint8_t* work, size_t work_bytes,
                                uint2* gtab, uint32_t* fail_list, uint32_t* fail_count, int mode, const ScoreArgsV2* band_tabs, const uint2* gtab_band, int32_t* band_dbg,
                                uint32_t narrow_min_reads, uint32_t band_grid_cap, hipStream_t stream, KernelTimer* window_timer, bool narrow_only, bool reads_reversed,
-                               std::vector<uint32_t>* launches, bool strip_first_tier, bool diag_lane_events, uint32_t min_thr, uint32_t* min_counts) {
+                               std::vector<uint32_t>* launches, bool strip_first_tier, bool diag_lane_events, uint32_t min_thr, uint32_t* min_counts,
+                               const CoscheduleCase* co, uint32_t* n0, bool* coscheduled) {
     const uint32_t n = a2.b.n_items;
+    if (coscheduled) *coscheduled = false;
     if (!min_counts) min_thr = 0;
     if (n == 0) return hipSuccess;
     if (!work || !gtab || work_bytes < seed_workspace_bytes(n, max_len, band_grid_cap)) return hipErrorNotSupported;
@@ -325,7 +327,22 @@
             b1.diag_lane_events = diag_lane_events;
             note_launch(launches, ZSW_LAUNCH_SEED_BAND, G, C, mode);
             const bool diagonal = mode == 0 && !narrow_only && !strip_first_tier && seed_diag_applicable(max_len, band_tabs->K);
-            e = launch_seed_band(b1, mode, true, stream, diagonal);
+            CoscheduleCase cc{};
+            if (co) cc = *co;
+            cc.two_tiers = !narrow_only;
+            cc.diagonal = diagonal;
+            if (co && n0 && coscheduled && handback_coschedule(cc) && cc.mode == mode && cc.G == G && cc.mins == (min_thr != 0)) {
+                e = hipMemcpyAsync(n0, fail_count, 4, hipMemcpyDeviceToDevice, stream);
+                if (e != hipSuccess) return e;
+                ScoreArgsV2 hb = a2;
+                hb.b.items = fail_list;
+                hb.n_items_dev = fail_count;
+                note_launch(launches, ZSW_LAUNCH_V2, G, C, 0);
+                e = launch_seed_diag_handback(b1, hb, G, C, stream);
+                *coscheduled = true;
+            } else {
+                e = launch_seed_band(b1, mode, true, stream, diagonal);
+            }
             if (e != hipSuccess) return e;
             if (narrow_only) {
                 if (window_timer) window_timer->end(stream);
diff --git a/zoe_amd/csrc/zsw_score_seed.hpp b/zoe_amd/csrc/zsw_score_seed.hpp
--- a/zoe_amd/csrc/zsw_score_seed.hpp
+++ b/zoe_amd/csrc/zsw_score_seed.hpp
@@ -1,4 +1,5 @@
 #pragma once
+#include "zsw_handback.hpp"
 #include "zsw_internal.hpp"
 #include "zsw_seed.hpp"
 
@@ -101,6 +102,7 @@
 bool seed_diag_applicable(uint32_t max_len, uint32_t rebase_rows);
 
 struct ScoreArgsV2;
+hipError_t launch_seed_diag_handback(const SeedBandArgs& a, const ScoreArgsV2& hb, int G, int C, hipStream_t stream);
 
 constexpr uint32_t SEED_BAND_CLASS_MIN_GRID = 64;
 inline uint32_t seed_band_class_cap(uint32_t n_class, uint32_t n_total) {
@@ -114,7 +116,8 @@
                                uint32_t narrow_min_reads, uint32_t band_grid_cap, hipStream_t stream, KernelTimer* window_timer, bool narrow_only = false, bool reads_reversed = false,
                                std::vector<uint32_t>* launches = nullptr , bool strip_first_tier = false ,
                                bool diag_lane_events = false ,
-                               uint32_t min_thr = 0 , uint32_t* min_counts = nullptr );
+                               uint32_t min_thr = 0 , uint32_t* min_counts = nullptr ,
+                               const CoscheduleCase* co = nullptr, uint32_t* n0 = nullptr, bool* coscheduled = nullptr);
 hipError_t seed_index_update(SeedIndex* ix, const ScoringDev& sc, const uint8_t* h_ref, size_t ref_len);
 void seed_index_release(SeedIndex* ix);
 
diff --git a/zoe_amd/csrc/zsw_score_v2.hpp b/zoe_amd/csrc/zsw_score_v2.hpp
--- a/zoe_amd/csrc/zsw_score_v2.hpp
+++ b/zoe_amd/csrc/zsw_score_v2.hpp
@@ -52,6 +52,7 @@
     const uint32_t* rev_query_end;
     const uint32_t* n_items_dev = nullptr;
     uint32_t gate_lo = 0, gate_hi = 0xffffffffu;
+    const uint32_t* first_item_dev = nullptr;
     uint32_t chunk_rows = 0, chunk_overlap = 0;
     unsigned long long* chunk_keys = nullptr;
 };
@@ -63,7 +64,7 @@
 }
 
 template <int G, int C, int MODE, bool WIDE = false, bool TILED = false>
-__global__ __launch_bounds__(BLOCK, min_waves(C, MODE)) void score_kernel_v2(ScoreArgsV2 a) {
+__device__ __forceinline__ void score_body_v2(const ScoreArgsV2& a, const uint32_t block) {
     __shared__ uint2 rp[WIDE ? 1 : CH + G];
     __shared__ uint16_t rpw[WIDE ? CH + G : 1];
     __shared__ uint32_t wt32[WIDE ? 33 * 9 : 1];
@@ -73,13 +74,15 @@
 
     const int tid = threadIdx.x;
     const int g = tid & (G - 1);
-    const uint32_t group = blockIdx.x * (BLOCK / G) + tid / G;
+    const uint32_t group = block * (BLOCK / G) + tid / G;
     const uint32_t itemA = 2 * group, itemB = 2 * group + 1;
-    const uint32_t n_items = a.n_items_dev ? min(*a.n_items_dev, a.b.n_items) : a.b.n_items;
-    if (2 * blockIdx.x * (BLOCK / G) >= n_items || n_items < a.gate_lo || n_items >= a.gate_hi) return;
+    const uint32_t n_list = a.n_items_dev ? *a.n_items_dev : a.b.n_items;
+    const uint32_t first = (!TILED && a.first_item_dev) ? min(*a.first_item_dev, n_list) : 0u;
+    const uint32_t n_items = min(n_list - first, a.b.n_items);
+    if (2 * block * (BLOCK / G) >= n_items || n_items < a.gate_lo || n_items >= a.gate_hi) return;
     const bool validA = itemA < n_items, validB = itemB < n_items;
-    const uint32_t idA = validA ? (a.b.items ? a.b.items[itemA] : itemA) : 0;
-    const uint32_t idB = validB ? (a.b.items ? a.b.items[itemB] : itemB) : 0;
+    const uint32_t idA = validA ? (a.b.items ? a.b.items[first + itemA] : first + itemA) : 0;
+    const uint32_t idB = validB ? (a.b.items ? a.b.items[first + itemB] : first + itemB) : 0;
 
     if (tid < 64) lut32[tid] = reinterpret_cast<const uint32_t*>(a.sc->index_map)[tid];
     if (tid < 9) swt[tid] = make_uint2(a.wtab[tid][0], a.wtab[tid][1]);
@@ -354,6 +357,11 @@
     }
 }
 
+template <int G, int C, int MODE, bool WIDE = false, bool TILED = false>
+__global__ __launch_bounds__(BLOCK, min_waves(C, MODE)) void score_kernel_v2(ScoreArgsV2 a) {
+    score_body_v2<G, C, MODE, WIDE, TILED>(a, blockIdx.x);
+}
+
 hipError_t launch_table_cfg_v2_wide(const ScoreArgsV2& a, int G, int C, int mode, hipStream_t stream);
 constexpr int TILE_G = 64, TILE_C = 38, TILE_COLS = TILE_G * TILE_C;
 hipError_t launch_tile_v2(const ScoreArgsV2& a, bool wide, int mode, hipStream_t stream);
diff --git a/zoe_amd/csrc/zsw_seed_diag_body.inc b/zoe_amd/csrc/zsw_seed_diag_body.inc
--- /dev/null
+++ b/zoe_amd/csrc/zsw_seed_diag_body.inc
@@ -0,0 +1,168 @@
+    constexpr int TAG = -1;
+    static_assert(D == 16, "a group of columns is two dwords of residue codes and 16 bits per read in the column masks");
+    static_assert(D <= SEED_GROUP_MAX, "three k-mers per group (zsw_seed_diag.hpp)");
+    static_assert(SEED_NARROW_WU_PER16 == 0 && SEED_NARROW_WD_PER32 == 0, "the window's height is fixed at compile time");
+    __shared__ uint16_t sel_lut[16];
+    __shared__ int sst[UNI ? 1 : BF_N * BLOCK];
+    const int tid = threadIdx.x;
+    int* const st = sst + (UNI ? 0 : tid);
+    if (tid < 16) {
+        const uint32_t k = (uint32_t)tid;
+        sel_lut[tid] = (uint16_t)(k < 4 ? (2 * k + 1) | ((8 + k) << 8) : (k == 15 ? 0x0c00u : (2 * (k - 3)) | 0x0c00u));
+    }
+    __syncthreads();
+    const int R = (int)a.ref_len;
+    const uint32_t n_items = a.n_dev ? min(*a.n_dev, a.n) : a.n;
+    const uint32_t n_pairs = (n_items + 1) / 2;
+    const bool bail = a.bail_check && a.accepted && ((uint64_t)(*a.accepted) * SEED_BAIL_RATIO < (uint64_t)n_items || n_items < a.bail_below);
+    uint32_t n_accepted = 0;
+    uint32_t n_below = 0;
+    const uint32_t ge2 = a.ge2, gd2 = a.gd2;
+    const uint32_t ge1 = ge2 & 0xffffu;
+    const uint32_t maxw2 = (uint32_t)a.sp.maxw * 0x00010001u, go2p = (uint32_t)a.sp.go * 0x00010001u;
+    const int wu = a.wu0, wd = a.wd0;
+    int um = 0, ustride = 0, uc0 = 0;
+    uint32_t umagic = 0, ulam2 = 0;
+    if (UNI) {
+        seed_layout((int)a.b.fixed_len, a.sp.K, a.sp.spacer, &um, &ustride, &uc0);
+        umagic = seed_div_magic(ustride);
+        ulam2 = (uint32_t)seed_lambda(a.sp, ustride) * 0x00010001u;
+    }
+    const char* const gt = reinterpret_cast<const char*>(a.gtab + SEED_GTAB_PAD);
+    const uint32_t row_end = (uint32_t)R * (uint32_t)sizeof(uint2);
+
+    for (;;) {
+        BandPair P;
+        const int fetched = band_fetch(a, tid, n_items, n_pairs, bail, SEED_DIAG_SLACK, &P);
+        if (fetched == 0) break;
+        if (fetched == 2) {
+        const uint32_t ridA = P.ridA, ridB = P.ridB;
+        const bool validB = P.validB;
+        const int lenA = UNI ? (int)a.b.fixed_len : (int)P.lenA, lenB = UNI ? (validB ? (int)a.b.fixed_len : 0) : (int)P.lenB;
+        const int lenmax = UNI ? (int)a.b.fixed_len : max(lenA, lenB);
+        const int dtmin = min(P.dtA, P.dtB), dtmax = max(P.dtA, P.dtB);
+        const bool narrow = dtmax - dtmin < SEED_DIAG_SLACK;
+        const uint32_t infoA = a.info[ridA], infoB = a.info[ridB];
+        const uint32_t masksA = a.band_masks[ridA], masksB = validB ? a.band_masks[ridB] : 0u;
+        const uint32_t fa2 = __builtin_amdgcn_perm(masksB, masksA, 0x05040100u), fb2 = __builtin_amdgcn_perm(masksB, masksA, 0x07060302u);
+        uint32_t lam2 = ulam2;
+        if (!UNI) {
+            band_lane_init(a.sp, st, lenA, masksA, lenB, masksB);
+            lam2 = (uint32_t)st[BF_LAM2 * BLOCK];
+        }
+        const uint32_t lamx = pk_subu_sat(lam2, maxw2);
+        const uint32_t* codeA = a.codes + (size_t)ridA * a.cs;
+        const uint32_t* codeB = a.codes + (size_t)ridB * a.cs;
+        const int base = dtmin - wu;
+        const auto table_row = [&](uint32_t off) { return *reinterpret_cast<const uint2*>(gt + min(off, row_end)); };
+        uint2 w[D];
+        uint32_t H[D], F[D];
+        uint32_t Dc = (a.floor0 - ge1) * 0x00010001u;
+#pragma unroll
+        for (int j = 0; j < D; ++j) {
+            w[j] = table_row((uint32_t)(base + j) * (uint32_t)sizeof(uint2));
+            H[j] = Dc;
+            F[j] = pk_addu(Dc, ge2);
+        }
+        uint32_t Fbelow = pk_addu(Dc, ge2);
+        BandPk up, lo;
+        up.ch = lo.ch = PKB2;
+        up.fr = lo.fr = 0;
+        uint32_t oa2 = 0, ob2 = 0, best = 0;
+#pragma unroll 1
+        for (int k0 = 0; k0 < lenmax; k0 += D) {
+            uint32_t sel[D];
+#pragma unroll
+            for (int d = 0; d < D / 8; ++d) {
+                const uint32_t di = (uint32_t)(k0 / 8 + d);
+                const uint32_t wa = di < a.cs ? codeA[di] : 0xffffffffu;
+                const uint32_t wb = (validB && di < a.cs) ? codeB[di] : 0xffffffffu;
+#pragma unroll
+                for (int j = 0; j < 8; ++j)
+                    sel[8 * d + j] = (uint32_t)sel_lut[(wa >> (4 * j)) & 15u] | ((uint32_t)sel_lut[(wb >> (4 * j)) & 15u] << 16);
+            }
+            uint32_t upS, upE, loS, loE, loI, freeb, anyup, anylo, inj, join, ex, bel, nm, topin;
+            {
+                DiagGroupEvents ev;
+                if (UNI) {
+                    const SeedGroupPatterns g = seed_group_patterns(k0, D, um, uc0, ustride, a.sp.K, a.sp.spacer, umagic);
+                    ev = diag_group_events(g, g, fa2, fb2);
+                } else {
+                    const BandLayout yA = band_layout(st, false), yB = band_layout(st, true);
+                    ev = diag_group_events(seed_group_patterns(k0, D, yA.m, yA.c0, yA.stride, a.sp.K, a.sp.spacer, yA.magic),
+                                           seed_group_patterns(k0, D, yB.m, yB.c0, yB.stride, a.sp.K, a.sp.spacer, yB.magic), fa2, fb2);
+                }
+                upS = ev.upS;
+                upE = ev.upE;
+                loS = ev.loS;
+                loE = ev.loE;
+                loI = ev.loI;
+                freeb = ev.freeb;
+                anyup = upS | upE;
+                anyup |= anyup >> 16;
+                anylo = loS | loE;
+                anylo |= anylo >> 16;
+                const int t0 = base + k0, t1 = dtmax + k0 + 1 + wd;
+                const uint32_t above = seed_bits_from(1 - t0), below = seed_bits_below(R - t1);
+                topin = seed_bits_from(-t0) & seed_bits_below(R - t0);
+                const uint32_t exits = below & seed_bits_from(1 - t1), yfok = below & seed_bits_from(-t1);
+                const uint32_t realA = seed_bits_below(lenA - k0), realB = seed_bits_below(lenB - k0);
+                inj = pair_bits(realA & above, realB & above);
+                join = pair_bits(seed_bits_below(lenA - k0 - 1) & topin, seed_bits_below(lenB - k0 - 1) & topin);
+                ex = pair_bits(realA & exits, realB & exits);
+                bel = pair_bits(realA & below, realB & below);
+                nm = pair_bits(realA & yfok, realB & yfok);
+            }
+            const uint32_t enter = (uint32_t)(base + k0 + D) * (uint32_t)sizeof(uint2);
+#pragma unroll
+            for (int u = 0; u < D; ++u) {
+                if (k0 + u < lenmax) {
+                Dc = pk_addu(Dc, ge2);
+                const uint32_t Dn = pk_addu(Dc, ge2);
+                up.ch += maxw2;
+                up.fr += maxw2;
+                if (__ballot((anyup >> u) & 1u) != 0) pk_events(&up, pair_mask(upS, u), pair_mask(upE, u), lam2);
+                const uint32_t v = pk_subu_sat(pk_maxu(up.ch, up.fr), PKB2) & pair_mask(inj, u);
+                oa2 = pk_maxu(oa2, v);
+                uint32_t E = pk_addu(Dc, pk_tag<TAG>(pk_subu_sat(v, go2p) & lane_mask(topin, u)));
+                uint32_t rmax = 0x04000400u;
+#pragma unroll
+                for (int j = 0; j < D; ++j) {
+                    const uint2 wr = w[(u + j) % D];
+                    const uint32_t hd = pk_addu(H[j], __builtin_amdgcn_perm(wr.y, wr.x, sel[u]));
+                    const uint32_t Fin = j + 1 < D ? F[j + 1 < D ? j + 1 : j] : Fbelow;
+                    const uint32_t h = pk_max3(hd, E, Fin);
+                    H[j] = h;
+                    const uint32_t hg = h - gd2;
+                    F[j] = pk_max3(Fin, hg, Dn);
+                    E = pk_max3(E, hg, Dn) - ge2;
+                    if (j == D - 1) rmax = pk_max3(rmax, H[j - 1], narrow ? 0u : h);
+                    else if (j & 1) rmax = pk_max3(rmax, H[j - 1], h);
+                    if (j == 0) w[u] = table_row(enter + (uint32_t)u * (uint32_t)sizeof(uint2));
+                }
+                best = pk_maxu(best, pk_subu(rmax, Dc));
+                {
+                    const uint32_t ux = pk_addu(pk_untag<TAG>(pk_subu(H[0], Dc)), PKB2) & pair_mask(join, u);
+                    const uint32_t fm = pair_mask(freeb, u);
+                    up.fr = pk_maxu(up.fr, ux & fm);
+                    up.ch = pk_maxu(up.ch, ux & ~fm);
+                }
+                lo.ch += maxw2;
+                lo.fr += maxw2;
+                if (__ballot((anylo >> u) & 1u) != 0) pk_events(&lo, pair_mask(loS, u), pair_mask(loE, u), lam2);
+                const uint32_t he = pk_addu(pk_untag<TAG>(pk_subu(narrow ? H[D - 2] : H[D - 1], Dc)), PKB2) & pair_mask(ex, u);
+                const uint32_t im = pair_mask(loI, u);
+                lo.fr = pk_maxu(lo.fr, he & im);
+                lo.ch = pk_maxu(lo.ch, he & ~im);
+                const uint32_t b2 = pk_subu_sat(pk_maxu(lo.ch, lo.fr), PKB2);
+                ob2 = pk_maxu(ob2, b2 & pair_mask(bel, u));
+                Fbelow = pk_addu(Dn, pk_tag<TAG>(pk_subu_sat(pk_addu(b2, lamx), go2p) & pair_mask(nm, u)));
+                if (narrow) F[D - 1] = Fbelow;
+                }
+            }
+        }
+        band_finish<0, MINS>(a, P, best, oa2, ob2, dtmin, dtmax, lenmax | (wu << 8) | (wd << 20), 1, infoA, infoB, BandEnds{}, &n_accepted, &n_below);
+        }
+    }
+    band_count_accepted(a, tid, n_accepted);
+    if (MINS) band_count_below(a, tid, n_below);
```

After: 690.0 million (median of 6 runs). +5.4%, better.
